# SeoYeonnLee/Video-Chapter-Generation

Hardware: AMD Instinct MI355X
Metric: clip-windows/sec (16f×224²+128tok) train-step at 1/2/4/8 MI355X; % HBM roofline (higher is better)
Workload: dtype bf16; 1 GPU; TwoStream train step: TSM-ResNet-50 + BERT-base + ChapterHead(mlp), B=64 windows/GPU of 16x224^2 frames + 128 tokens, fused clip+AdamW; global_batch=64, seq_len=128, frames=16, resolution=224, text_fill=n_valid ~ U[L/2, L], parallelism=dp1

## Files before the change

### include/vcg_hip.h

```cpp
#ifndef VCG_HIP_H
#define VCG_HIP_H
#include <hip/hip_runtime.h>
#include <stdint.h>
#include "vcg_gpt_decode.h"
#ifdef __cplusplus
extern "C" {
#endif

#define VCG_API
enum { VCG_F32 = 0, VCG_BF16 = 1 };
enum { VCG_GRAD_F32 = 0x10 };
enum { VCG_OK = 0, VCG_ERR_INVALID = -1, VCG_ERR_UNSUPPORTED = -2, VCG_ERR_HIP = -3 };
enum { VCG_ACT_NONE = 0, VCG_ACT_RELU = 1, VCG_ACT_GELU = 2, VCG_ACT_TANH = 3, VCG_ACT_GELU_BWD = 4 };
enum { VCG_ACT_GELU_TANH = 5, VCG_ACT_GELU_TANH_BWD = 6 };
enum { VCG_ACT_FLAG_ROUND_PRE = 0x100 };
enum { VCG_ACT_FLAG_WIDE = 0x200 };
enum { VCG_ACT_FLAG_F32_OUT = 0x400 };
VCG_API int vcg_gemm_census_enable(int on);
VCG_API int vcg_gemm_census_size(void);
VCG_API int vcg_gemm_census_get(int i, char* key, int n, long long* count);

VCG_API const char* vcg_last_error(void);
VCG_API int vcg_version(void);
VCG_API int vcg_init(int device);
VCG_API int vcg_finalize(void);
VCG_API int vcg_sync(hipStream_t stream);
VCG_API int vcg_timing_enable(int on);
VCG_API int vcg_timing_query(int kernel_id, double* ms_total, long long* launches, double* flops);
VCG_API int vcg_timing_roofline(int kernel_id, double peak_tflops, double peak_gbs, double* ms_total, double* ideal_ms, double* bytes, double* flops);
VCG_API int vcg_patch_stamps(unsigned long long* out, int n);
VCG_API int vcg_fast_stamps(unsigned long long* out, int n);
VCG_API int vcg_g256_stamps(unsigned long long* out, int n);
VCG_API int vcg_wide_stamps(unsigned long long* out, int n);

VCG_API int vcg_conv_stats_tiles(int M);
VCG_API int vcg_conv_fwd(int dtype, const void* x, const void* w, void* y, float* stats, int N, int H, int W, int C, int Cout, int KH, int KW, int stride, int pad, int tsm_T, int tsm_fold, hipStream_t stream);
VCG_API int vcg_conv_fwd_bias_act(int dtype, const void* x, const void* w, const float* bias, int act, void* y, int N, int H, int W, int C, int Cout, int KH, int KW, int stride, int pad, int tsm_T, int tsm_fold, hipStream_t stream);
VCG_API int vcg_conv_dgrad(int dtype, const void* dy, const void* wt, void* dx, int N, int H, int W, int C, int Cout, int KH, int KW, int stride, int pad, hipStream_t stream);
VCG_API long long vcg_conv_dgrad_bwd_ws_bytes(int C, int Cout, int KH, int KW);
VCG_API long long vcg_conv_dgrad_bwd_p_ws_bytes(int C, int a2_c);
VCG_API int vcg_conv_dgrad_bwd(int dtype, const void* dy, const void* wt, void* g, int N, int H, int W, int C, int Cout, int KH, int KW, int stride, int pad, int tsm_T, int tsm_fold, const void* res, int res_stride, const unsigned char* bits, const void* y, const float* mean, const float* invstd, const float* mscale, const float* mshift, const void* y2, const float* mean2, const float* invstd2, float* ws, long long ws_bytes, float* sum_g, float* sum_gx, float* dgamma, float* dbeta, float* sum_gx2, float* dgamma2, float* dbeta2, const void* a2, int a2_c, float* pg, float* pws, long long pws_bytes, hipStream_t s);
VCG_API long long vcg_conv_wgrad_ws_bytes(int dtype, int N, int H, int W, int C, int Cout, int KH, int KW, int stride, int pad);
VCG_API int vcg_conv_wgrad(int dtype, const void* x, const void* dy, float* dw, int accumulate, float* ws, long long ws_bytes, int N, int H, int W, int C, int Cin, int Cout, int KH, int KW, int stride, int pad, int tsm_T, int tsm_fold, hipStream_t stream);
VCG_API int vcg_conv1x1_bn_res_relu(const void* x, const void* wfold, const float* bias, const void* res, const float* res_scale, const float* res_shift, void* out, unsigned char* bits, int M, int N, int K, hipStream_t stream);
VCG_API int vcg_bn_bwd_fold_weights(const void* wt, int N, int K, const float* mean, const float* invstd, const float* gamma, const float* sum_g, const float* sum_gx, float inv_count, void* wfold, float* bias, hipStream_t stream);
VCG_API long long vcg_bn_apply_colsum_ws_bytes(long long P, int C);
VCG_API int vcg_bn_apply_colsum(const void* y, const float* scale, const float* shift, int relu, void* out, float* colsum, float* ws, long long ws_bytes, long long P, int C, hipStream_t s);
VCG_API long long vcg_bn_apply_gram_ws_bytes(long long P, int C);
VCG_API int vcg_bn_apply_gram(const void* y, const float* scale, const float* shift, const float* mean, const float* invstd, void* out, float* colsum, float* gram, double* g64, float* ws, long long ws_bytes, long long P, int C, hipStream_t s);
VCG_API int vcg_bn_stats_from_gram(const double* g64, const void* w, long long M, int N, int C, float* stats, int mtiles, hipStream_t s);
VCG_API int vcg_bn_finalize_from_gram(const double* g64, const void* w, long long M, int N, int C, const float* gamma,
                                      const float* beta, float* mean, float* invstd, float* scale, float* shift,
                                      float* running_mean, float* running_var, float momentum, float eps,
                                      const float* w32, void* wfold, hipStream_t s);
VCG_API int vcg_conv1x1_stats(const void* x, const void* w, float* stats, int M, int N, int K, hipStream_t stream);
VCG_API int vcg_bn_bwd_sumgx_from_wgrad(const float* P, const void* w, int K, int C, const float* mean, const float* invstd, const float* sum_g, float* sum_gx, float* dgamma, hipStream_t stream);
VCG_API int vcg_bn_bwd_fold_weights_a2(const void* wt, int C, int K, const float* invstd, const float* gamma, const float* sum_g, const float* sum_gx, float inv_count, const float* colsum_a, void* wfold, float* bias, hipStream_t stream);
VCG_API int vcg_bn_bwd_fold_wgrad_a2(const float* P, const float* G, const float* w3, int K, int C, const float* mean, const float* invstd, const float* gamma, const float* sum_g, const float* sum_gx, float inv_count, const float* colsum_a, float* dw, int accumulate, hipStream_t stream);
VCG_API int vcg_conv_dgrad_bwd_bnfold(const void* g, const void* yg, int Ky, const void* wfold, const float* bias, void* out, int N, int H, int W, int C, int Cout, const void* y, const float* mean, const float* invstd, const float* mscale, const float* mshift, float* ws, long long ws_bytes, float* sum_g, float* sum_gx, float* dgamma, float* dbeta, hipStream_t stream);
VCG_API long long vcg_conv_wgrad_bnfold_ws_bytes(int N, int H, int W, int C, int Cout);
VCG_API int vcg_conv_wgrad_bnfold(const void* x, const void* g, const void* yg, const float* mean, const float* invstd, const float* gamma, const float* sum_g, const float* sum_gx, float inv_count, const float* colsum_x, float* dw, int accumulate, float* ws, long long ws_bytes, int N, int H, int W, int C, int Cout, hipStream_t stream);
VCG_API int vcg_gemm(int dtype, int transA, int transB, int M, int N, int K, const void* A, long long lda, const void* B, long long ldb, void* C, long long ldc, const float* bias, int act, const void* residual, long long ldr, void* aux, float alpha, hipStream_t stream);
VCG_API int vcg_gemm_batched(int dtype, int transA, int transB, int M, int N, int K, const void* A, long long lda, long long a_so, long long a_si, const void* B, long long ldb, long long b_so, long long b_si, void* C, long long ldc, long long c_so, long long c_si, int batch_outer, int batch_inner, const float* bias, int act, float alpha, hipStream_t stream);
VCG_API long long vcg_gemm_splitk_ws_bytes(int dtype, int M, int N, int K);
VCG_API int vcg_gemm_splitk(int dtype, int transA, int transB, int M, int N, int K, const void* A, long long lda, const void* B, long long ldb, float* out, int accumulate, float* ws, long long ws_bytes, hipStream_t stream);

VCG_API int vcg_bn_finalize(const float* stats, int mtiles, int M, int C, const float* gamma, const float* beta, float* mean_out, float* invstd_out, float* scale_out, float* shift_out, float* running_mean, float* running_var, float momentum, float eps, hipStream_t s);
VCG_API int vcg_bn_eval_params(const float* gamma, const float* beta, const float* rm, const float* rv, float eps, int C, float* mean_out, float* invstd_out, float* scale, float* shift, hipStream_t s);
VCG_API int vcg_bn_apply(int dtype, const void* y, const float* scale, const float* shift, const void* res, const float* rscale, const float* rshift, int relu, void* out, unsigned char* bits, long long P, int C, hipStream_t s);
VCG_API long long vcg_bn_bwd_ws_bytes(long long P, int C);
VCG_API int vcg_bn_bwd_reduce(int dtype, const void* dout, int mask_mode, const void* mask, const unsigned char* mbits, const float* mscale, const float* mshift, const void* y, const float* mean, const float* invstd, long long P, int C, float* ws, long long ws_bytes, float* sum_g, float* sum_gx, float* dgamma, float* dbeta, int accumulate, hipStream_t s);
VCG_API int vcg_bn_bwd_apply(int dtype, const void* dout, int mask_mode, const void* mask, const unsigned char* mbits, const float* mscale, const float* mshift, const void* y, const float* mean, const float* invstd, const float* gamma, const float* sum_g, const float* sum_gx, long long count, int train_stats, void* dy, void* gout, long long P, int C, hipStream_t s);
VCG_API int vcg_bn_bwd_apply_dual(int dtype, const void* g, const void* y, const float* mean, const float* invstd, const float* gamma, const float* sum_g, const float* sum_gx, const void* yd, const float* mean_d, const float* invstd_d, const float* gamma_d, const float* sum_g_d, const float* sum_gx_d, long long count, void* dy, void* dyd, long long P, int C, hipStream_t s);
VCG_API int vcg_maxpool_fwd(int dtype, const void* x, void* y, unsigned char* idx, int N, int H, int W, int C, hipStream_t s);
VCG_API int vcg_maxpool_bwd(int dtype, const void* dy, const unsigned char* idx, void* dx, int N, int H, int W, int C, hipStream_t s);
VCG_API long long vcg_maxpool_bwd_bn_ws_bytes(int C);
VCG_API int vcg_maxpool_bwd_bn(int dtype, const void* dy, const unsigned char* idx, void* g, int N, int H, int W, int C, const void* y, const float* mean, const float* invstd, const float* mscale, const float* mshift, float* ws, long long ws_bytes, float* sum_g, float* sum_gx, float* dgamma, float* dbeta, hipStream_t s);
VCG_API int vcg_maxpool_bwd_bn_sums_pooled(int dtype, const void* dy, const void* mp, const unsigned char* idx, const void* y, int N, int H, int W, int C, const float* mean, const float* invstd, const float* mscale, const float* mshift, float* ws, long long ws_bytes, float* sum_g, float* sum_gx, float* dgamma, float* dbeta, hipStream_t s);
VCG_API int vcg_maxpool_bwd_bn_apply(int dtype, const void* dy, const unsigned char* idx, void* dx, int N, int H, int W, int C, const void* y, const float* mean, const float* invstd, const float* mscale, const float* mshift, const float* gamma, const float* sum_g, const float* sum_gx, long long count, int train_stats, hipStream_t s);
VCG_API long long vcg_stem_bwd_fused_ws_bytes(void);
VCG_API int vcg_stem_bwd_fused_fits(int N, int H, int W);
VCG_API int vcg_stem_bwd_fused(const void* dy, const unsigned char* idx, const void* y, const void* x, int N, int H, int W, const float* mean, const float* invstd, const float* mscale, const float* mshift, const float* gamma, const float* sum_g, const float* sum_gx, long long count, int train_stats, float* ws, long long ws_bytes, float* dw, int accumulate, hipStream_t s);
VCG_API int vcg_bn_relu_maxpool(int dtype, const void* y, const float* scale, const float* shift, void* out, unsigned char* idx, int N, int H, int W, int C, hipStream_t s);
VCG_API int vcg_avgpool_fwd(int dtype, const void* x, float* y, int N, int HW, int C, hipStream_t s);
VCG_API int vcg_avgpool_bwd(int dtype, const float* dy, void* dx, int N, int HW, int C, hipStream_t s);
VCG_API int vcg_frames_to_nhwc(int dtype, const float* src, void* dst, int N, int C, int H, int W, int Cpad, hipStream_t s);
VCG_API int vcg_window_frames_u8(int dtype, const uint8_t* frames, const long long* idx, void* dst, long long n_rows, int F, int H, int W, const float* mean3, const float* std3, hipStream_t s);
VCG_API int vcg_window_frames_u8_cpad(int dtype, const uint8_t* frames, const long long* idx, void* dst, long long n_rows, int F, int H, int W, int Cpad, const float* mean3, const float* std3, hipStream_t s);
VCG_API int vcg_weight_prep(int dtype, const float* w, void* out, int Cout, int Cin, int KH, int KW, int Cpad, int transposed, hipStream_t s);
VCG_API int vcg_weight_fold(int dtype, const float* w, const float* scale, void* out, int rows, int cols, hipStream_t s);
VCG_API int vcg_weight_prep_multi(int dtype, const long long* desc, int n, hipStream_t s);
VCG_API int vcg_transpose(int dtype, const void* in, void* out, int rows, int cols, long long ld_in, long long ld_out, hipStream_t s);
VCG_API int vcg_transpose_multi(const long long* desc, int n, int total_tiles, hipStream_t s);
VCG_API int vcg_cast_from_f32(int dtype, const float* in, void* out, long long n, hipStream_t s);
VCG_API int vcg_cast_to_f32(int dtype, const void* in, float* out, long long n, hipStream_t s);
VCG_API int vcg_tsm_shift(int dtype, const void* x, void* y, long long n_batch, int T, int C, long long HW, int fold_div, int direction, hipStream_t s);
VCG_API int vcg_tsm_unshift_add(int dtype, const void* dshift, const void* other, const unsigned char* other_bits, void* dx, long long NT, int T, long long HW, int C, int fold, hipStream_t s);

VCG_API int vcg_embed_ln_fwd(int dtype, const long long* ids, const float* word, const float* pos, const float* type, const float* gamma, const float* beta, void* out, float* mean, float* rstd, int B, int L, int H, float eps, float dropout_p, unsigned long long seed, hipStream_t s);
VCG_API long long vcg_ln_bwd_ws_bytes(int rows, int H);
VCG_API int vcg_embed_ln_bwd(int dtype, const void* dout, const long long* ids, const float* word, const float* pos, const float* type, const float* gamma, const float* mean, const float* rstd, float* word_grad, float* pos_grad, float* type_grad, float* gamma_grad, float* beta_grad, float* ws, long long ws_bytes, int B, int L, int H, float dropout_p, unsigned long long seed, long long pad_idx, hipStream_t s);
VCG_API int vcg_ln_fwd(int dtype, const void* x, const void* res, const float* gamma, const float* beta, void* out, float* mean, float* rstd, int rows, int H, float eps, float dropout_p, unsigned long long seed, hipStream_t s);
VCG_API int vcg_ln_bwd(int dtype, const void* dout, const void* x, const void* res, const float* gamma, const float* mean, const float* rstd, void* dx, void* dres, float* gamma_grad, float* beta_grad, float* bias_grad, float* ws, long long ws_bytes, int rows, int H, float dropout_p, unsigned long long seed, hipStream_t s);
VCG_API long long vcg_colsum_ws_bytes(int rows, int N);
VCG_API int vcg_colsum(int dtype, const void* x, long long ld, int rows, int N, float* out, int accumulate, float* ws, long long ws_bytes, hipStream_t s);
VCG_API int vcg_attn_softmax_fwd(int dtype, const void* S, const long long* mask, void* P, void* Pd, int B, int nh, int L, int Lp, float scale, float dropout_p, unsigned long long seed, hipStream_t s);
VCG_API int vcg_attn_softmax_bwd(int dtype, const void* dPd, const void* P, void* dS, int Z, int L, int Lp, float scale, float dropout_p, unsigned long long seed, hipStream_t s);
VCG_API long long vcg_bert_attn_stats_bytes(int B, int nh, int L);
VCG_API int vcg_bert_attn_fwd(const void* qkv, const long long* mask, void* ctx, void* stats, int B, int nh, int L, int Lp, float scale, float dropout_p, unsigned long long seed, hipStream_t s);
VCG_API int vcg_bert_attn_bwd(const void* qkv, const void* dctx, const void* ctx, const long long* mask, const void* stats, void* dqkv, int B, int nh, int L, int Lp, float scale, float dropout_p, unsigned long long seed, hipStream_t s);
VCG_API int vcg_bert_attn_fwd_varlen(const void* qkv, const long long* mask, const int* seq, void* ctx, void* stats, int B, int nh, int Lmax, int Lp, float scale, float dropout_p, unsigned long long seed, hipStream_t s);
VCG_API int vcg_bert_attn_bwd_varlen(const void* qkv, const void* dctx, const long long* mask, const int* seq, const void* stats, void* dqkv, int B, int nh, int Lmax, int Lp, float scale, float dropout_p, unsigned long long seed, hipStream_t s);
enum { VCG_ATTN_CAUSAL = 1 };
VCG_API int vcg_bert_attn_fwd_ex(const void* qkv, const long long* mask, const int* seq, void* ctx, void* stats, int B, int nh, int Lmax, int Lp, float scale, float dropout_p, unsigned long long seed, int flags, hipStream_t s);
VCG_API int vcg_bert_attn_bwd_ex(const void* qkv, const void* dctx, const long long* mask, const int* seq, const void* stats, void* dqkv, int B, int nh, int Lmax, int Lp, float scale, float dropout_p, unsigned long long seed, int flags, hipStream_t s);
VCG_API int vcg_attn_softmax_fwd_ex(int dtype, const void* S, const long long* mask, void* P, void* Pd, int B, int nh, int L, int Lp, float scale, float dropout_p, unsigned long long seed, int flags, hipStream_t s);
VCG_API int vcg_attn_softmax_bwd_ex(int dtype, const void* dPd, const void* P, void* dS, int Z, int L, int Lp, float scale, float dropout_p, unsigned long long seed, int flags, hipStream_t s);
VCG_API int vcg_gpt_embed_fwd(int dtype, const long long* ids, const float* tok, const float* pos, void* out, int B, int L, int H, float dropout_p, unsigned long long seed, hipStream_t s);
VCG_API int vcg_gpt_embed_bwd(int dtype, const void* dout, const long long* ids, float* tok_grad, float* pos_grad, float* ws, long long ws_bytes, int B, int L, int H, float dropout_p, unsigned long long seed, hipStream_t s);
VCG_API int vcg_tanh_bwd(int dtype, const void* dy, const void* t, void* dx, long long n, hipStream_t s);

VCG_API int vcg_head_mlp_fwd(int dtype, const void* Vout, const void* Lout, const float* W, const float* bias, float* logits, float* prob, int B, int T, int hid, int O, hipStream_t s);
VCG_API int vcg_head_mlp_bwd(int dtype, const void* Vout, const void* Lout, const float* W, const float* dlogits, void* dV, void* dL, float* dW, float* dbias, int B, int T, int hid, int O, int relu_mask, hipStream_t s);
VCG_API long long vcg_head_attn_saved_floats(int B, int T, int hid, int nh);
VCG_API int vcg_head_attn_fwd(int dtype, const void* Vout, const void* Lout, const float* Wq, const float* bq, const float* Wk, const float* bk, const float* Wv, const float* bv, const float* Wp, const float* bp, float* saved, long long saved_floats, float* logits, float* prob, int B, int T, int hid, int nh, int O, float dropout_p, unsigned long long seed, hipStream_t s);
VCG_API long long vcg_head_attn_bwd_ws_floats(int B, int T, int hid);
VCG_API int vcg_head_attn_bwd(int dtype, const float* saved, const float* Wq, const float* Wk, const float* Wv, const float* Wp, const float* dlogits, void* dVout, void* dLout, float* dWq, float* dbq, float* dWk, float* dbk, float* dWv, float* dbv, float* dWp, float* dbp, float* ws, long long ws_floats, int B, int T, int hid, int nh, int O, float dropout_p, unsigned long long seed, int relu_mask, hipStream_t s);
VCG_API long long vcg_window_attn_weight_floats(int H, int nh, int P);
VCG_API int vcg_window_attn_fwd(const float* emb, const float* weights, long long weight_floats, float* logits, float* prob, int B, int S, int H, int nh, int P, hipStream_t s);
VCG_API long long vcg_cross_attn_weight_floats(int H);
VCG_API int vcg_cross_attn_fwd(const float* lang, const float* vis, const float* weights, long long weight_floats, float* out, int B, int T, int H, int nh, hipStream_t s);
VCG_API int vcg_mul_fwd(const float* a, const float* b, float* out, long long n, hipStream_t s);
VCG_API int vcg_rowdot_fwd(const float* U, const float* x, const float* bias, float* out, int B, int R, int K, hipStream_t s);
VCG_API int vcg_rowdot_bwd(const float* U, const float* x, const float* dy, float* dU, float* dx, int B, int R, int K, hipStream_t s);
VCG_API int vcg_ln_act_fwd(const float* x, const float* gamma, const float* beta, float* out, int rows, int D, float eps, int act, hipStream_t s);
VCG_API int vcg_cross_entropy_fwd(const float* logits, const long long* labels, float* loss, int B, int C, hipStream_t s);
VCG_API int vcg_cross_entropy_bwd(const float* logits, const long long* labels, const float* dloss, float* dlogits, int B, int C, hipStream_t s);

VCG_API long long vcg_sumsq_ws_bytes(void);
VCG_API int vcg_sumsq(const float* x, long long n, float* ws, float* out, hipStream_t s);
VCG_API int vcg_adamw(float* p, const float* g, float* m, float* v, const unsigned char* wd_flags, int flag_shift, long long n, float lr, float beta1, float beta2, float eps, float wd, float step_size, float bc2_sqrt, const float* sumsq, float max_norm, float grad_scale, void* bf16_shadow, hipStream_t s);

VCG_API int vcg_ln_act_drop_fwd(const float* x, const float* gamma, const float* beta, float* out, float* mean, float* rstd, int rows, int D, float eps, int act, float dropout_p, unsigned long long seed, hipStream_t s);
VCG_API long long vcg_ln_act_drop_bwd_ws_bytes(int rows, int D);
VCG_API int vcg_ln_act_drop_bwd(const float* dout, const float* x, const float* gamma, const float* beta, const float* mean, const float* rstd, float* dx, float* gamma_grad, float* beta_grad, float* ws, long long ws_bytes, int rows, int D, int act, float dropout_p, unsigned long long seed, hipStream_t s);
VCG_API int vcg_act_drop_fwd(const float* x, const float* res, float* out, long long n, int act, float dropout_p, unsigned long long seed, hipStream_t s);
VCG_API int vcg_act_drop_bwd(const float* dout, const float* x, float* dx, long long n, int act, float dropout_p, unsigned long long seed, hipStream_t s);
VCG_API int vcg_mul_bwd(const float* dout, const float* a, const float* b, float* da, float* db, long long n, hipStream_t s);
VCG_API int vcg_mha_small_fwd(const float* q, long long ldq, const float* k, long long ldk, const float* v, long long ldv, const float* bias, int Pb, float* ctx, long long ldc, float* probs, int B, int Sq, int Sk, int nh, int dh, float scale, float dropout_p, unsigned long long seed, hipStream_t s);
VCG_API long long vcg_mha_small_bwd_ws_bytes(int B, int nh, int Pb);
VCG_API int vcg_mha_small_bwd(const float* q, long long ldq, const float* k, long long ldk, const float* v, long long ldv, const float* probs, const float* dctx, long long lddc, float* dq, long long lddq, float* dk, long long lddk, float* dv, long long lddv, float* dbias, int Pb, float* ws, long long ws_bytes, int B, int Sq, int Sk, int nh, int dh, float scale, float dropout_p, unsigned long long seed, hipStream_t s);

VCG_API int vcg_posenc_fwd(const float* x, const float* pos, const float* w, const float* b, float* out, long long rows, int S, int H, hipStream_t s);
VCG_API int vcg_posenc_bwd(const float* d, const float* pos, float* dw, float* db, long long rows, int S, int H, hipStream_t s);
VCG_API int vcg_linear_small_fwd(const float* x, const float* W, const float* b, const float* res, float* y, int M, int N, int K, int act, hipStream_t s);
VCG_API int vcg_linear_small_bwd(const float* g, const float* x, const float* W, float* dx, float* dw, float* db, int M, int N, int K, hipStream_t s);
VCG_API int vcg_softmax_rows(const float* x, float* out, int rows, int C, hipStream_t s);

VCG_API long long vcg_mlm_loss_ws_bytes(int R, int V, int H);
VCG_API int vcg_mlm_loss_fwd(const void* hidden, int rows_total, const long long* rows, const void* W, const long long* targets, int R, int V, int H, float* ws, long long ws_bytes, float* lse, float* row_loss, float* mean_loss, long long* n_correct, hipStream_t stream);
VCG_API int vcg_mlm_loss_bwd(const void* hidden, int rows_total, const long long* rows, const void* W, const long long* targets, const float* lse, const float* dloss, int R, int V, int H, void* dZ, long long ldz, hipStream_t stream);
VCG_API int vcg_mlm_logits(const void* hidden, int rows, const void* W, int V, int H, float* logits, long long ldz, hipStream_t stream);
VCG_API int vcg_mlm_reduce_f32(const float* logits, long long ldz, const long long* targets, int R, int V, float* ws, long long ws_bytes, float* lse, float* row_loss, float* mean_loss, long long* n_correct, hipStream_t stream);
VCG_API int vcg_mlm_dz_f32(float* logits, long long ldz, const float* lse, const long long* targets, const float* dloss, int R, int V, hipStream_t stream);
VCG_API int vcg_seq_softmax_fwd(const float* logits, long long ldz, float* prob, long long ldp, int B, int L, int V, hipStream_t stream);

VCG_API int vcg_momentum_update(float* k, const float* q, long long n, float m, float one_minus_m, void* k_shadow, hipStream_t stream);
VCG_API int vcg_l2norm_fwd(int dtype, const void* x, void* y, float* denom, int N, int H, float eps, hipStream_t stream);
VCG_API int vcg_l2norm_bwd(int dtype, const float* g, const void* x, const float* denom, float* dx, int N, int H, hipStream_t stream);
VCG_API int vcg_contrast_select(int dtype, const void* q, const void* cand, int B, int C, int H, float eps, long long* k0, hipStream_t stream);
VCG_API int vcg_queue_enqueue(int key_dtype, int km_dtype, const void* keys, float* queue, void* queue_km, long long* queue_ptr, int N, int K, int H, hipStream_t stream);
VCG_API int vcg_queue_rebuild(int km_dtype, const float* queue, void* queue_km, int K, int H, hipStream_t stream);
VCG_API int vcg_rowdot(int dtype, const void* a, const void* b, int N, int H, float scale, float* out, long long ldo, hipStream_t stream);
VCG_API long long vcg_infonce_ws_bytes(int N, int K, int H);
VCG_API int vcg_infonce_fwd(const void* q, const void* queue_km, const float* lpos, int N, int K, int H, float inv_T, float* ws, long long ws_bytes, float* lse, float* row_loss, float* one_minus_p0, float* mean_loss, long long* n_correct, hipStream_t stream);
VCG_API int vcg_infonce_dz(const void* q, const void* queue_km, const float* lse, int N, int K, int H, float inv_T, float scale, void* dZ, long long ldz, hipStream_t stream);
VCG_API int vcg_infonce_logits(const void* q, const void* queue_km, int N, int K, int H, float inv_T, float* key_logits, long long ldz, hipStream_t stream);
VCG_API int vcg_infonce_reduce_f32(const float* key_logits, long long ldz, const float* lpos, int N, int K, float* ws, long long ws_bytes, float* lse, float* row_loss, float* one_minus_p0, float* mean_loss, long long* n_correct, hipStream_t stream);
VCG_API int vcg_infonce_dz_f32(float* key_logits, long long ldz, const float* lse, float scale, int N, int K, hipStream_t stream);
VCG_API int vcg_infonce_dq_pos(int dtype, float* dq, const void* k, const float* one_minus_p0, float scale, int N, int H, hipStream_t stream);

VCG_API int vcg_listnet_max_slate(void);
VCG_API int vcg_listnet_max_hidden(void);
VCG_API int vcg_listnet_fwd(int dtype, const void* P, const float* targets, const long long* sel, const long long* cls, const float* W, const float* bias, int B, int S, int H, int M, float* p, float* logits, float* prob, float* part, float* loss3, hipStream_t stream);
VCG_API int vcg_listnet_bwd(int dtype, const void* P, const float* targets, const long long* sel, const long long* cls, const float* W, const float* p, const float* prob, const float* dloss, int B, int S, int H, int M, float* dP, float* dW, float* db, hipStream_t stream);

VCG_API int vcg_attn_decode(int dtype, const void* qkv_new, void* kcache, void* vcache, const int* len0, int max_len0, int t, void* ctx, int B, int nh, int dh, int Tcap, float scale, hipStream_t s);
VCG_API int vcg_sample_topk(const float* logits, long long ldz, int B, int V, float temperature, int top_k, int greedy, const float* u, long long* seq, int Tcap, const int* len0, int max_len0, int col_off, const long long* forced, long long forced_ld, long long* chosen, long long chosen_ld, float* prob, hipStream_t s);
VCG_API int vcg_gpt_embed_at(int dtype, const long long* seq, int Tcap, const int* len0, int max_len0, int t, const float* tok, const float* pos, void* out, int B, int H, int V, int n_pos, hipStream_t s);
VCG_API int vcg_gemm_skinny(const void* x, const void* W, const float* bias, void* y, int M, int N, int K, long long ldc, int act, int f32_out, hipStream_t s);
VCG_API long long vcg_gpt_decode_desc_bytes(void);
VCG_API int vcg_gpt_decode_step(const vcg_gpt_decode_desc* d, int t, hipStream_t s);

VCG_API int vcg_cross_attn_kv_fwd(int dtype, const void* q, long long ldq, const void* kv, long long ldkv, const long long* key_mask, void* ctx, float* stats, int B, int nh, int dh, int Lq, int Lk, float scale, hipStream_t s);
VCG_API int vcg_pegasus_embed_fwd(int dtype, const long long* ids, const float* tok, const float* pos, void* out, int B, int L, int H, int V, int n_pos, float scale, int pos0, hipStream_t s);

VCG_API int vcg_cross_attn_kv_fwd_ex(int dtype, const void* q, long long ldq, const void* kv, long long ldkv, const long long* key_mask, void* ctx, float* stats, int B, int nh, int dh, int Lq, int Lk, float scale, float dropout_p, unsigned long long seed, hipStream_t s);
VCG_API int vcg_cross_attn_kv_bwd(int dtype, const void* q, long long ldq, const void* kv, long long ldkv, const long long* key_mask, const void* dctx, long long lddo, const float* stats, float* d_ws, void* dq, long long lddq, void* dkv, long long lddkv, int B, int nh, int dh, int Lq, int Lk, float scale, float dropout_p, unsigned long long seed, hipStream_t s);
VCG_API int vcg_pegasus_embed_fwd_ex(int dtype, const long long* ids, const float* tok, const float* pos, void* out, int B, int L, int H, int V, int n_pos, float scale, int pos0, float dropout_p, unsigned long long seed, hipStream_t s);
VCG_API int vcg_pegasus_embed_bwd(int dtype, const void* dout, const long long* ids, float* tok_grad, float* ws, long long ws_bytes, int B, int L, int H, float scale, long long pad_idx, float dropout_p, unsigned long long seed, hipStream_t s);
VCG_API int vcg_ln_bwd_acc(int dtype, const void* dout, const float* x, const float* gamma, const float* mean, const float* rstd, float* dh, float* gamma_grad, float* beta_grad, float* ws, long long ws_bytes, int rows, int H, hipStream_t s);
VCG_API int vcg_dropout_add_fwd(int dtype, float* h, const void* branch, long long n, float dropout_p, unsigned long long seed, hipStream_t s);
VCG_API int vcg_dropout_add_bwd(int dtype, const float* dh, void* dbranch, long long n, float dropout_p, unsigned long long seed, hipStream_t s);
VCG_API int vcg_relu_dropout_fwd(int dtype, const void* pre, void* f, long long n, float dropout_p, unsigned long long seed, hipStream_t s);
VCG_API int vcg_relu_dropout_bwd(int dtype, const void* dy, const void* f, void* dpre, long long n, float dropout_p, hipStream_t s);

VCG_API int vcg_comm_unique_id(void* uid_out, int uid_bytes);
VCG_API int vcg_comm_init(int rank, int world, const void* uid, int uid_bytes);
VCG_API int vcg_comm_world(int* rank, int* world);
VCG_API int vcg_allreduce_bucket(void* ptr, long long count, int dtype, hipStream_t s);
VCG_API int vcg_broadcast_bucket(void* ptr, long long count, int dtype, int root, hipStream_t s);
VCG_API int vcg_comm_finalize(void);

VCG_API int vcg_synth(int kind, void* out, long long n, unsigned long long key, double a, double b, hipStream_t s);

#ifdef __cplusplus
}
#endif
#endif
```

### video-chapter-generation_amd/csrc/igemm.h

```cpp
#pragma once
#include "common.h"

namespace vcg {

enum { OP_DENSE_K = 0, OP_IM2COL = 1, OP_DGRAD = 2, OP_DENSE_MN = 3, OP_IM2COL_T = 4 };
enum { EPI_STORE = 0, EPI_STATS = 1, EPI_SPLITK = 2, EPI_BWD = 3, EPI_BWD_AFF = 4, EPI_STORE_AUX = 5,
       EPI_BWD_STREAM = 6 };
enum { ACT_NONE = 0, ACT_RELU = 1, ACT_GELU = 2, ACT_TANH = 3, ACT_GELU_BWD = 4, ACT_GELU_TANH = 5, ACT_GELU_TANH_BWD = 6 };
__host__ __device__ __forceinline__ bool act_is_gelu_bwd(int act) { return act == ACT_GELU_BWD || act == ACT_GELU_TANH_BWD; }
enum { ACT_FLAG_ROUND_PRE = 0x100 };
enum { ACT_FLAG_WIDE = 0x200 };
enum { ACT_FLAG_F32_OUT = 0x400 };

template <typename T> struct Cfg;
template <> struct Cfg<float> { static constexpr int VEC = 4, BK = 16, LDK = 20; };
template <> struct Cfg<bf16_t> { static constexpr int VEC = 8, BK = 32, LDK = 40; };

template <typename T, int COLS> struct LdMN {
  static constexpr int v = sizeof(T) == 2 ? (COLS == 128 ? 144 : 80) : (COLS == 128 ? 132 : 68);
};

constexpr bool is_kcontig(int mode) { return mode == OP_DENSE_K || mode == OP_IM2COL || mode == OP_DGRAD; }

struct OpArgs {
  const void* ptr;
  long long bytes;
  long long ld;
  int rows;
  int N, H, W, C, logC;
  int GH, GW;
  int KH, KW, stride, pad;
  int tsm_T, tsm_fold;
  FastDiv fd_ghw, fd_gw, fd_T;
  int tKH, tKW, tkh0, tkw0, ry, rx;
  int sw, pw;
  const void* ptr2;
  int split2;
  long long ld2, bytes2;
};

struct BwdEpi {
  int tsm_T, tsm_fold;
  FastDiv fd_hw, fd_T;
  int hw;
  const void* res;
  int res_s;
  int rH, rW;
  FastDiv fd_w;
  const uint8_t* bits;
  const void* y;
  const float *mean, *invstd, *msc, *msh;
  const void* y2;
  const float *mean2, *invstd2;
  float* part;
  int nred;
  const void* a2;
  int pj;
  float* ppart;
  int sub, cW, ry, rx, fH, fW;
  FastDiv fd_chw, fd_cw;
};

struct GemmParams {
  int M, N, K;
  int k_per_split;
  OpArgs a, b;
  void* C;
  long long ldc;
  const float* bias;
  int act;
  const void* residual;
  long long ldr;
  void* aux;
  float alpha;
  float* stats;
  float* ws;
  int batch_inner;
  long long a_so, a_si, b_so, b_si, c_so, c_si;
  int res_round;
  int fast_act;
  BwdEpi bwd;
  uint8_t* obits;
  const float *res_sc, *res_sh;
};


template <typename T> __device__ __forceinline__ void load4(const T* p, float (&v)[4]) {
  if constexpr (sizeof(T) == 4) {
    const float4 q = *reinterpret_cast<const float4*>(p);
    v[0] = q.x; v[1] = q.y; v[2] = q.z; v[3] = q.w;
  } else {
    const uint2 q = *reinterpret_cast<const uint2*>(p);
    v[0] = __uint_as_float(q.x << 16); v[1] = __uint_as_float(q.x & 0xffff0000u);
    v[2] = __uint_as_float(q.y << 16); v[3] = __uint_as_float(q.y & 0xffff0000u);
  }
}
template <typename T> __device__ __forceinline__ void store4(T* p, const float (&v)[4]) {
  if constexpr (sizeof(T) == 4) {
    *reinterpret_cast<float4*>(p) = make_float4(v[0], v[1], v[2], v[3]);
  } else {
    uint2 q;
    q.x = (uint32_t)f2bf(v[0]) | ((uint32_t)f2bf(v[1]) << 16);
    q.y = (uint32_t)f2bf(v[2]) | ((uint32_t)f2bf(v[3]) << 16);
    *reinterpret_cast<uint2*>(p) = q;
  }
}

__device__ __forceinline__ float apply_act(float v, int act, bool fast = false) {
  if (act == ACT_RELU) return fmaxf(v, 0.f);
  if (act == ACT_GELU) return fast ? gelu_erf_fast(v) : gelu_erf(v);
  if (act == ACT_TANH) return tanhf(v);
  if (act == ACT_GELU_TANH) return fast ? gelu_tanh_fast(v) : gelu_tanh(v);
  return v;
}


__device__ __forceinline__ float row16_sum(float v) {
  v += __builtin_bit_cast(float, __builtin_amdgcn_update_dpp(0, __builtin_bit_cast(int, v), 0xB1, 0xF, 0xF, false));
  v += __builtin_bit_cast(float, __builtin_amdgcn_update_dpp(0, __builtin_bit_cast(int, v), 0x4E, 0xF, 0xF, false));
  v += __builtin_bit_cast(float, __builtin_amdgcn_update_dpp(0, __builtin_bit_cast(int, v), 0x141, 0xF, 0xF, false));
  v += __builtin_bit_cast(float, __builtin_amdgcn_update_dpp(0, __builtin_bit_cast(int, v), 0x140, 0xF, 0xF, false));
  return v;
}

template <int BN>
__device__ __forceinline__ void load_bias(float (&bv)[BN / 32][4], const float* bias, int n0, int wn, int lane, int N) {
#pragma unroll
  for (int j = 0; j < BN / 32; ++j) {
    const int n = n0 + wn * (BN / 2) + 4 * (lane >> 4) + j * 16;
    float4 b4 = make_float4(0.f, 0.f, 0.f, 0.f);
    if (bias && n < N) b4 = *reinterpret_cast<const float4*>(bias + n);
    bv[j][0] = b4.x; bv[j][1] = b4.y; bv[j][2] = b4.z; bv[j][3] = b4.w;
  }
}

__device__ __forceinline__ void ep_barrier() {
  __builtin_amdgcn_s_waitcnt(0xC07F);
  __builtin_amdgcn_s_barrier();
}

template <typename T, int BM, int BN, int EPI>
__device__ __forceinline__ void gemm_epilogue(f32x4 (&acc)[BM / 32][BN / 32], const GemmParams& p, float* red,
                                              const float (&bv)[BN / 32][4], T* Cout, const T* Res, int m0, int n0,
                                              int wm, int wn, int lane, int mtile, int mtiles) {
  constexpr int MT = BM / 32, NT = BN / 32;
  const int g = lane >> 4, ci = lane & 15;
  const int mbase = m0 + wm * (BM / 2) + ci, nbase = n0 + wn * (BN / 2) + 4 * g;
#pragma unroll
  for (int j = 0; j < NT; ++j) {
    const int n = nbase + j * 16;
#pragma unroll
    for (int i = 0; i < MT; ++i) {
      const int m = mbase + i * 16;
      if (m >= p.M || n >= p.N) {
        acc[i][j] = f32x4{0.f, 0.f, 0.f, 0.f};
        continue;
      }
      float v[4];
#pragma unroll
      for (int r = 0; r < 4; ++r) v[r] = acc[i][j][r] * p.alpha + bv[j][r];
      if (Res) {
        float rv[4];
        load4<T>(Res + (long long)m * p.ldr + n, rv);
        if (p.act == ACT_GELU_BWD) {
#pragma unroll
          for (int r = 0; r < 4; ++r) v[r] *= (sizeof(T) == 2 && p.fast_act) ? gelu_erf_grad_fast(rv[r]) : gelu_erf_grad(rv[r]);
        } else if (p.act == ACT_GELU_TANH_BWD) {
#pragma unroll
          for (int r = 0; r < 4; ++r) v[r] *= (sizeof(T) == 2 && p.fast_act) ? gelu_tanh_grad_fast(rv[r]) : gelu_tanh_grad(rv[r]);
        } else {
#pragma unroll
          for (int r = 0; r < 4; ++r) v[r] += rv[r];
        }
      }
      if (p.aux) store4<T>(reinterpret_cast<T*>(p.aux) + (long long)m * p.ldc + n, v);
      if (p.act != ACT_NONE && !act_is_gelu_bwd(p.act)) {
#pragma unroll
        for (int r = 0; r < 4; ++r) v[r] = apply_act(v[r], p.act, sizeof(T) == 2 && p.fast_act);
      }
      if constexpr (EPI == EPI_STATS) {
#pragma unroll
        for (int r = 0; r < 4; ++r) acc[i][j][r] = to_f<T>(from_f<T>(v[r]));
      } else {
        store4<T>(Cout + (long long)m * p.ldc + n, v);
      }
    }
  }
  if constexpr (EPI == EPI_STATS) {
    const int r0 = m0 + wm * (BM / 2);
    const int cw = min(BM / 2, max(0, p.M - r0));
    const float inv_cw = cw > 0 ? 1.f / (float)cw : 0.f;
#pragma unroll
    for (int j = 0; j < NT; ++j)
#pragma unroll
      for (int r = 0; r < 4; ++r) {
        float t = 0.f;
#pragma unroll
        for (int i = 0; i < MT; ++i) t += acc[i][j][r];
        t = row16_sum(t);
        const float mean = t * inv_cw;
        float q = 0.f;
#pragma unroll
        for (int i = 0; i < MT; ++i) {
          const float d = acc[i][j][r] - mean;
          q += (mbase + i * 16 < p.M) ? d * d : 0.f;
        }
        q = row16_sum(q);
        if (ci == 0) {
          const int lc = wn * (BN / 2) + j * 16 + 4 * g + r;
          red[wm * 2 * BN + lc] = mean;
          red[wm * 2 * BN + BN + lc] = q;
        }
      }
    ep_barrier();
    if (wm == 0 && ci == 0) {
      const float n1 = (float)min(BM / 2, max(0, p.M - m0));
      const float n2 = (float)min(BM / 2, max(0, p.M - m0 - BM / 2));
#pragma unroll
      for (int j = 0; j < NT; ++j)
#pragma unroll
        for (int r = 0; r < 4; ++r) {
          const int lc = wn * (BN / 2) + j * 16 + 4 * g + r;
          const int col = n0 + lc;
          if (col >= p.N) continue;
          float mean = red[lc], m2 = red[BN + lc];
          if (n2 > 0.f) {
            const float mb = red[2 * BN + lc], d = mb - mean, nt = n1 + n2;
            mean += d * (n2 / nt);
            m2 += red[3 * BN + lc] + d * d * (n1 * n2 / nt);
          }
          reinterpret_cast<float2*>(p.stats)[(long long)col * mtiles + mtile] = make_float2(mean, m2);
        }
    }
    if (blockIdx.x == 0 && threadIdx.x == 0)
      reinterpret_cast<float2*>(p.stats)[(long long)p.N * mtiles + mtile] =
          make_float2((float)min(BM, p.M - m0), 0.f);
#pragma unroll
    for (int j = 0; j < NT; ++j) {
      const int n = nbase + j * 16;
#pragma unroll
      for (int i = 0; i < MT; ++i) {
        const int m = mbase + i * 16;
        if (m >= p.M || n >= p.N) continue;
        float v[4] = {acc[i][j][0], acc[i][j][1], acc[i][j][2], acc[i][j][3]};
        store4<T>(Cout + (long long)m * p.ldc + n, v);
      }
    }
  }
}

int run_fast_gemm(GemmParams& p, int amode, int epi, int z, hipStream_t s);
int fast_grid_rows(int M, int N, int z, int epi);
bool fast_bwd_streams(const GemmParams& p);
int wide_gemm_class(const GemmParams& p);
int wide_gemm_class_f32(const GemmParams& p);
int run_gemm_wide(GemmParams& p, int we, hipStream_t s);
int fast_bwd_slots(const GemmParams& p);
int run_patch_conv(const GemmParams& p, int amode, int epi, hipStream_t s);
int patch_bwd_slots(const GemmParams& p);
int bn_bwd_finalize_launch(const float* partial, int nb, int C, long long ld, int gx_off, float* sum_g, float* sum_gx,
                           float* dgamma, float* dbeta, int accumulate, hipStream_t s);
int run_fast_wgrad(const GemmParams& p, int splits, hipStream_t s, bool dense_b = false);
int wgrad_patch_rows(int dtype, int H, int W, int C, int Cin, int Cout, int KH, int KW, int stride, int pad,
                     int tsm_fold);
int wgrad_patch_splits(int C, int Cout);
int run_rs1x1_bnres(const void* x, const void* wfold, const float* bias, const void* res, void* out, uint8_t* bits,
                    long long M, int N, int K, hipStream_t s);
int run_wgrad_patch(const void* x, const void* dy, float* ws, int N, int H, int W, int C, int Cout, int R,
                    hipStream_t s);
int wgrad_fast_tile_m(int M);
int wgrad_fast_tile_n(int N);

bool gemm256_ok(const GemmParams& p, int amode, int epi, int z);
int run_gemm256(const GemmParams& p, int amode, int epi, hipStream_t s);

}
```

### video-chapter-generation_amd/csrc/igemm.hip

```cpp
#include <cstdio>

#include "igemm.h"

namespace vcg {

template <typename T, int ROWS, int MODE> struct Loader {
  static constexpr int VEC = Cfg<T>::VEC, BK = Cfg<T>::BK;
  static constexpr int NC = ROWS * 4 / 256;
  static constexpr bool KC = is_kcontig(MODE);
  static constexpr int CPR = ROWS / VEC;

  uint4 reg[NC];
  const T* ptr[NC];
  int ra[NC], rb[NC], rc[NC];
  int sub[NC];
  int lds_off[NC];

  __device__ __forceinline__ void init(const OpArgs& a, int row0, int tid) {
    const T* base = reinterpret_cast<const T*>(a.ptr);
#pragma unroll
    for (int j = 0; j < NC; ++j) {
      const int q = tid + j * 256;
      if constexpr (KC) {
        const int row = q >> 2;
// ... 810 lines not shown
}

static void wgrad_geometry(int dtype, int N, int H, int W, int C, int Cout, int KH, int KW, int stride, int pad,
                           int* M, int* Nn, int* K, int* splits, int* kps, bool* fast) {
  const int OH = (H + 2 * pad - KH) / stride + 1, OW = (W + 2 * pad - KW) / stride + 1;
  const bool pair = stem_pair(dtype, C);
  int KWp = KW, pwp = 0;
  if (pair) pair_taps(KW, pad, &KWp, &pwp);
  *M = Cout;
  *Nn = pair ? KH * KWp * 8 : KH * KW * C;
  *K = N * OH * OW;
  *fast = wgrad_fast_ok(dtype, N, H, pair ? W / 2 : W, pair ? 8 : C, Cout, *K);
  int BK, sp;
  if (*fast) {
    BK = 64;
    const int tiles = ((*Nn + wgrad_fast_tile_n(*Nn) - 1) / wgrad_fast_tile_n(*Nn)) *
                      ((*M + wgrad_fast_tile_m(*M) - 1) / wgrad_fast_tile_m(*M));
    sp = (splitk_target() + tiles - 1) / tiles;
    const int max_sp = (*K + 8 * BK - 1) / (8 * BK);
    sp = sp > max_sp ? max_sp : sp;
    sp = sp < 1 ? 1 : sp;
  } else {
    BK = dtype == VCG_BF16 ? 32 : 16;
    sp = choose_splits(*M, *Nn, *K, BK);
  }
  int k = (*K + sp - 1) / sp;
  k = (k + BK - 1) / BK * BK;
  *kps = k;
  *splits = (*K + k - 1) / k;
}

VCG_API long long vcg_conv_wgrad_ws_bytes(int dtype, int N, int H, int W, int C, int Cout, int KH, int KW,
                                          int stride, int pad) {
  int M, Nn, K, splits, kps;
  bool fast;
  wgrad_geometry(dtype, N, H, W, C, Cout, KH, KW, stride, pad, &M, &Nn, &K, &splits, &kps, &fast);
  if (wgrad_patch_rows(dtype, H, W, C, C, Cout, KH, KW, stride, pad, 0) > 0 && splits < wgrad_patch_splits(C, Cout))
    splits = wgrad_patch_splits(C, Cout);
  return (long long)splits * M * Nn * 4;
}

static int conv_wgrad_impl(int dtype, const void* x, const float* in_sc, const float* in_sh, const void* dy,
                           float* dw, int accumulate, float* ws, long long ws_bytes, int N, int H, int W, int C, int Cin,
                           int Cout, int KH, int KW, int stride, int pad, int tsm_T, int tsm_fold, hipStream_t stream);

VCG_API int vcg_conv_wgrad(int dtype, const void* x, const void* dy, float* dw, int accumulate, float* ws,
                           long long ws_bytes, int N, int H, int W, int C, int Cin, int Cout, int KH, int KW,
                           int stride, int pad, int tsm_T, int tsm_fold, hipStream_t stream) {
  return conv_wgrad_impl(dtype, x, nullptr, nullptr, dy, dw, accumulate, ws, ws_bytes, N, H, W, C, Cin, Cout, KH, KW,
                         stride, pad, tsm_T, tsm_fold, stream);
}

static int conv_wgrad_impl(int dtype, const void* x, const float* in_sc, const float* in_sh, const void* dy,
                           float* dw, int accumulate, float* ws, long long ws_bytes, int N, int H, int W, int C, int Cin,
                           int Cout, int KH, int KW, int stride, int pad, int tsm_T, int tsm_fold, hipStream_t stream) {
  const int logC = ilog2_exact(C);
  VCG_REQUIRE(logC >= 0, "C must be a power of two");
  VCG_REQUIRE(Cout % 64 == 0, "Cout must be a multiple of 64");
  int M, Nn, K, splits, kps;
  bool fast;
  wgrad_geometry(dtype, N, H, W, C, Cout, KH, KW, stride, pad, &M, &Nn, &K, &splits, &kps, &fast);
  const bool pair = stem_pair(dtype, C);
  int KWp = KW, pwp = 0;
  if (pair) pair_taps(KW, pad, &KWp, &pwp);
  VCG_REQUIRE(!pair || (fast && stride == 2 && W % 2 == 0 && tsm_fold == 0),
              "bf16 C = 4 (pair-packed stem) needs stride 2, even W, no TSM and the fast engine");
  VCG_REQUIRE(ws_bytes >= (long long)splits * M * Nn * 4, "workspace too small");
  const int OH = (H + 2 * pad - KH) / stride + 1, OW = (W + 2 * pad - KW) / stride + 1;
  GemmParams p{};
  p.M = M;
  p.N = Nn;
  p.K = K;
  p.k_per_split = kps;
  p.a = dense_op(dy, Cout, Cout);
  p.a.bytes = (long long)K * Cout * (dtype == VCG_BF16 ? 2 : 4);
  OpArgs b{};
  b.ptr = x; b.rows = Nn; b.N = N; b.H = H; b.W = W; b.C = C; b.logC = logC;
  b.bytes = (long long)N * H * W * C * (dtype == VCG_BF16 ? 2 : 4);
  b.GH = OH; b.GW = OW; b.KH = KH; b.KW = KW; b.stride = stride; b.pad = pad;
  b.tsm_T = tsm_T > 0 ? tsm_T : 1; b.tsm_fold = tsm_fold;
  b.fd_ghw = make_fastdiv(OH * OW); b.fd_gw = make_fastdiv(OW); b.fd_T = make_fastdiv(b.tsm_T);
  if (pair) {
    b.W = W / 2; b.C = 8; b.logC = 3; b.KW = KWp; b.sw = 1; b.pw = pwp;
  }
  p.b = b;
  p.ws = ws;
  p.alpha = 1.f;
  const int wpr = wgrad_patch_rows(dtype, H, W, C, Cin, Cout, KH, KW, stride, pad, tsm_fold);
  if (wpr > 0) {
    const int wsp = wgrad_patch_splits(C, Cout);
    VCG_REQUIRE(ws_bytes >= (long long)wsp * M * Nn * 4, "workspace too small");
    if (FILE* f = gemm_log())
      fprintf(f, "a=3 b=4 epi=2 M=%d N=%d K=%d z=%d fast=3 conv=%dx%d/%d C=%d\n", M, Nn, K, wsp, KH, KW, stride, C);
    int rc = run_wgrad_patch(x, dy, ws, N, H, W, C, Cout, wpr, stream);
    if (rc) return rc;
    const long long MN = (long long)M * Nn;
    splitk_reduce(stream, ws, wsp, MN,
                       Nn, dw, accumulate, 1, KH, KW, C, Cin, 1.f, KW, 0, pad);
    VCG_LAUNCH_CHECK();
    return VCG_OK;
  }
  FILE* f = fast ? gemm_log() : nullptr;
  if (f)
    fprintf(f, "a=3 b=4 epi=2 M=%d N=%d K=%d z=%d fast=2 conv=%dx%d/%d C=%d\n", M, Nn, K, splits, KH, KW, stride, C);
  int rc;
  if (fast)
    rc = run_fast_wgrad(p, splits, stream);
  else
    rc = dtype == VCG_BF16 ? run_gemm<bf16_t, OP_DENSE_MN, OP_IM2COL_T>(p, EPI_SPLITK, splits, stream)
                           : run_gemm<float, OP_DENSE_MN, OP_IM2COL_T>(p, EPI_SPLITK, splits, stream);
  if (rc) return rc;
  const long long MN = (long long)M * Nn;
  splitk_reduce(stream, ws, splits,
                     MN, Nn, dw, accumulate, pair ? 2 : 1, KH, KW, C, Cin, 1.f, KWp, pwp, pad);
  VCG_LAUNCH_CHECK();
  return VCG_OK;
}

namespace {
__global__ __launch_bounds__(256) void bn_fold_weights_kernel(const bf16_t* __restrict__ wt, int K,
                                                              const float* __restrict__ mean,
                                                              const float* __restrict__ invstd,
                                                              const float* __restrict__ gamma,
                                                              const float* __restrict__ sum_g,
                                                              const float* __restrict__ sum_gx, float ic,
                                                              bf16_t* __restrict__ wf, float* __restrict__ bias) {
  __shared__ float red[256];
  const int n = blockIdx.x, t = threadIdx.x;
  float acc = 0.f;
  for (int k = t; k < K; k += 256) {
    const float is = invstd[k], A = (gamma ? gamma[k] : 1.f) * is;
    const float B = -A * is * sum_gx[k] * ic;
    const float w = bf2f(wt[(long long)n * K + k]);
    const bf16_t wy = f2bf(B * w);
    wf[(long long)n * 2 * K + k] = f2bf(A * w);
    wf[(long long)n * 2 * K + K + k] = wy;
    acc += (-A * sum_g[k] * ic) * w - mean[k] * bf2f(wy);
  }
  red[t] = acc;
  __syncthreads();
  for (int o = 128; o > 0; o >>= 1) {
    if (t < o) red[t] += red[t + o];
    __syncthreads();
  }
  if (t == 0) bias[n] = red[0];
}

template <int G>
__global__ __launch_bounds__(256) void splitk_reduce_bnfold_kernel(const float* __restrict__ ws, int splits, int Cout,
                                                                   int N, const float* __restrict__ mean,
                                                                   const float* __restrict__ invstd,
                                                                   const float* __restrict__ gamma,
                                                                   const float* __restrict__ sum_g,
                                                                   const float* __restrict__ sum_gx, float ic,
                                                                   const float* __restrict__ cs, float* __restrict__ out,
                                                                   int accumulate) {
  const long long MN = (long long)Cout * N, slab = 2 * MN;
  const long long gid = blockIdx.x * (long long)blockDim.x + threadIdx.x;
  const long long idx = gid / G;
  const int t = (int)(gid - idx * G);
  if (idx >= MN) return;
  float v1 = 0.f, v2 = 0.f;
  const float* p = ws + idx;
  for (int s = t; s < splits; s += G) {
    v1 += p[(long long)s * slab];
    v2 += p[(long long)s * slab + MN];
  }
#pragma unroll
  for (int o = G / 2; o > 0; o >>= 1) {
    v1 += __shfl_xor(v1, o, 64);
    v2 += __shfl_xor(v2, o, 64);
  }
  if (t != 0) return;
  const int k = (int)(idx / N), n = (int)(idx - (long long)k * N);
  const float is = invstd[k], A = (gamma ? gamma[k] : 1.f) * is;
  const float B = -A * is * sum_gx[k] * ic;
  const float Cc = -A * sum_g[k] * ic - B * mean[k];
  const float v = fmaf(A, v1, fmaf(B, v2, Cc * cs[n]));
  if (accumulate) out[idx] += v;
  else out[idx] = v;
}
}

VCG_API int vcg_bn_bwd_fold_weights(const void* wt, int N, int K, const float* mean, const float* invstd,
                                    const float* gamma, const float* sum_g, const float* sum_gx, float inv_count,
                                    void* wfold, float* bias, hipStream_t stream) {
  VCG_REQUIRE(wt && wfold && bias && mean && invstd && sum_g && sum_gx, "null argument");
  VCG_REQUIRE(N > 0 && K > 0, "empty weight");
  hipLaunchKernelGGL(bn_fold_weights_kernel, dim3(N), dim3(256), 0, stream, (const bf16_t*)wt, K, mean, invstd, gamma,
                     sum_g, sum_gx, inv_count, (bf16_t*)wfold, bias);
  VCG_LAUNCH_CHECK();
  return VCG_OK;
}

namespace {
constexpr int FW_NB = 2;
__global__ __launch_bounds__(256) void bn_fold_weights_a2_kernel(const bf16_t* __restrict__ wt, int C, int K,
                                                                 const float* __restrict__ invstd,
                                                                 const float* __restrict__ gamma,
                                                                 const float* __restrict__ sum_g,
                                                                 const float* __restrict__ sum_gx, float ic,
                                                                 const float* __restrict__ colsum_a,
                                                                 bf16_t* __restrict__ wf, float* __restrict__ bias) {
  __shared__ float bw[FW_NB][2048];
  __shared__ float red[FW_NB][256];
  const int n0 = blockIdx.x * FW_NB, t = threadIdx.x;
  float acc[FW_NB];
#pragma unroll
  for (int q = 0; q < FW_NB; ++q) acc[q] = 0.f;
  for (int k = t; k < K; k += 256) {
    const float is = invstd[k], A = (gamma ? gamma[k] : 1.f) * is;
    const float B = -A * is * sum_gx[k] * ic;
#pragma unroll
    for (int q = 0; q < FW_NB; ++q) {
      const int n = n0 + q;
      if (n < C) {
        const float w = bf2f(wt[(long long)n * K + k]);
        bw[q][k] = B * w;
        wf[(long long)n * (K + C) + k] = f2bf(A * w);
        acc[q] += (-A * sum_g[k] * ic) * w;
      }
    }
  }
  __syncthreads();
  for (int j = t; j < C; j += 256) {
    const bf16_t* row = wt + (long long)j * K;
    float qv[FW_NB];
#pragma unroll
    for (int q = 0; q < FW_NB; ++q) qv[q] = 0.f;
    for (int k0 = 0; k0 < K; k0 += 64) {
      uint4 u8[8];
#pragma unroll
      for (int b = 0; b < 8; ++b) u8[b] = *reinterpret_cast<const uint4*>(row + k0 + 8 * b);
#pragma unroll
      for (int b = 0; b < 8; ++b) {
        const uint32_t w4[4] = {u8[b].x, u8[b].y, u8[b].z, u8[b].w};
#pragma unroll
        for (int e = 0; e < 8; ++e) {
          const float w = __uint_as_float((e & 1) ? (w4[e >> 1] & 0xffff0000u) : (w4[e >> 1] << 16));
#pragma unroll
          for (int q = 0; q < FW_NB; ++q) qv[q] = fmaf(w, bw[q][k0 + 8 * b + e], qv[q]);
        }
      }
    }
#pragma unroll
    for (int q = 0; q < FW_NB; ++q) {
      const int n = n0 + q;
      if (n < C) {
        const bf16_t qb = f2bf(qv[q]);
        wf[(long long)n * (K + C) + K + j] = qb;
        acc[q] -= colsum_a[j] * ic * bf2f(qb);
      }
    }
  }
#pragma unroll
  for (int q = 0; q < FW_NB; ++q) red[q][t] = acc[q];
  __syncthreads();
  for (int o = 128; o > 0; o >>= 1) {
    if (t < o) {
#pragma unroll
      for (int q = 0; q < FW_NB; ++q) red[q][t] += red[q][t + o];
    }
    __syncthreads();
  }
  if (t < FW_NB && n0 + t < C) bias[n0 + t] = red[t][0];
}

__global__ __launch_bounds__(256) void bn_fold_wgrad_a2_kernel(const float* __restrict__ P, const float* __restrict__ G,
                                                               const float* __restrict__ w3, int K, int C,
                                                               const float* __restrict__ mean,
                                                               const float* __restrict__ invstd,
                                                               const float* __restrict__ gamma,
                                                               const float* __restrict__ sum_g,
                                                               const float* __restrict__ sum_gx, float ic,
                                                               const float* __restrict__ cs, float* __restrict__ dw,
                                                               int accumulate) {
  __shared__ float wr[512];
  const int k = blockIdx.x;
  for (int i = threadIdx.x; i < C; i += 256) wr[i] = w3[(long long)k * C + i];
  __syncthreads();
  const float is = invstd[k], A = (gamma ? gamma[k] : 1.f) * is;
  const float B = -A * is * sum_gx[k] * ic;
  const float Cc = -A * sum_g[k] * ic - B * mean[k];
  for (int j = threadIdx.x; j < C; j += 256) {
    float wg = 0.f;
    for (int i0 = 0; i0 < C; i0 += 16) {
      float gv[16];
#pragma unroll
      for (int u = 0; u < 16; ++u) gv[u] = G[(long long)(i0 + u) * C + j];
#pragma unroll
      for (int u = 0; u < 16; ++u) wg = fmaf(wr[i0 + u], gv[u], wg);
    }
    const float v = fmaf(A, P[(long long)k * C + j], fmaf(B, wg, Cc * cs[j]));
    float* o = dw + (long long)k * C + j;
    *o = accumulate ? *o + v : v;
  }
}
}

namespace {
__global__ __launch_bounds__(64) void bn_sumgx_kernel(const float* __restrict__ P, const bf16_t* __restrict__ w, int C,
                                                      const float* __restrict__ mean, const float* __restrict__ invstd,
                                                      const float* __restrict__ sum_g, float* __restrict__ sum_gx,
                                                      float* __restrict__ dgamma) {
  const int k = blockIdx.x, t = threadIdx.x;
  float a = 0.f;
  for (int j = t; j < C; j += 64) a = fmaf(bf2f(w[(long long)k * C + j]), P[(long long)k * C + j], a);
#pragma unroll
  for (int o = 32; o > 0; o >>= 1) a += __shfl_xor(a, o, 64);
  if (t == 0) {
    const float v = invstd[k] * (a - mean[k] * sum_g[k]);
    sum_gx[k] = v;
    if (dgamma) dgamma[k] += v;
  }
}
}

VCG_API int vcg_bn_bwd_sumgx_from_wgrad(const float* P, const void* w, int K, int C, const float* mean,
                                        const float* invstd, const float* sum_g, float* sum_gx, float* dgamma,
                                        hipStream_t stream) {
  VCG_REQUIRE(P && w && mean && invstd && sum_g && sum_gx, "null argument");
  VCG_REQUIRE(K > 0 && C > 0, "empty");
  hipLaunchKernelGGL(bn_sumgx_kernel, dim3(K), dim3(64), 0, stream, P, (const bf16_t*)w, C, mean, invstd, sum_g,
                     sum_gx, dgamma);
  VCG_LAUNCH_CHECK();
  return VCG_OK;
}

VCG_API int vcg_bn_bwd_fold_weights_a2(const void* wt, int C, int K, const float* invstd, const float* gamma,
                                       const float* sum_g, const float* sum_gx, float inv_count, const float* colsum_a,
                                       void* wfold, float* bias, hipStream_t stream) {
  VCG_REQUIRE(wt && wfold && bias && invstd && sum_g && sum_gx && colsum_a, "null argument");
  VCG_REQUIRE(C > 0 && K > 0 && K <= 2048 && K % 64 == 0, "K must be a multiple of 64, <= 2048");
  VCG_REQUIRE(((uintptr_t)wt & 15) == 0, "wt must be 16-B aligned");
  hipLaunchKernelGGL(bn_fold_weights_a2_kernel, dim3((C + FW_NB - 1) / FW_NB), dim3(256), 0, stream, (const bf16_t*)wt, C, K, invstd, gamma,
                     sum_g, sum_gx, inv_count, colsum_a, (bf16_t*)wfold, bias);
  VCG_LAUNCH_CHECK();
  return VCG_OK;
}

VCG_API int vcg_bn_bwd_fold_wgrad_a2(const float* P, const float* G, const float* w3, int K, int C, const float* mean,
                                     const float* invstd, const float* gamma, const float* sum_g, const float* sum_gx,
                                     float inv_count, const float* colsum_a, float* dw, int accumulate,
                                     hipStream_t stream) {
  VCG_REQUIRE(P && G && w3 && mean && invstd && sum_g && sum_gx && colsum_a && dw, "null argument");
  VCG_REQUIRE(C > 0 && C <= 512 && C % 16 == 0 && K > 0, "C must be a multiple of 16, <= 512");
  hipLaunchKernelGGL(bn_fold_wgrad_a2_kernel, dim3(K), dim3(256), 0, stream, P, G, w3, K, C, mean, invstd, gamma,
                     sum_g, sum_gx, inv_count, colsum_a, dw, accumulate);
  VCG_LAUNCH_CHECK();
  return VCG_OK;
}

VCG_API int vcg_conv_dgrad_bwd_bnfold(const void* g, const void* yg, int Ky, const void* wfold, const float* bias,
                                      void* out, int N, int H, int W, int C, int Cout, const void* y, const float* mean,
                                      const float* invstd, const float* mscale, const float* mshift, float* ws,
                                      long long ws_bytes, float* sum_g, float* sum_gx, float* dgamma, float* dbeta,
                                      hipStream_t stream) {
  VCG_REQUIRE(g && yg && wfold && bias && out, "null argument");
  VCG_REQUIRE(C % 64 == 0 && Cout % 64 == 0 && Ky % 64 == 0, "C, Cout and Ky must be multiples of 64");
  VCG_REQUIRE(!mscale || (mshift && y), "mscale needs mshift and y");
  VCG_REQUIRE(!y || (mean && invstd && sum_g && sum_gx), "the reduction needs mean/invstd/sum_g/sum_gx");
  VCG_REQUIRE(ws_bytes >= vcg_conv_dgrad_bwd_ws_bytes(C, Cout + Ky, 1, 1), "workspace too small");
  const long long M = (long long)N * H * W;
  if (!fast_gemm_enabled() || M * C * 2 >= 0xFFFFFF00LL || M * Cout * 2 >= 0xFFFFFF00LL || M * Ky * 2 >= 0xFFFFFF00LL ||
      M >= (1LL << 31))
    return VCG_ERR_UNSUPPORTED;
  GemmParams p{};
  p.M = (int)M;
  p.N = C;
  p.K = Cout + Ky;
  p.k_per_split = p.K + 64;
  p.a = dense_op(g, Cout, p.M, Cout, 2);
  p.a.ptr2 = yg;
  p.a.split2 = Cout;
  p.a.ld2 = Ky;
  p.a.bytes2 = M * Ky * 2;
  p.b = dense_op(wfold, p.K, C, p.K, 2);
  p.bias = bias;
  p.C = out;
  p.ldc = C;
  p.alpha = 1.f;
  BwdEpi& e = p.bwd;
  e.hw = H * W;
  e.fd_hw = make_fastdiv((uint32_t)(H * W));
  e.fd_T = make_fastdiv(1u);
  e.fd_w = make_fastdiv((uint32_t)W);
  e.res_s = 1;
  e.y = y; e.mean = mean; e.invstd = invstd; e.msc = mscale; e.msh = mshift;
  e.part = ws;
  e.nred = y ? 2 : 0;
  if (FILE* f = gemm_log()) {
    fprintf(f, "a=0 b=0 epi=3 M=%d N=%d K=%d z=1 fast=1 conv=1x1/1 C=%d bnfold=1\n", p.M, p.N, p.K, Cout);
    fflush(f);
  }
  int rc = run_fast_gemm(p, OP_DENSE_K, EPI_BWD, 1, stream);
  if (rc < 0) return VCG_ERR_UNSUPPORTED;
  if (rc) return rc;
  if (e.nred > 0) {
    rc = bn_bwd_finalize_launch(ws, fast_bwd_slots(p), C, 2LL * C, C, sum_g, sum_gx, dgamma, dbeta, 1, stream);
    if (rc) return rc;
  }
  return VCG_OK;
}

VCG_API long long vcg_conv_wgrad_bnfold_ws_bytes(int N, int H, int W, int C, int Cout) {
  int M, Nn, K, splits, kps;
  bool fast;
  wgrad_geometry(VCG_BF16, N, H, W, C, 2 * Cout, 1, 1, 1, 0, &M, &Nn, &K, &splits, &kps, &fast);
  return (long long)splits * M * Nn * 4;
}

VCG_API int vcg_conv_wgrad_bnfold(const void* x, const void* g, const void* yg, const float* mean, const float* invstd,
                                  const float* gamma, const float* sum_g, const float* sum_gx, float inv_count,
                                  const float* colsum_x, float* dw, int accumulate, float* ws, long long ws_bytes, int N,
                                  int H, int W, int C, int Cout, hipStream_t stream) {
  VCG_REQUIRE(x && g && yg && mean && invstd && sum_g && sum_gx && colsum_x && dw, "null argument");
  const int logC = ilog2_exact(C);
  VCG_REQUIRE(logC >= 6 && Cout % 128 == 0, "C must be a power of two >= 64, Cout a multiple of 128");
  int M, Nn, K, splits, kps;
  bool fast;
  wgrad_geometry(VCG_BF16, N, H, W, C, 2 * Cout, 1, 1, 1, 0, &M, &Nn, &K, &splits, &kps, &fast);
  if (!fast || wgrad_fast_tile_m(M) != 128 || (long long)K * Cout * 2 >= 0xFFFFFF00LL) return VCG_ERR_UNSUPPORTED;
  VCG_REQUIRE(ws_bytes >= (long long)splits * M * Nn * 4, "workspace too small");
  GemmParams p{};
  p.M = M;
  p.N = Nn;
  p.K = K;
  p.k_per_split = kps;
  p.a = dense_op(g, Cout, Cout);
  p.a.bytes = (long long)K * Cout * 2;
  p.a.ptr2 = yg;
  p.a.split2 = Cout;
  OpArgs b{};
  b.ptr = x; b.rows = Nn; b.N = N; b.H = H; b.W = W; b.C = C; b.logC = logC;
  b.bytes = (long long)N * H * W * C * 2;
  b.GH = H; b.GW = W; b.KH = 1; b.KW = 1; b.stride = 1; b.pad = 0;
  b.tsm_T = 1; b.tsm_fold = 0;
  b.fd_ghw = make_fastdiv(H * W); b.fd_gw = make_fastdiv(W); b.fd_T = make_fastdiv(1);
  p.b = b;
  p.ws = ws;
  p.alpha = 1.f;
  if (FILE* f = gemm_log())
    fprintf(f, "a=3 b=4 epi=2 M=%d N=%d K=%d z=%d fast=2 conv=1x1/1 C=%d bnfold=1\n", M, Nn, K, splits, C);
  int rc = run_fast_wgrad(p, splits, stream);
  if (rc) return rc;
  const long long MN = (long long)Cout * Nn;
  if ((MN + 255) / 256 < 1024 && splits >= 16)
    hipLaunchKernelGGL(splitk_reduce_bnfold_kernel<8>, dim3((unsigned)((MN * 8 + 255) / 256)), dim3(256), 0, stream,
                       ws, splits, Cout, Nn, mean, invstd, gamma, sum_g, sum_gx, inv_count, colsum_x, dw, accumulate);
  else
    hipLaunchKernelGGL(splitk_reduce_bnfold_kernel<1>, dim3((unsigned)((MN + 255) / 256)), dim3(256), 0, stream, ws,
                       splits, Cout, Nn, mean, invstd, gamma, sum_g, sum_gx, inv_count, colsum_x, dw, accumulate);
  VCG_LAUNCH_CHECK();
  return VCG_OK;
}

VCG_API int vcg_conv1x1_stats(const void* x, const void* w, float* stats, int M, int N, int K, hipStream_t stream) {
  VCG_REQUIRE(x && w && stats, "null argument");
  VCG_REQUIRE(M > 0 && N % 64 == 0 && K % 64 == 0, "N and K must be multiples of 64");
  if (!fast_gemm_enabled() || (long long)M * K * 2 >= 0xFFFFFF00LL) return VCG_ERR_UNSUPPORTED;
  GemmParams p{};
  p.M = M;
  p.N = N;
  p.K = K;
  p.k_per_split = K + 64;
  p.a = dense_op(x, K, M, K, 2);
  p.b = dense_op(w, K, N, K, 2);
  p.C = nullptr;
  p.ldc = N;
  p.alpha = 1.f;
  p.stats = stats;
  if (FILE* f = gemm_log()) {
    fprintf(f, "a=0 b=0 epi=1 M=%d N=%d K=%d z=1 fast=1 conv=1x1/1 C=%d nostore=1\n", M, N, K, K);
    fflush(f);
  }
  const int rc = run_fast_gemm(p, OP_DENSE_K, EPI_STATS, 1, stream);
  return rc < 0 ? VCG_ERR_UNSUPPORTED : rc;
}

VCG_API int vcg_conv1x1_bn_res_relu(const void* x, const void* wfold, const float* bias, const void* res,
                                    const float* res_scale, const float* res_shift, void* out, unsigned char* bits,
                                    int M, int N, int K, hipStream_t stream) {
  VCG_REQUIRE(x && wfold && bias && res && out && bits, "null argument");
  VCG_REQUIRE(M > 0 && N % 64 == 0 && K % 64 == 0, "N and K must be multiples of 64");
  VCG_REQUIRE((((uintptr_t)x | (uintptr_t)wfold | (uintptr_t)res | (uintptr_t)out) & 15) == 0, "16-B alignment");
  VCG_REQUIRE(!res_scale == !res_shift, "res_scale and res_shift go together");
  if (!res_scale) {
    const int rc = run_rs1x1_bnres(x, wfold, bias, res, out, bits, M, N, K, stream);
    if (rc >= 0) {
      if (FILE* f = gemm_log()) {
        fprintf(f, "a=0 b=0 epi=0 M=%d N=%d K=%d z=1 fast=4 conv=1x1/1 C=%d bnres=1\n", M, N, K, K);
        fflush(f);
      }
      return rc;
    }
  }
  if (!fast_gemm_enabled() || (long long)M * K * 2 >= 0xFFFFFF00LL || (long long)M * N * 2 >= 0xFFFFFF00LL)
    return VCG_ERR_UNSUPPORTED;
  GemmParams p{};
  p.M = M;
  p.N = N;
  p.K = K;
  p.k_per_split = K + 64;
  p.a = dense_op(x, K, M, K, 2);
  p.b = dense_op(wfold, K, N, K, 2);
  p.C = out;
  p.ldc = N;
  p.alpha = 1.f;
  p.bias = bias;
  p.act = ACT_RELU;
  p.residual = res;
  p.ldr = N;
  p.res_round = 1;
  p.obits = bits;
  p.res_sc = res_scale;
  p.res_sh = res_shift;
  if (FILE* f = gemm_log()) {
    fprintf(f, "a=0 b=0 epi=0 M=%d N=%d K=%d z=1 fast=1 conv=1x1/1 C=%d bnres=1\n", M, N, K, K);
    fflush(f);
  }
  const int rc = run_fast_gemm(p, OP_DENSE_K, EPI_STORE, 1, stream);
  return rc < 0 ? VCG_ERR_UNSUPPORTED : rc;
}

VCG_API int vcg_gemm(int dtype, int transA, int transB, int M, int N, int K, const void* A, long long lda,
                     const void* B, long long ldb, void* C, long long ldc, const float* bias, int act,
                     const void* residual, long long ldr, void* aux, float alpha, hipStream_t stream) {
  const int VEC = dtype == VCG_BF16 ? 8 : 4;
  VCG_REQUIRE(N % VEC == 0 && ldc % VEC == 0 && K % VEC == 0, "N, ldc, K must be multiples of 16 bytes");
  VCG_REQUIRE(residual == nullptr || ldr % 4 == 0, "ldr must be a multiple of 4");
  VCG_REQUIRE(M > 0 && N > 0 && K > 0, "empty GEMM");
  GemmParams p{};
  p.M = M; p.N = N; p.K = K; p.k_per_split = K + 64;
  const int esz = dtype == VCG_BF16 ? 2 : 4;
  p.a = transA ? dense_op(A, lda, K, M, esz) : dense_op(A, lda, M, K, esz);
  p.b = transB ? dense_op(B, ldb, K, N, esz) : dense_op(B, ldb, N, K, esz);
  p.a.rows = M;
  p.b.rows = N;
  VCG_REQUIRE((act & ~(0xff | ACT_FLAG_ROUND_PRE | ACT_FLAG_WIDE | ACT_FLAG_F32_OUT)) == 0, "unknown act flags");
  const bool wide = (act & ACT_FLAG_WIDE) != 0 && dtype == VCG_BF16 && !transA && !transB;
  const bool f32out = (act & ACT_FLAG_F32_OUT) != 0;
  VCG_REQUIRE(!f32out || (wide && residual && (act & 0xff) == 0 && !aux && alpha == 1.f),
              "VCG_ACT_FLAG_F32_OUT: a wide-engine bf16 GEMM with a residual addend only");
  act &= ~(ACT_FLAG_WIDE | ACT_FLAG_F32_OUT);
  p.C = C; p.ldc = ldc; p.bias = bias; p.act = act & 0xff; p.residual = residual; p.ldr = ldr; p.aux = aux;
  p.res_round = (act & ACT_FLAG_ROUND_PRE) != 0 && residual != nullptr;
  p.alpha = alpha;
  if (wide) {
    p.fast_act = fast_gelu_enabled();
    const int we = f32out ? wide_gemm_class_f32(p) : wide_gemm_class(p);
    VCG_REQUIRE(!f32out || we >= 0, "VCG_ACT_FLAG_F32_OUT: unsupported shape / alignment");
    if (we >= 0) {
      if (FILE* f = gemm_log()) {
        fprintf(f, "wide M=%d N=%d K=%d we=%d\n", M, N, K, we);
        fflush(f);
      }
      return run_gemm_wide(p, we, stream);
    }
  }
#define VCG_GEMM_CASE(TT)                                                                   \
  if (!transA && !transB) return run_gemm<TT, OP_DENSE_K, OP_DENSE_K>(p, EPI_STORE, 1, stream);   \
  if (!transA && transB) return run_gemm<TT, OP_DENSE_K, OP_DENSE_MN>(p, EPI_STORE, 1, stream);   \
  if (transA && !transB) return run_gemm<TT, OP_DENSE_MN, OP_DENSE_K>(p, EPI_STORE, 1, stream);   \
  return run_gemm<TT, OP_DENSE_MN, OP_DENSE_MN>(p, EPI_STORE, 1, stream);
  if (dtype == VCG_BF16) { VCG_GEMM_CASE(bf16_t) }
  VCG_GEMM_CASE(float)
#undef VCG_GEMM_CASE
}

VCG_API long long vcg_gemm_splitk_ws_bytes(int dtype, int M, int N, int K) {
  const int splits = choose_splits(M, N, K, dtype == VCG_BF16 ? 32 : 16, VCG_SPLITK_TARGET_DENSE);
  return (long long)splits * M * N * 4;
}

VCG_API int vcg_gemm_splitk(int dtype, int transA, int transB, int M, int N, int K, const void* A, long long lda,
                            const void* B, long long ldb, float* out, int accumulate, float* ws, long long ws_bytes,
                            hipStream_t stream) {
  const int BK = dtype == VCG_BF16 ? 32 : 16;
  int splits = choose_splits(M, N, K, BK, VCG_SPLITK_TARGET_DENSE);
  VCG_REQUIRE(ws_bytes >= (long long)splits * M * N * 4, "workspace too small");
  int kps = (K + splits - 1) / splits;
  kps = (kps + BK - 1) / BK * BK;
  splits = (K + kps - 1) / kps;
  GemmParams p{};
  p.M = M; p.N = N; p.K = K; p.k_per_split = kps;
  p.a = dense_op(A, lda, M);
  p.b = dense_op(B, ldb, N);
  p.ws = ws;
  p.alpha = 1.f;
  int rc;
  const long long a_ext = ((long long)(K - 1) * lda + M) * 2, b_ext = ((long long)(K - 1) * ldb + N) * 2;
  if (dtype == VCG_BF16 && transA && transB && fast_gemm_enabled() &&
      M % 8 == 0 && N % 8 == 0 && lda % 8 == 0 && ldb % 8 == 0 && a_ext < 0xFFFFFF00LL && b_ext < 0xFFFFFF00LL) {
    p.a.bytes = a_ext;
    p.b.bytes = b_ext;
    int fk = (K + splits - 1) / splits;
    fk = (fk + 63) / 64 * 64;
    const int fsplits = (K + fk - 1) / fk;
    p.k_per_split = fk;
    if (FILE* f = gemm_log()) {
      fprintf(f, "a=3 b=3 epi=2 M=%d N=%d K=%d z=%d fast=2 conv=0x0/0 C=0\n", M, N, K, fsplits);
      fflush(f);
    }
    rc = run_fast_wgrad(p, fsplits, stream, true);
    if (rc) return rc;
    const long long MN = (long long)M * N;
    splitk_reduce(stream, ws, fsplits,
                       MN, N, out, accumulate, 0, 1, 1, 1, 1, 1.f, 0, 0, 0);
    VCG_LAUNCH_CHECK();
    return VCG_OK;
  }
#define VCG_SK_CASE(TT)                                                                             \
  if (!transA && !transB) rc = run_gemm<TT, OP_DENSE_K, OP_DENSE_K>(p, EPI_SPLITK, splits, stream);       \
  else if (!transA && transB) rc = run_gemm<TT, OP_DENSE_K, OP_DENSE_MN>(p, EPI_SPLITK, splits, stream);  \
  else if (transA && !transB) rc = run_gemm<TT, OP_DENSE_MN, OP_DENSE_K>(p, EPI_SPLITK, splits, stream);  \
  else rc = run_gemm<TT, OP_DENSE_MN, OP_DENSE_MN>(p, EPI_SPLITK, splits, stream);
  if (dtype == VCG_BF16) { VCG_SK_CASE(bf16_t) } else { VCG_SK_CASE(float) }
#undef VCG_SK_CASE
  if (rc) return rc;
  const long long MN = (long long)M * N;
  splitk_reduce(stream, ws, splits,
                     MN, N, out, accumulate, 0, 1, 1, 1, 1, 1.f, 0, 0, 0);
  VCG_LAUNCH_CHECK();
  return VCG_OK;
}

VCG_API int vcg_gemm_batched(int dtype, int transA, int transB, int M, int N, int K, const void* A, long long lda,
                             long long a_so, long long a_si, const void* B, long long ldb, long long b_so,
                             long long b_si, void* C, long long ldc, long long c_so, long long c_si, int batch_outer,
                             int batch_inner, const float* bias, int act, float alpha, hipStream_t stream) {
  const int VEC = dtype == VCG_BF16 ? 8 : 4;
  VCG_REQUIRE(N % VEC == 0 && ldc % VEC == 0, "N and ldc must be multiples of 16 bytes");
  VCG_REQUIRE(batch_outer > 0 && batch_inner > 0 && M > 0 && N > 0 && K > 0, "empty batched GEMM");
  GemmParams p{};
  p.M = M; p.N = N; p.K = K; p.k_per_split = K + 64;
  const int esz = dtype == VCG_BF16 ? 2 : 4;
  p.a = transA ? dense_op(A, lda, K, M, esz) : dense_op(A, lda, M, K, esz);
  p.b = transB ? dense_op(B, ldb, K, N, esz) : dense_op(B, ldb, N, K, esz);
  p.a.rows = M;
  p.b.rows = N;
  p.a.bytes += ((long long)(batch_outer - 1) * a_so + (long long)(batch_inner - 1) * a_si) * esz;
  p.b.bytes += ((long long)(batch_outer - 1) * b_so + (long long)(batch_inner - 1) * b_si) * esz;
  p.C = C; p.ldc = ldc; p.bias = bias; p.act = act; p.alpha = alpha;
  p.batch_inner = batch_inner;
  p.a_so = a_so; p.a_si = a_si; p.b_so = b_so; p.b_si = b_si; p.c_so = c_so; p.c_si = c_si;
  const int z = batch_outer * batch_inner;
#define VCG_BT_CASE(TT)                                                                   \
  if (!transA && !transB) return run_gemm<TT, OP_DENSE_K, OP_DENSE_K>(p, EPI_STORE, z, stream);   \
  if (!transA && transB) return run_gemm<TT, OP_DENSE_K, OP_DENSE_MN>(p, EPI_STORE, z, stream);   \
  if (transA && !transB) return run_gemm<TT, OP_DENSE_MN, OP_DENSE_K>(p, EPI_STORE, z, stream);   \
  return run_gemm<TT, OP_DENSE_MN, OP_DENSE_MN>(p, EPI_STORE, z, stream);
  if (dtype == VCG_BF16) { VCG_BT_CASE(bf16_t) }
  VCG_BT_CASE(float)
#undef VCG_BT_CASE
}
```

### video-chapter-generation_amd/csrc/igemm_fast.hip

```cpp
#include "fast_epilogue.h"

#ifdef VCG_FAST_STAMPS
namespace vcg { __device__ unsigned long long g_fast_stamps[64 * 4]; }
#define FAST_STAMP(t, k)                                                                       \
  do {                                                                                         \
    if (blockIdx.x == 0 && threadIdx.x == 0 && (t) < 64) vcg::g_fast_stamps[(t) * 4 + (k)] = __builtin_amdgcn_s_memtime(); \
  } while (0)
#else
#define FAST_STAMP(t, k) do {} while (0)
#endif

#include "bwd_stream.h"

namespace vcg {

template <int BN, int AM, int EPI, int RES>
__device__ __forceinline__ void igemm_fast_body(const GemmParams& p) {
  constexpr int BM = 128, NW = 4;
  constexpr int MT = 4, NT = BN / 32;
  constexpr int AE = BM * FBK, BE = BN * FBK;
  constexpr int NLD = BM / (8 * NW) + BN / (8 * NW);
  constexpr bool BWD = EPI == EPI_BWD || EPI == EPI_BWD_AFF;
  constexpr int CPAR = BWD ? 6 * BN : 0;
  constexpr int RED = 4 * BN + 2 + 4;
  __shared__ __attribute__((aligned(1024))) char smem[2 * (AE + BE) * 2 + (RED + CPAR) * 4];
  bf16_t* As = reinterpret_cast<bf16_t*>(smem);
  bf16_t* Bs = As + 2 * AE;
  float* red = reinterpret_cast<float*>(smem + 2 * (AE + BE) * 2);
  float* cpar = red + RED;

  const int tid = threadIdx.x, lane = tid & 63, wave = __builtin_amdgcn_readfirstlane(tid >> 6);
  const int wm = wave >> 1, wn = wave & 1;
  const int nx = (p.N + BN - 1) / BN, gy = gridDim.x / nx;
  int bx, by;
  xcd_row_decode(nx, gy, bx, by);
  const int n0 = bx * BN;
  long long aoff = 0, boff = 0;
  bf16_t* Cout = reinterpret_cast<bf16_t*>(p.C);
  const bf16_t* Res = RES ? reinterpret_cast<const bf16_t*>(p.residual) : nullptr;
  if (p.batch_inner > 0) {
    const int zo = blockIdx.z / p.batch_inner, zi = blockIdx.z - zo * p.batch_inner;
    aoff = zo * p.a_so + zi * p.a_si;
    boff = zo * p.b_so + zi * p.b_si;
    Cout += zo * p.c_so + zi * p.c_si;
    if (Res) Res += zo * p.c_so + zi * p.c_si;
  }
  const int mtiles = (p.M + BM - 1) / BM;
  const int my_tiles = by < mtiles ? (mtiles - 1 - by) / gy + 1 : 0;
  const int ntiles = (p.K + FBK - 1) / FBK;
  const int steps = my_tiles * ntiles;
  if constexpr (BWD) {
    if (steps == 0) {
      if (p.bwd.nred > 0 && tid < BN && n0 + tid < p.N)
        for (int r = 0; r < p.bwd.nred; ++r) p.bwd.part[((long long)by * p.bwd.nred + r) * p.N + n0 + tid] = 0.f;
      return;
    }
    if (tid < BN) {
      const int n = min(n0 + tid, p.N - 1);
      const BwdEpi& e = p.bwd;
      cpar[tid] = e.mean ? e.mean[n] : 0.f;
      cpar[BN + tid] = e.msc ? e.msc[n] : 0.f;
      cpar[2 * BN + tid] = e.msh ? e.msh[n] : 0.f;
      cpar[3 * BN + tid] = e.mean2 ? e.mean2[n] : 0.f;
      cpar[4 * BN + tid] = e.invstd ? e.invstd[n] : 0.f;
      cpar[5 * BN + tid] = e.invstd2 ? e.invstd2[n] : 0.f;
    }
  }
  if (steps == 0) return;

  float bv[NT][4];
  if constexpr (EPI == EPI_STATS) {
#pragma unroll
    for (int j = 0; j < NT; ++j) bv[j][0] = bv[j][1] = bv[j][2] = bv[j][3] = 0.f;
  } else {
    load_bias<BN>(bv, p.bias, n0, wn, lane, p.N);
#pragma unroll
    for (int j = 0; j < NT; ++j) asm volatile("" ::"v"(bv[j][0]), "v"(bv[j][1]), "v"(bv[j][2]), "v"(bv[j][3]));
  }

  FastLoader<BM, AM, NW> la;
  FastLoader<BN, OP_DENSE_K, NW> lb;
  la.init(p.a, aoff, by * BM, wave, lane);
  lb.init(p.b, boff, n0, wave, lane);

  f32x4 acc[MT][NT];
#pragma unroll
  for (int i = 0; i < MT; ++i)
#pragma unroll
    for (int j = 0; j < NT; ++j) acc[i][j] = f32x4{0.f, 0.f, 0.f, 0.f};

  float b1[8], b2[8], b3[8];
  int scnt = 0;
#pragma unroll
  for (int i = 0; i < 8; ++i) b1[i] = b2[i] = b3[i] = 0.f;

  int ikt = 0, itile = 0;
  auto issue_next = [&](int stage) {
    if (ikt == 0 && itile > 0) la.init(p.a, aoff, (by + itile * gy) * BM, wave, lane);
    la.issue(p.a, ikt * FBK, p.K, As + stage * AE, wave);
    lb.issue(p.b, ikt * FBK, p.K, Bs + stage * BE, wave);
    if (++ikt == ntiles) {
      ikt = 0;
      ++itile;
    }
  };
  issue_next(0);
  int kt = 0, tile = 0, cur = 0;
  for (int s = 0; s < steps; ++s) {
    if (s + 1 < steps) {
      issue_next(cur ^ 1);
      __builtin_amdgcn_s_waitcnt(waitcnt_vm(NLD));
    } else {
      __builtin_amdgcn_s_waitcnt(waitcnt_vm(0));
    }
    __builtin_amdgcn_s_barrier();
    if (kt == 0) FAST_STAMP(tile, 0);
    const bf16_t* Ac = As + cur * AE;
    const bf16_t* Bc = Bs + cur * BE;
#pragma unroll
    for (int s2 = 0; s2 < 2; ++s2) {
      s16x8 af[MT], bfr[NT];
#pragma unroll
      for (int i = 0; i < MT; ++i) af[i] = fast_frag(Ac, wm * 64 + i * 16, lane, s2);
#pragma unroll
      for (int j = 0; j < NT; ++j) bfr[j] = fast_frag(Bc, wn * (BN / 2) + j * 16, lane, s2);
#pragma unroll
      for (int i = 0; i < MT; ++i)
#pragma unroll
        for (int j = 0; j < NT; ++j)
          acc[i][j] = __builtin_amdgcn_mfma_f32_16x16x32_bf16(bfr[j], af[i], acc[i][j], 0, 0, 0);
    }
    __builtin_amdgcn_s_waitcnt(0xC07F);
    __builtin_amdgcn_s_barrier();
    if (++kt == ntiles) {
      FAST_STAMP(tile, 1);
      const int mt = by + tile * gy;
      bf16_t* stA = As + cur * AE;
      bf16_t* stB = Bs + cur * BE;
      if constexpr (BWD) {
#pragma unroll
        for (int j = 0; j < NT; ++j)
#pragma unroll
          for (int i = 0; i < MT; ++i) {
            float v[4] = {acc[i][j][0], acc[i][j][1], acc[i][j][2], acc[i][j][3]};
            if constexpr (AM == OP_DENSE_K2) {
#pragma unroll
              for (int r = 0; r < 4; ++r) v[r] += bv[j][r];
            }
            stage_put<BN>(stA, stB, wm, wn, lane, i, j, v);
          }
        FAST_STAMP(tile, 2);
        stage_flush_bwd<BN, EPI == EPI_BWD_AFF>(stA, stB, p, Cout, mt * BM, n0, cpar, b1, b2, b3, p.M);
      } else if constexpr (EPI == EPI_STATS) {
#pragma unroll
        for (int j = 0; j < NT; ++j)
#pragma unroll
          for (int i = 0; i < MT; ++i) {
            float v[4] = {acc[i][j][0], acc[i][j][1], acc[i][j][2], acc[i][j][3]};
            stage_put<BN>(stA, stB, wm, wn, lane, i, j, v);
          }
        stage_flush_stats<BN>(stA, stB, p, Cout, mt * BM, n0, scnt, b1, b2, b3, p.M);
      } else if constexpr (EPI == EPI_STORE_AUX) {
        epilogue_staged_aux<BN>(acc, p, bv, Cout, stA, stB, mt * BM, n0, wm, wn, lane);
      } else if (!RES && p.aux == nullptr && (p.ldc & 7) == 0 && ((uintptr_t)p.C & 15) == 0) {
        epilogue_staged<BN>(acc, p, bv, Cout, stA, stB, mt * BM, n0, wm, wn, lane, p.M);
      } else if (RES && p.aux == nullptr && (RES >= 2 ? !p.res_sc : (p.res_round && p.act == ACT_RELU)) &&
                 ((p.ldc | p.ldr | p.N) & 7) == 0 && (((uintptr_t)p.residual | (uintptr_t)p.C) & 15) == 0) {
        if constexpr (RES)
          epilogue_staged_res<BN, RES >= 2 ? RES - 1 : 0>(acc, p, bv, Cout, Res, stA, stB, mt * BM, n0, wm, wn, lane, p.M);
      } else {
        gemm_epilogue<bf16_t, BM, BN, EPI>(acc, p, red, bv, Cout, Res, mt * BM, n0, wm, wn, lane, mt, mtiles);
      }
      FAST_STAMP(tile, 3);
#pragma unroll
      for (int i = 0; i < MT; ++i)
#pragma unroll
        for (int j = 0; j < NT; ++j) acc[i][j] = f32x4{0.f, 0.f, 0.f, 0.f};
      kt = 0;
      ++tile;
    }
    cur ^= 1;
  }
  if constexpr (EPI == EPI_STATS)
    stats_finish<BN>(p, reinterpret_cast<float*>(smem), scnt, b1, b2, b3, n0, by, bx, gy, (p.M + 127) / 128);
  if constexpr (BWD) {
    if (p.bwd.nred > 0) bwd_finish<2 * BM, BN>(p, reinterpret_cast<float*>(smem), cpar + 4 * BN, b1, b2, b3, n0, by);
  }
}

template <int BM, int BN, int AM, int EPI, int RES, int XF = 0>
__global__ __launch_bounds__(BM * 2) __attribute__((amdgpu_waves_per_eu(EPI == EPI_BWD_AFF && BN == 64 ? 3 : 2)))
void igemm_fast_kernel(GemmParams p) {
  if constexpr (EPI == EPI_BWD_STREAM && BN == 128) {
    bwd_stream128_body<XF>(p);
  } else if constexpr (EPI == EPI_BWD_STREAM) {
    bwd_stream_body<AM, XF>(p);
  } else {
    static_assert(BM == 128, "the persistent engine runs 128-row tiles");
    igemm_fast_body<BN, AM, EPI, RES>(p);
  }
}

static int grid_rows(int M, int N, int z, int BN, int epi) {
  const int nx = (N + BN - 1) / BN, mtiles = (M + 127) / 128;
  const int resident = (BN == 128 || epi == EPI_BWD ? 2 : 3) * 256;
  int gy = resident / (nx * z);
  if (gy >= 8) gy &= ~7;
  if (gy > mtiles) gy = mtiles >= 8 ? (mtiles & ~7) : mtiles;
  if (gy < 1) gy = 1;
  return gy;
}

static int fast_bn_cols(int N) { return (N % 128 == 0 || N > 64 * 3) ? 128 : 64; }

int fast_grid_rows(int M, int N, int z, int epi) { return grid_rows(M, N, z, fast_bn_cols(N), epi); }

static bool bwd_stream_ok(const GemmParams& p) {
  const char* v = getenv("VCG_BWD_STREAM");
  if (v && v[0] == '0') return false;
  const BwdEpi& e = p.bwd;
  const bool dense = p.a.KH == 0 && p.a.GH == 0;
  if (!dense || (p.K != 64 && p.K != 128 && p.K != 256) || p.N % 64 != 0 || p.batch_inner > 0 || p.ldc != p.N || p.a.ld != p.K ||
      !e.res || e.msc || e.sub || bwd_light(p))
    return false;
  if ((e.y && !e.bits) || (e.y2 && !e.y)) return false;
  if ((e.y || e.bits) && e.nred < 2) return false;
  if (e.tsm_T > 0 && e.tsm_fold % 32 != 0) return false;
  if (p.K == 256 && ((e.tsm_T > 0 && e.tsm_fold % 64 != 0) || e.y)) return false;
  if (p.K == 256 && ((uintptr_t)p.b.ptr & 15 || p.b.ld % 8 != 0)) return false;
  if (((uintptr_t)p.C | (uintptr_t)e.res | (uintptr_t)e.y | (uintptr_t)e.y2 | (uintptr_t)p.a.ptr) & 15) return false;
  if (e.res_s > 1 && (p.M % e.hw) != 0) return false;
  if (e.pj > 0) {
    if (e.y || !e.bits || e.pj != 64 || p.K > 128 || ((uintptr_t)e.a2 & 15) || !e.ppart) return false;
    if (((uintptr_t)p.b.ptr & 15) || p.b.ld % 8 != 0) return false;
  }
  return true;
}

static int bwd_stream_tn(const GemmParams& p) {
  const BwdEpi& e = p.bwd;
  const char* v = getenv("VCG_BWD_STREAM");
  if ((v && v[0] == '6') || p.bwd.pj > 0) return 64;
  return p.K == 256 && p.N % 128 == 0 && !e.y && (e.tsm_T <= 0 || e.tsm_fold % 128 == 0) ? 128 : 64;
}

static int bwd_stream_rows(const GemmParams& p) {
  const int nx = p.N / bwd_stream_tn(p), mtiles = (p.M + 63) / 64;
  int gy = 256 / nx;
  if (gy >= 8) gy &= ~7;
  if (gy > mtiles) gy = mtiles >= 8 ? (mtiles & ~7) : mtiles;
  return gy < 1 ? 1 : gy;
}

bool fast_bwd_streams(const GemmParams& p) { return bwd_stream_ok(p); }

int fast_bwd_slots(const GemmParams& p) {
  if (bwd_stream_ok(p)) return bwd_stream_rows(p);
  const int ps = patch_bwd_slots(p);
  if (ps > 0) return ps;
  return fast_grid_rows(p.M, p.N, 1, bwd_light(p) ? EPI_BWD_AFF : EPI_BWD);
}

template <int BN, int AM, int EPI, int RES>
static int launch_fast(const GemmParams& p, int z, hipStream_t s) {
  const int nx = (p.N + BN - 1) / BN;
  const int gy = grid_rows(p.M, p.N, z, BN, EPI);
  dim3 grid(nx * gy, 1, z);
  const int tk = timing_begin(s);
  hipLaunchKernelGGL((igemm_fast_kernel<128, BN, AM, EPI, RES>), grid, dim3(256), 0, s, p);
  if (census_on()) { char t_[96]; snprintf(t_, sizeof(t_), "igemm_fast 128x%d a%d e%d r%d z%d", BN, AM, EPI, RES, z); census_add(t_, p.M, p.N, p.K); }
  timing_end(tk, s, TIMING_FAST_GEMM, 2.0 * p.M * p.N * (double)p.K * z, algorithmic_bytes<AM, EPI, RES>(p, z));
  VCG_LAUNCH_CHECK();
  return VCG_OK;
}

template <int KC, int XF, int TN = 64>
static int launch_bwd_stream(const GemmParams& p, hipStream_t s) {
  const int nx = p.N / TN, gy = bwd_stream_rows(p);
  const int tk = timing_begin(s);
  hipLaunchKernelGGL((igemm_fast_kernel<256, TN, KC, EPI_BWD_STREAM, false, XF>), dim3(nx * gy), dim3(512), 0, s, p);
  if (census_on()) { char t_[96]; snprintf(t_, sizeof(t_), "igemm_fast_stream tn%d xf%d", TN, XF); census_add(t_, p.M, p.N, p.K); }
  const double pj = bwd_stream_pj(XF);
  timing_end(tk, s, TIMING_FAST_GEMM, 2.0 * p.M * p.N * (double)p.K + 2.0 * p.M * p.N * pj,
             algorithmic_bytes<OP_DENSE_K, EPI_BWD, false>(p, 1) + 2.0 * p.M * pj + 4.0 * p.N * pj);
  VCG_LAUNCH_CHECK();
  return VCG_OK;
}

template <int KC>
static int run_bwd_stream(const GemmParams& p, hipStream_t s) {
  if constexpr (KC == 4) {
    if (bwd_stream_tn(p) == 128)
      return p.bwd.bits ? launch_bwd_stream<4, XF_BITS, 128>(p, s) : launch_bwd_stream<4, 0, 128>(p, s);
    return p.bwd.bits ? launch_bwd_stream<4, XF_BITS>(p, s) : launch_bwd_stream<4, 0>(p, s);
  } else {
    if (p.bwd.pj == 64) return launch_bwd_stream<KC, XF_BITS | XF_P64>(p, s);
    if (!p.bwd.y) return p.bwd.bits ? launch_bwd_stream<KC, XF_BITS>(p, s) : launch_bwd_stream<KC, 0>(p, s);
    if (!p.bwd.y2) return launch_bwd_stream<KC, XF_HASY>(p, s);
    return launch_bwd_stream<KC, XF_HASY | XF_Y2>(p, s);
  }
}

template <int AM, int EPI, int RES = 0>
static int fast_bn(const GemmParams& p, int z, hipStream_t s) {
  if (fast_bn_cols(p.N) == 128) return launch_fast<128, AM, EPI, RES>(p, z, s);
  return launch_fast<64, AM, EPI, RES>(p, z, s);
}

int run_fast_gemm(GemmParams& p, int amode, int epi, int z, hipStream_t s) {
  if (p.a.ptr2) {
    if (amode != OP_DENSE_K || epi != EPI_BWD || z != 1 || !bwd_light(p) || p.a.split2 % FBK != 0) return -1;
    return fast_bn<OP_DENSE_K2, EPI_BWD_AFF>(p, z, s);
  }
  if (amode == OP_IM2COL && p.a.tsm_fold > 0) amode = OP_IM2COL_TSM;
  if (amode == OP_IM2COL && p.a.C < FBK) amode = OP_IM2COL_SMALLC;
  if (amode == OP_IM2COL_TSM && p.a.C < FBK) return -1;
  if (amode == OP_DGRAD && p.a.C < FBK) return -1;
  if (z == 1) {
    const int r = run_patch_conv(p, amode, epi, s);
    if (r != -1) return r;
  }
  if (amode != OP_IM2COL_SMALLC && gemm256_ok(p, amode, epi, z)) return run_gemm256(p, amode, epi, s);
  if (epi == EPI_BWD && amode == OP_DENSE_K && z == 1 && bwd_stream_ok(p))
    return p.K == 64 ? run_bwd_stream<1>(p, s) : p.K == 128 ? run_bwd_stream<2>(p, s) : run_bwd_stream<4>(p, s);
  if (epi == EPI_BWD && bwd_light(p)) {
    if (amode == OP_DGRAD) return fast_bn<OP_DGRAD, EPI_BWD_AFF>(p, z, s);
    if (amode == OP_DENSE_K) return fast_bn<OP_DENSE_K, EPI_BWD_AFF>(p, z, s);
    return -1;
  }
  if (epi == EPI_BWD) {
    if (amode == OP_DGRAD) return fast_bn<OP_DGRAD, EPI_BWD>(p, z, s);
    if (amode == OP_DENSE_K) return fast_bn<OP_DENSE_K, EPI_BWD>(p, z, s);
    return -1;
  }
  if (epi == EPI_STATS) {
    if (amode == OP_IM2COL_SMALLC) return fast_bn<OP_IM2COL_SMALLC, EPI_STATS>(p, z, s);
    if (amode == OP_IM2COL_TSM) return fast_bn<OP_IM2COL_TSM, EPI_STATS>(p, z, s);
    if (amode == OP_IM2COL) return fast_bn<OP_IM2COL, EPI_STATS>(p, z, s);
    if (amode == OP_DGRAD) return fast_bn<OP_DGRAD, EPI_STATS>(p, z, s);
    return fast_bn<OP_DENSE_K, EPI_STATS>(p, z, s);
  }
  if (p.residual) return p.act == ACT_GELU_BWD        ? fast_bn<OP_DENSE_K, EPI_STORE, 2>(p, z, s)
                         : p.act == ACT_GELU_TANH_BWD ? fast_bn<OP_DENSE_K, EPI_STORE, 3>(p, z, s)
                                                      : fast_bn<OP_DENSE_K, EPI_STORE, 1>(p, z, s);
  if (p.aux && amode == OP_DENSE_K && (p.ldc & 7) == 0)
    return fast_bn<OP_DENSE_K, EPI_STORE_AUX>(p, z, s);
  if (amode == OP_IM2COL_SMALLC) return fast_bn<OP_IM2COL_SMALLC, EPI_STORE>(p, z, s);
  if (amode == OP_IM2COL_TSM) return fast_bn<OP_IM2COL_TSM, EPI_STORE>(p, z, s);
  if (amode == OP_IM2COL) return fast_bn<OP_IM2COL, EPI_STORE>(p, z, s);
  if (amode == OP_DGRAD) return fast_bn<OP_DGRAD, EPI_STORE>(p, z, s);
  return fast_bn<OP_DENSE_K, EPI_STORE>(p, z, s);
}

}

VCG_API int vcg_fast_stamps(unsigned long long* out, int n) {
#ifdef VCG_FAST_STAMPS
  n = n < 64 * 4 ? n : 64 * 4;
  return hipMemcpyFromSymbol(out, HIP_SYMBOL(vcg::g_fast_stamps), (size_t)n * 8, 0, hipMemcpyDeviceToHost) == hipSuccess
             ? 0 : 2;
#else
  (void)out;
  (void)n;
  return 1;
#endif
}
```

### video-chapter-generation_amd/csrc/stream1x1.hip

```cpp
#include "igemm.h"
#include "mfma_util.h"

namespace vcg {
namespace {

constexpr int RS_NTH = 512;
constexpr int RS_TN = 256;

__device__ __forceinline__ int rswz(int row, int chunk) { return chunk ^ ((row >> 1) & 7); }

__device__ __forceinline__ s16x8 rs_bfrag(const bf16_t* Bkt, int r0, int lane, int s2) {
  const int g = lane >> 4, i = lane & 15;
  const int row = r0 + i;
  const uint32_t addr = lds_u32(Bkt + row * 64 + 8 * rswz(row, 4 * s2 + g));
  s16x8 v;
  asm volatile("ds_read_b128 %0, %1" : "=v"(v) : "v"(addr) : "memory");
  return v;
}

__device__ __forceinline__ int rs_col(int p, int g) { return 32 * p + 16 * (g & 1) + 8 * (g >> 1); }

template <int K> struct RsTile {
  uint4 a[K / 32];
  uint4 r[RS_TN / 32];
};

template <int K>
__device__ __forceinline__ void rs_load(RsTile<K>& t, const bf16_t* __restrict__ X, const bf16_t* __restrict__ R,
                                        long long tile, long long M, int N, int n0, int lane) {
  const int g = lane >> 4, i = lane & 15;
  long long m = tile * 16 + i;
  m = m < M ? m : M - 1;
#pragma unroll
  for (int s = 0; s < K / 32; ++s) t.a[s] = *reinterpret_cast<const uint4*>(X + m * K + 32 * s + 8 * g);
#pragma unroll
  for (int p = 0; p < RS_TN / 32; ++p) t.r[p] = *reinterpret_cast<const uint4*>(R + m * N + n0 + rs_col(p, g));
}

template <int K>
__device__ __forceinline__ void rs_compute(const RsTile<K>& t, const bf16_t* Bs, const float* bias_s,
                                           bf16_t* __restrict__ out, uint8_t* __restrict__ bits, long long tile,
                                           long long M, int N, int n0, int lane) {
  constexpr int NJ = RS_TN / 16, JG = 4;
  const int g = lane >> 4, i = lane & 15;
  const long long m = tile * 16 + i;
  const bool ok = m < M;
  uint32_t mb[2] = {0u, 0u};
#pragma unroll
  for (int j0 = 0; j0 < NJ; j0 += JG) {
    f32x4 acc[JG];
#pragma unroll
    for (int jj = 0; jj < JG; ++jj) acc[jj] = f32x4{0.f, 0.f, 0.f, 0.f};
#pragma unroll
    for (int s = 0; s < K / 32; ++s) {
      const s16x8 af = __builtin_bit_cast(s16x8, t.a[s]);
      const bf16_t* Bkt = Bs + (s >> 1) * RS_TN * 64;
      s16x8 bf[JG];
#pragma unroll
      for (int jj = 0; jj < JG; ++jj) bf[jj] = rs_bfrag(Bkt, 16 * (j0 + jj), lane, s & 1);
      asm volatile("s_waitcnt lgkmcnt(0)" ::: "memory");
      __builtin_amdgcn_sched_barrier(0);
#pragma unroll
      for (int jj = 0; jj < JG; ++jj) acc[jj] = __builtin_amdgcn_mfma_f32_16x16x32_bf16(bf[jj], af, acc[jj], 0, 0, 0);
    }
#pragma unroll
    for (int pp = 0; pp < JG / 2; ++pp) {
      const int p = j0 / 2 + pp;
      uint32_t vw[2][2];
#pragma unroll
      for (int h = 0; h < 2; ++h) {
        const int jj = 2 * pp + h, j = j0 + jj;
        const float4 bv = *reinterpret_cast<const float4*>(bias_s + 16 * j + 4 * g);
        vw[h][0] = (uint32_t)f2bf(acc[jj][0] + bv.x) | ((uint32_t)f2bf(acc[jj][1] + bv.y) << 16);
        vw[h][1] = (uint32_t)f2bf(acc[jj][2] + bv.z) | ((uint32_t)f2bf(acc[jj][3] + bv.w) << 16);
      }
#pragma unroll
      for (int d = 0; d < 2; ++d) {
        const auto sw = __builtin_amdgcn_permlane16_swap(vw[0][d], vw[1][d], false, false);
        vw[0][d] = sw[0];
        vw[1][d] = sw[1];
      }
      const uint4 cv = make_uint4(vw[0][0], vw[0][1], vw[1][0], vw[1][1]);
      float a8[8], r8[8];
      unpack8(cv, a8);
      unpack8(t.r[p], r8);
      uint32_t byte = 0;
#pragma unroll
      for (int e = 0; e < 8; ++e) {
        a8[e] = fmaxf(a8[e] + r8[e], 0.f);
        byte |= (a8[e] > 0.f ? 1u : 0u) << e;
      }
      const uint4 o = pack8(a8);
      if (ok) *reinterpret_cast<uint4*>(out + m * N + n0 + rs_col(p, g)) = o;
      mb[p >> 2] |= byte << (8 * (p & 3));
    }
  }
  uint32_t gm[4][2];
#pragma unroll
  for (int w = 0; w < 2; ++w) {
    gm[0][w] = mb[w];
    gm[1][w] = (uint32_t)__shfl_xor((int)mb[w], 16);
    gm[2][w] = (uint32_t)__shfl_xor((int)mb[w], 32);
    gm[3][w] = (uint32_t)__shfl_xor((int)mb[w], 48);
  }
  if (g == 0 && ok) {
    uint32_t row[8];
#pragma unroll
    for (int p = 0; p < 8; ++p) {
      const int w = p >> 2, sh = 8 * (p & 3);
      row[p] = ((gm[0][w] >> sh) & 0xffu) | (((gm[2][w] >> sh) & 0xffu) << 8) | (((gm[1][w] >> sh) & 0xffu) << 16) |
               (((gm[3][w] >> sh) & 0xffu) << 24);
    }
    uint8_t* bp = bits + ((m * N + n0) >> 3);
    *reinterpret_cast<uint4*>(bp) = make_uint4(row[0], row[1], row[2], row[3]);
    *reinterpret_cast<uint4*>(bp + 16) = make_uint4(row[4], row[5], row[6], row[7]);
  }
}

template <int K>
__global__ __launch_bounds__(RS_NTH) void rs1x1_bnres_kernel(const bf16_t* __restrict__ X, const bf16_t* __restrict__ W,
                                                            const float* __restrict__ bias,
                                                            const bf16_t* __restrict__ R, bf16_t* __restrict__ out,
                                                            uint8_t* __restrict__ bits, long long M, int N) {
  __shared__ __attribute__((aligned(1024))) bf16_t Bs[RS_TN * K];
  __shared__ __attribute__((aligned(16))) float bias_s[RS_TN];
  const int ncb = N / RS_TN;
  const int cb = blockIdx.x % ncb, q = blockIdx.x / ncb, nq = gridDim.x / ncb;
  const int n0 = cb * RS_TN;
  const int tid = threadIdx.x, lane = tid & 63, wave = tid >> 6;
  for (int c = tid; c < RS_TN * K / 8; c += RS_NTH) {
    const int row = c / (K / 8), ch = c % (K / 8);
    const uint4 v = *reinterpret_cast<const uint4*>(W + (long long)(n0 + row) * K + 8 * ch);
    *reinterpret_cast<uint4*>(Bs + (ch >> 3) * RS_TN * 64 + row * 64 + 8 * rswz(row, ch & 7)) = v;
  }
  for (int c = tid; c < RS_TN; c += RS_NTH) bias_s[c] = bias[n0 + c];
  __syncthreads();
  const long long ntiles = (M + 15) / 16;
  const long long stride = (long long)nq * (RS_NTH / 64);
  long long t = (long long)q * (RS_NTH / 64) + wave;
  if (t >= ntiles) return;
  const long long last = ntiles - 1;
  RsTile<K> T0, T1;
  rs_load<K>(T0, X, R, t, M, N, n0, lane);
  for (; t < ntiles; t += 2 * stride) {
    rs_load<K>(T1, X, R, min(t + stride, last), M, N, n0, lane);
    rs_compute<K>(T0, Bs, bias_s, out, bits, t, M, N, n0, lane);
    if (t + stride >= ntiles) break;
    rs_load<K>(T0, X, R, min(t + 2 * stride, last), M, N, n0, lane);
    rs_compute<K>(T1, Bs, bias_s, out, bits, t + stride, M, N, n0, lane);
  }
}

int rs_grid(int N) {
  int dev = 0, cus = 256;
  if (hipGetDevice(&dev) == hipSuccess) (void)hipDeviceGetAttribute(&cus, hipDeviceAttributeMultiprocessorCount, dev);
  const int ncb = N / RS_TN;
  return (cus / ncb) * ncb;
}

}

int run_rs1x1_bnres(const void* x, const void* wfold, const float* bias, const void* res, void* out, uint8_t* bits,
                    long long M, int N, int K, hipStream_t s) {
  const char* e = getenv("VCG_RS1X1");
  if ((e && e[0] == '0') || (K != 64 && K != 128 && K != 256) || N % RS_TN != 0 || N / RS_TN > 8 || M <= 0) return -1;
  const int g = rs_grid(N);
  if (census_on()) { char t_[96]; snprintf(t_, sizeof(t_), "rs1x1_bnres"); census_add(t_, M, N, K); }
  if (K == 64)
    hipLaunchKernelGGL(rs1x1_bnres_kernel<64>, dim3(g), dim3(RS_NTH), 0, s, (const bf16_t*)x, (const bf16_t*)wfold,
                       bias, (const bf16_t*)res, (bf16_t*)out, bits, M, N);
  else if (K == 128)
    hipLaunchKernelGGL(rs1x1_bnres_kernel<128>, dim3(g), dim3(RS_NTH), 0, s, (const bf16_t*)x, (const bf16_t*)wfold,
                       bias, (const bf16_t*)res, (bf16_t*)out, bits, M, N);
  else
    hipLaunchKernelGGL(rs1x1_bnres_kernel<256>, dim3(g), dim3(RS_NTH), 0, s, (const bf16_t*)x, (const bf16_t*)wfold,
                       bias, (const bf16_t*)res, (bf16_t*)out, bits, M, N);
  VCG_LAUNCH_CHECK();
  return VCG_OK;
}

}
```

### video-chapter-generation_amd/vcg_hip/ops.py

```python
import os

import torch

from . import _lib

F32, BF16 = 0, 1
ACT_NONE, ACT_RELU, ACT_GELU, ACT_TANH, ACT_GELU_BWD = 0, 1, 2, 3, 4
ACT_GELU_TANH, ACT_GELU_TANH_BWD = 5, 6
ATTN_CAUSAL = 1
ACT_FLAG_ROUND_PRE = 0x100
ACT_FLAG_WIDE = 0x200
ACT_FLAG_F32_OUT = 0x400
GRAD_F32 = 0x10

_DT = {torch.float32: F32, torch.bfloat16: BF16}


def dt_code(dtype):
    try:
        return _DT[dtype]
    except KeyError:
        raise TypeError(f"unsupported storage dtype {dtype}; expected float32 or bfloat16")


def torch_dtype(precision):
    return {"fp32": torch.float32, "bf16": torch.bfloat16}[precision]


def stream():
    return torch.cuda.current_stream().cuda_stream


def P(t):
    if t is None:
        return None
    if not t.is_cuda:
        raise RuntimeError("libvcg_hip ops need GPU tensors (no CPU fallback)")
    return t.data_ptr()


def _chk(t, dtype=None, name="tensor"):
    if not t.is_cuda:
        raise RuntimeError(f"{name} must be on the GPU (libvcg_hip has no CPU path)")
    if not t.is_contiguous():
        raise RuntimeError(f"{name} must be contiguous")
    if dtype is not None and t.dtype != dtype:
        raise RuntimeError(f"{name} has dtype {t.dtype}, expected {dtype}")


def ws(nbytes, device):
    return torch.empty((max(int(nbytes), 4) + 3) // 4, dtype=torch.float32, device=device)


def conv_out_hw(H, W, KH, KW, stride, pad):
    return (H + 2 * pad - KH) // stride + 1, (W + 2 * pad - KW) // stride + 1


TIMING_FAST_GEMM, TIMING_WGRAD, TIMING_GENERIC_GEMM, TIMING_PATCH_CONV, TIMING_WIDE_GEMM = 0, 1, 2, 3, 4


def gemm_census_enable(on):
    _lib.call("vcg_gemm_census_enable", int(bool(on)))


def gemm_census():
    import ctypes
    out = {}
    for i in range(_lib.query("vcg_gemm_census_size")):
        buf = ctypes.create_string_buffer(256)
        n = ctypes.c_longlong()
        _lib.call("vcg_gemm_census_get", i, buf, 256, ctypes.addressof(n))
        out[buf.value.decode()] = n.value
    return out


def timing_enable(on):
    _lib.call("vcg_timing_enable", int(bool(on)))


def timing_query(kernel_id):
    import ctypes
    ms, n, fl = ctypes.c_double(), ctypes.c_longlong(), ctypes.c_double()
    _lib.call("vcg_timing_query", int(kernel_id), ctypes.addressof(ms), ctypes.addressof(n), ctypes.addressof(fl))
    return ms.value, n.value, fl.value


def timing_roofline(kernel_id, peak_tflops, peak_gbs):
    import ctypes
    ms, ideal, nb, fl = ctypes.c_double(), ctypes.c_double(), ctypes.c_double(), ctypes.c_double()
    _lib.call("vcg_timing_roofline", int(kernel_id), float(peak_tflops), float(peak_gbs), ctypes.addressof(ms),
              ctypes.addressof(ideal), ctypes.addressof(nb), ctypes.addressof(fl))
    return ms.value, ideal.value, nb.value, fl.value


def stats_tiles(M):
    return _lib.query("vcg_conv_stats_tiles", M)


def stats_buffer(Cout, M, device):
    return torch.empty((Cout + 1, stats_tiles(M), 2), dtype=torch.float32, device=device)


def conv_fwd(x, w, N, H, W, C, Cout, KH, KW, stride, pad, tsm_T=0, tsm_fold=0, stats=None, out=None):
    _chk(x, name="x")
    if stats is not None:
        OH_, OW_ = conv_out_hw(H, W, KH, KW, stride, pad)
        if stats.numel() < (Cout + 1) * stats_tiles(N * OH_ * OW_) * 2:
            raise ValueError("stats buffer too small: use ops.stats_buffer(Cout, M)")
    _chk(w, x.dtype, "w")
    OH, OW = conv_out_hw(H, W, KH, KW, stride, pad)
    y = out if out is not None else torch.empty((N, OH, OW, Cout), dtype=x.dtype, device=x.device)
    _lib.call("vcg_conv_fwd", dt_code(x.dtype), P(x), P(w), P(y), P(stats), N, H, W, C, Cout, KH, KW, stride, pad,
              tsm_T, tsm_fold, stream())
    return y


def conv_fwd_bias_act(x, w, bias, act, N, H, W, C, Cout, KH, KW, stride, pad, tsm_T=0, tsm_fold=0, out=None):
    _chk(x, name="x")
    _chk(w, x.dtype, "w")
    _chk(bias, torch.float32, "bias")
    OH, OW = conv_out_hw(H, W, KH, KW, stride, pad)
    y = out if out is not None else torch.empty((N, OH, OW, Cout), dtype=x.dtype, device=x.device)
    _lib.call("vcg_conv_fwd_bias_act", dt_code(x.dtype), P(x), P(w), P(bias), int(act), P(y), N, H, W, C, Cout, KH,
              KW, stride, pad, tsm_T, tsm_fold, stream())
    return y


def conv_dgrad(dy, wt, N, H, W, C, Cout, KH, KW, stride, pad, out=None):
    _chk(dy, name="dy")
    _chk(wt, dy.dtype, "wt")
    dx = out if out is not None else torch.empty((N, H, W, C), dtype=dy.dtype, device=dy.device)
    _lib.call("vcg_conv_dgrad", dt_code(dy.dtype), P(dy), P(wt), P(dx), N, H, W, C, Cout, KH, KW, stride, pad,
              stream())
    return dx


def conv_dgrad_bwd(dy, wt, N, H, W, C, Cout, KH, KW, stride, pad, tsm_T=0, tsm_fold=0, res=None, res_stride=1,
                   bits=None, y=None, mean=None, invstd=None, mscale=None, mshift=None, y2=None, mean2=None, invstd2=None, sums=None,
                   sum_gx2=None, dgamma=None, dbeta=None, dgamma2=None, dbeta2=None, out=None, workspace=None, a2=None,
                   pg=None):
    OH, OW = conv_out_hw(H, W, KH, KW, stride, pad)
    _chk(dy, None, "dy")
    assert dy.numel() == N * OH * OW * Cout and wt.numel() == C * KH * KW * Cout
    g = out if out is not None else torch.empty((N, H, W, C), dtype=dy.dtype, device=dy.device)
    nbytes = _lib.query("vcg_conv_dgrad_bwd_ws_bytes", C, Cout, KH, KW)
    if workspace is None or workspace.numel() * 4 < nbytes:
        workspace = ws(nbytes, dy.device)
    for t in (res, y, y2):
        if t is not None:
            _chk(t, dy.dtype)
            assert t.numel() == (N * ((H + 1) // 2) * ((W + 1) // 2) * C if t is res and res_stride == 2
                                 else N * H * W * C)
    def call(a2_, pg_, pws_):
        return _lib.query("vcg_conv_dgrad_bwd", dt_code(dy.dtype), P(dy), P(wt), P(g), N, H, W, C, Cout, KH, KW,
                          stride, pad, tsm_T, tsm_fold, P(res), int(res_stride), P(bits), P(y), P(mean), P(invstd),
                          P(mscale), P(mshift), P(y2), P(mean2), P(invstd2), P(workspace), workspace.numel() * 4,
                          P(sums[0]) if sums is not None else None, P(sums[1]) if sums is not None else None,
                          P(dgamma), P(dbeta), P(sum_gx2), P(dgamma2), P(dbeta2), P(a2_),
                          a2_.shape[-1] if a2_ is not None else 0, P(pg_), P(pws_),
                          pws_.numel() * 4 if pws_ is not None else 0, stream())
    done = False
    rc = -2
    if a2 is not None:
        _chk(a2, torch.bfloat16, "a2")
        _chk(pg, torch.float32, "pg")
        assert a2.numel() == N * H * W * a2.shape[-1] and pg.numel() == C * a2.shape[-1]
        pws = ws(_lib.query("vcg_conv_dgrad_bwd_p_ws_bytes", C, a2.shape[-1]), dy.device)
        rc = call(a2, pg, pws)
        done = rc == 0
    if rc == -2:
        rc = call(None, None, None)
    if rc == -2:
        return (None, False) if a2 is not None else None
    if rc != 0:
        raise _lib.VcgError(f"vcg_conv_dgrad_bwd failed ({rc}): {_lib.last_error()}")
    return (g, done) if a2 is not None else g


def bn_apply_colsum(y, scale, shift, C, relu=True):
    _chk(y, torch.bfloat16, "y")
    out = torch.empty_like(y)
    cs = torch.empty(C, dtype=torch.float32, device=y.device)
    P_ = y.numel() // C
    w = ws(_lib.query("vcg_bn_apply_colsum_ws_bytes", P_, C), y.device)
    _lib.call("vcg_bn_apply_colsum", P(y), P(scale), P(shift), int(relu), P(out), P(cs), P(w), w.numel() * 4, P_, C,
              stream())
    return out, cs


def bn_apply_gram(y, scale, shift, C, mean, invstd):
    _chk(y, torch.bfloat16, "y")
    out = torch.empty_like(y)
    cs = torch.empty(C, dtype=torch.float32, device=y.device)
    gram = torch.empty((C, C), dtype=torch.float32, device=y.device)
    g64 = torch.empty(C * C + 2 * C, dtype=torch.float64, device=y.device)
    P_ = y.numel() // C
    w = ws(_lib.query("vcg_bn_apply_gram_ws_bytes", P_, C), y.device)
    _lib.call("vcg_bn_apply_gram", P(y), P(scale), P(shift), P(mean), P(invstd), P(out), P(cs), P(gram), P(g64),
              P(w), w.numel() * 4, P_, C, stream())
    return out, cs, gram, g64


def bn_stats_from_gram(g64, w, M, N, C, stats):
    _chk(w, torch.bfloat16, "w")
    _chk(g64, torch.float64, "g64")
    assert g64.numel() == C * C + 2 * C
    _lib.call("vcg_bn_stats_from_gram", P(g64), P(w), M, N, C, P(stats), stats.shape[1], stream())
    return stats


def bn_finalize_from_gram(g64, w, M, N, C, gamma, beta, mean, invstd, scale, shift, running_mean=None,
                          running_var=None, momentum=0.1, eps=1e-5, w32=None, wfold=None):
    _chk(w, torch.bfloat16, "w")
    _chk(g64, torch.float64, "g64")
    assert g64.numel() == C * C + 2 * C and C <= 256 and C % 16 == 0
    if w32 is not None:
        _chk(w32, torch.float32, "w32")
        _chk(wfold, torch.bfloat16, "wfold")
        assert w32.numel() == N * C and wfold.numel() == N * C
    _lib.call("vcg_bn_finalize_from_gram", P(g64), P(w), M, N, C, P(gamma), P(beta), P(mean), P(invstd), P(scale),
              P(shift), P(running_mean), P(running_var), float(momentum), float(eps), P(w32), P(wfold), stream())


def conv1x1_stats(x, w, stats, M, N, K):
    _chk(x, torch.bfloat16, "x")
    _chk(w, torch.bfloat16, "w")
    rc = _lib.query("vcg_conv1x1_stats", P(x), P(w), P(stats), M, N, K, stream())
    if rc == -2:
        return False
    if rc != 0:
        raise _lib.VcgError(f"vcg_conv1x1_stats failed ({rc}): {_lib.last_error()}")
    return True


def bn_bwd_sumgx_from_wgrad(Pg, w, K, C, mean, invstd, sum_g, sum_gx, dgamma=None):
    _chk(Pg, torch.float32, "Pg")
    _chk(w, torch.bfloat16, "w")
    _lib.call("vcg_bn_bwd_sumgx_from_wgrad", P(Pg), P(w), K, C, P(mean), P(invstd), P(sum_g), P(sum_gx), P(dgamma),
              stream())


def conv1x1_bn_res_relu(x, wfold, bias, res, M, N, K, res_scale=None, res_shift=None):
    _chk(x, torch.bfloat16, "x")
    _chk(res, torch.bfloat16, "res")
    out = torch.empty_like(res)
    bits = torch.empty(res.numel() // 8, dtype=torch.uint8, device=res.device)
    rc = _lib.query("vcg_conv1x1_bn_res_relu", P(x), P(wfold), P(bias), P(res), P(res_scale), P(res_shift), P(out),
                    P(bits), M, N, K, stream())
    if rc == -2:
        return None
    if rc != 0:
        raise _lib.VcgError(f"vcg_conv1x1_bn_res_relu failed ({rc}): {_lib.last_error()}")
    return out, bits


def bn_bwd_fold_weights(wt, N, K, mean, invstd, gamma, sum_g, sum_gx, count):
    _chk(wt, torch.bfloat16, "wt")
    wfold = torch.empty((N, 2 * K), dtype=torch.bfloat16, device=wt.device)
    bias = torch.empty(N, dtype=torch.float32, device=wt.device)
    _lib.call("vcg_bn_bwd_fold_weights", P(wt), N, K, P(mean), P(invstd), P(gamma), P(sum_g), P(sum_gx),
              float(1.0 / count), P(wfold), P(bias), stream())
    return wfold, bias


def conv_dgrad_bwd_bnfold(g, yg, wfold, bias, N, H, W, C, Cout, y=None, mean=None, invstd=None, mscale=None,
                          mshift=None, sums=None, dgamma=None, dbeta=None, out=None, workspace=None, Ky=None):
    Ky = Cout if Ky is None else Ky
    _chk(g, torch.bfloat16, "g")
    _chk(yg, torch.bfloat16, "yg")
    assert g.numel() == N * H * W * Cout and yg.numel() == N * H * W * Ky and wfold.numel() == C * (Cout + Ky)
    gout = out if out is not None else torch.empty((N, H, W, C), dtype=g.dtype, device=g.device)
    nbytes = _lib.query("vcg_conv_dgrad_bwd_ws_bytes", C, Cout + Ky, 1, 1)
    if workspace is None or workspace.numel() * 4 < nbytes:
        workspace = ws(nbytes, g.device)
    rc = _lib.query("vcg_conv_dgrad_bwd_bnfold", P(g), P(yg), int(Ky), P(wfold), P(bias), P(gout), N, H, W, C, Cout, P(y),
                    P(mean), P(invstd), P(mscale), P(mshift), P(workspace), workspace.numel() * 4,
                    P(sums[0]) if sums is not None else None, P(sums[1]) if sums is not None else None, P(dgamma),
                    P(dbeta), stream())
    if rc == -2:
        return None
    if rc != 0:
        raise _lib.VcgError(f"vcg_conv_dgrad_bwd_bnfold failed ({rc}): {_lib.last_error()}")
    return gout


def bn_bwd_fold_weights_a2(wt, C, K, invstd, gamma, sum_g, sum_gx, count, colsum_a):
    _chk(wt, torch.bfloat16, "wt")
    wfold = torch.empty((C, K + C), dtype=torch.bfloat16, device=wt.device)
    bias = torch.empty(C, dtype=torch.float32, device=wt.device)
    _lib.call("vcg_bn_bwd_fold_weights_a2", P(wt), C, K, P(invstd), P(gamma), P(sum_g), P(sum_gx), float(1.0 / count),
              P(colsum_a), P(wfold), P(bias), stream())
    return wfold, bias


def bn_bwd_fold_wgrad_a2(Pg, G, w3, K, C, mean, invstd, gamma, sum_g, sum_gx, count, colsum_a, dw, accumulate=True):
    for t, n in ((Pg, "Pg"), (G, "G"), (w3, "w3"), (dw, "dw")):
        _chk(t, torch.float32, n)
    _lib.call("vcg_bn_bwd_fold_wgrad_a2", P(Pg), P(G), P(w3), K, C, P(mean), P(invstd), P(gamma), P(sum_g), P(sum_gx),
              float(1.0 / count), P(colsum_a), P(dw), int(accumulate), stream())


def conv_wgrad_bnfold(x, g, yg, mean, invstd, gamma, sum_g, sum_gx, count, colsum_x, dw, N, H, W, C, Cout,
                      accumulate=True, workspace=None):
    _chk(x, torch.bfloat16, "x")
    _chk(dw, torch.float32, "dw")
    nbytes = _lib.query("vcg_conv_wgrad_bnfold_ws_bytes", N, H, W, C, Cout)
    if workspace is None or workspace.numel() * 4 < nbytes:
        workspace = ws(nbytes, x.device)
    rc = _lib.query("vcg_conv_wgrad_bnfold", P(x), P(g), P(yg), P(mean), P(invstd), P(gamma), P(sum_g), P(sum_gx),
                    float(1.0 / count), P(colsum_x), P(dw), int(accumulate), P(workspace), workspace.numel() * 4, N, H,
                    W, C, Cout, stream())
    if rc == -2:
        return False
    if rc != 0:
        raise _lib.VcgError(f"vcg_conv_wgrad_bnfold failed ({rc}): {_lib.last_error()}")
    return True


def conv_wgrad(x, dy, dw, N, H, W, C, Cin, Cout, KH, KW, stride, pad, tsm_T=0, tsm_fold=0, accumulate=True,
               workspace=None):
    _chk(x, name="x")
    _chk(dy, x.dtype, "dy")
    _chk(dw, torch.float32, "dw")
    nbytes = _lib.query("vcg_conv_wgrad_ws_bytes", dt_code(x.dtype), N, H, W, C, Cout, KH, KW, stride, pad)
    if workspace is None or workspace.numel() * 4 < nbytes:
        workspace = ws(nbytes, x.device)
    _lib.call("vcg_conv_wgrad", dt_code(x.dtype), P(x), P(dy), P(dw), int(accumulate), P(workspace),
              workspace.numel() * 4, N, H, W, C, Cin, Cout, KH, KW, stride, pad, tsm_T, tsm_fold, stream())
    return workspace


def conv_wgrad_ws_bytes(dtype, N, H, W, C, Cout, KH, KW, stride, pad):
    return _lib.query("vcg_conv_wgrad_ws_bytes", dt_code(dtype), N, H, W, C, Cout, KH, KW, stride, pad)


def gemm(A, B, M, N, K, lda, ldb, transA=False, transB=False, out=None, ldc=None, bias=None, act=ACT_NONE,
         residual=None, ldr=None, aux=None, alpha=1.0):
    if out is None:
        out = torch.empty((M, N), dtype=A.dtype, device=A.device)
        ldc = N
    ldc = ldc if ldc is not None else N
    _lib.call("vcg_gemm", dt_code(A.dtype), int(transA), int(transB), M, N, K, P(A), lda, P(B), ldb, P(out), ldc,
              P(bias), act, P(residual), ldr if ldr is not None else ldc, P(aux), float(alpha), stream())
    return out


def gemm_batched(A, B, C, M, N, K, lda, ldb, ldc, a_so, a_si, b_so, b_si, c_so, c_si, batch_outer, batch_inner,
                 transA=False, transB=False, bias=None, act=ACT_NONE, alpha=1.0):
    _lib.call("vcg_gemm_batched", dt_code(A.dtype), int(transA), int(transB), M, N, K, P(A), lda, a_so, a_si, P(B),
              ldb, b_so, b_si, P(C), ldc, c_so, c_si, batch_outer, batch_inner, P(bias), act, float(alpha), stream())
    return C


def gemm_splitk(A, B, out, M, N, K, lda, ldb, transA=False, transB=False, accumulate=True, workspace=None):
    _chk(out, torch.float32, "out")
    nbytes = _lib.query("vcg_gemm_splitk_ws_bytes", dt_code(A.dtype), M, N, K)
    if workspace is None or workspace.numel() * 4 < nbytes:
        workspace = ws(nbytes, A.device)
    _lib.call("vcg_gemm_splitk", dt_code(A.dtype), int(transA), int(transB), M, N, K, P(A), lda, P(B), ldb, P(out),
              int(accumulate), P(workspace), workspace.numel() * 4, stream())
    return workspace


def bn_finalize(stats, mtiles, M, C, gamma, beta, mean, invstd, scale, shift, running_mean=None, running_var=None,
                momentum=0.1, eps=1e-5):
    _lib.call("vcg_bn_finalize", P(stats), mtiles, M, C, P(gamma), P(beta), P(mean), P(invstd), P(scale), P(shift),
              P(running_mean), P(running_var), float(momentum), float(eps), stream())


def bn_eval_params(gamma, beta, rm, rv, eps, C, mean, invstd, scale, shift):
    _lib.call("vcg_bn_eval_params", P(gamma), P(beta), P(rm), P(rv), float(eps), C, P(mean), P(invstd), P(scale),
              P(shift), stream())


def bn_apply(y, scale, shift, C, relu, res=None, rscale=None, rshift=None, out=None, bits=False):
    out = out if out is not None else torch.empty_like(y)
    b = torch.empty(y.numel() * y.element_size() // 16, dtype=torch.uint8, device=y.device) if bits else None
    _lib.call("vcg_bn_apply", dt_code(y.dtype), P(y), P(scale), P(shift), P(res), P(rscale), P(rshift), int(relu),
              P(out), P(b), y.numel() // C, C, stream())
    return (out, b) if bits else out


def _mask_mode(mask, mbits, mscale):
    if mbits is not None:
        return 2
    if mscale is not None:
        return 3
    return 1 if mask is not None else 0


def bn_bwd_reduce(dout, mask, y, mean, invstd, C, sum_g, sum_gx, dgamma=None, dbeta=None, workspace=None,
                  mbits=None, mscale=None, mshift=None):
    Pn = y.numel() // C
    nbytes = _lib.query("vcg_bn_bwd_ws_bytes", Pn, C)
    if workspace is None or workspace.numel() * 4 < nbytes:
        workspace = ws(nbytes, y.device)
    _lib.call("vcg_bn_bwd_reduce", dt_code(y.dtype), P(dout), _mask_mode(mask, mbits, mscale), P(mask), P(mbits),
              P(mscale), P(mshift), P(y), P(mean), P(invstd), Pn, C, P(workspace), workspace.numel() * 4, P(sum_g),
              P(sum_gx), P(dgamma), P(dbeta), 1, stream())
    return workspace


def bn_bwd_apply(dout, mask, y, mean, invstd, gamma, sum_g, sum_gx, C, train_stats, gout=None, out=None,
                 mbits=None, mscale=None, mshift=None):
    Pn = y.numel() // C
    dy = out if out is not None else torch.empty_like(y)
    _lib.call("vcg_bn_bwd_apply", dt_code(y.dtype), P(dout), _mask_mode(mask, mbits, mscale), P(mask), P(mbits),
              P(mscale), P(mshift), P(y), P(mean), P(invstd), P(gamma), P(sum_g), P(sum_gx), Pn, int(train_stats),
              P(dy), P(gout), Pn, C, stream())
    return dy


def bn_bwd_apply_dual(g, y, mean, invstd, gamma, sum_g, sum_gx, yd, mean_d, invstd_d, gamma_d, sum_g_d, sum_gx_d,
                      C):
    Pn = y.numel() // C
    dy, dyd = torch.empty_like(y), torch.empty_like(yd)
    _lib.call("vcg_bn_bwd_apply_dual", dt_code(y.dtype), P(g), P(y), P(mean), P(invstd), P(gamma), P(sum_g),
              P(sum_gx), P(yd), P(mean_d), P(invstd_d), P(gamma_d), P(sum_g_d), P(sum_gx_d), Pn, P(dy), P(dyd), Pn, C,
              stream())
    return dy, dyd


def maxpool_fwd(x, N, H, W, C):
    OH, OW = (H - 1) // 2 + 1, (W - 1) // 2 + 1
    y = torch.empty((N, OH, OW, C), dtype=x.dtype, device=x.device)
    idx = torch.empty((N, OH, OW, C), dtype=torch.uint8, device=x.device)
    _lib.call("vcg_maxpool_fwd", dt_code(x.dtype), P(x), P(y), P(idx), N, H, W, C, stream())
    return y, idx


def maxpool_bwd(dy, idx, N, H, W, C):
    dx = torch.empty((N, H, W, C), dtype=dy.dtype, device=dy.device)
    _lib.call("vcg_maxpool_bwd", dt_code(dy.dtype), P(dy), P(idx), P(dx), N, H, W, C, stream())
    return dx


def maxpool_bwd_bn(dy, idx, N, H, W, C, y, mean, invstd, mscale, mshift, sums, dgamma=None, dbeta=None,
                   store_g=True):
    g = torch.empty((N, H, W, C), dtype=dy.dtype, device=dy.device) if store_g else None
    w = ws(_lib.query("vcg_maxpool_bwd_bn_ws_bytes", C), dy.device)
    _lib.call("vcg_maxpool_bwd_bn", dt_code(dy.dtype), P(dy), P(idx), P(g), N, H, W, C, P(y), P(mean), P(invstd),
              P(mscale), P(mshift), P(w), w.numel() * 4, P(sums[0]), P(sums[1]), P(dgamma), P(dbeta), stream())
    return g


def maxpool_bwd_bn_sums_pooled(dy, mp, idx, y, N, H, W, C, mean, invstd, mscale, mshift, sums, dgamma=None,
                               dbeta=None):
    OH, OW = (H - 1) // 2 + 1, (W - 1) // 2 + 1
    assert tuple(mp.shape) == (N, OH, OW, C) and idx.shape == mp.shape and tuple(y.shape) == (N, H, W, C)
    w = ws(_lib.query("vcg_maxpool_bwd_bn_ws_bytes", C), dy.device)
    _lib.call("vcg_maxpool_bwd_bn_sums_pooled", dt_code(dy.dtype), P(dy), P(mp), P(idx), P(y), N, H, W, C, P(mean),
              P(invstd), P(mscale), P(mshift), P(w), w.numel() * 4, P(sums[0]), P(sums[1]), P(dgamma), P(dbeta),
              stream())


def maxpool_bwd_bn_apply(dy, idx, N, H, W, C, y, mean, invstd, mscale, mshift, gamma, sums, count, train_stats):
    dx = torch.empty((N, H, W, C), dtype=dy.dtype, device=dy.device)
    _lib.call("vcg_maxpool_bwd_bn_apply", dt_code(dy.dtype), P(dy), P(idx), P(dx), N, H, W, C, P(y), P(mean),
              P(invstd), P(mscale), P(mshift), P(gamma), P(sums[0]), P(sums[1]), int(count), int(bool(train_stats)),
              stream())
    return dx


def stem_bwd_fused(dy, idx, y, x, N, H, W, mean, invstd, mscale, mshift, gamma, sums, count, train_stats, dw,
                   accumulate=True):
    for t, n in ((dy, "dy"), (y, "y"), (x, "x")):
        _chk(t, torch.bfloat16, n)
    _chk(dw, torch.float32, "dw")
    assert tuple(y.shape) == (N, H, W, 64) and tuple(x.shape) == (N, 2 * H, 2 * W, 4) and dw.numel() == 64 * 147
    assert tuple(dy.shape) == (N, (H - 1) // 2 + 1, (W - 1) // 2 + 1, 64) and idx.shape == dy.shape
    w = ws(_lib.query("vcg_stem_bwd_fused_ws_bytes"), dy.device)
    _lib.call("vcg_stem_bwd_fused", P(dy), P(idx), P(y), P(x), N, H, W, P(mean), P(invstd), P(mscale), P(mshift),
              P(gamma), P(sums[0]), P(sums[1]), int(count), int(bool(train_stats)), P(w), w.numel() * 4, P(dw),
              int(bool(accumulate)), stream())


def stem_bwd_fused_fits(N, H, W):
    return bool(_lib.query("vcg_stem_bwd_fused_fits", int(N), int(H), int(W)))


def bn_relu_maxpool(y, scale, shift, N, H, W, C):
    OH, OW = (H - 1) // 2 + 1, (W - 1) // 2 + 1
    out = torch.empty((N, OH, OW, C), dtype=y.dtype, device=y.device)
    idx = torch.empty((N, OH, OW, C), dtype=torch.uint8, device=y.device)
    _lib.call("vcg_bn_relu_maxpool", dt_code(y.dtype), P(y), P(scale), P(shift), P(out), P(idx), N, H, W, C, stream())
    return out, idx


def avgpool_fwd(x, N, HW, C):
    y = torch.empty((N, C), dtype=torch.float32, device=x.device)
    _lib.call("vcg_avgpool_fwd", dt_code(x.dtype), P(x), P(y), N, HW, C, stream())
    return y


def avgpool_bwd(dy, N, HW, C, dtype):
    dx = torch.empty((N, HW, C), dtype=dtype, device=dy.device)
    _lib.call("vcg_avgpool_bwd", dt_code(dtype), P(dy), P(dx), N, HW, C, stream())
    return dx


IMAGENET_MEAN = (0.485, 0.456, 0.406)
IMAGENET_STD = (0.229, 0.224, 0.225)


def stem_cpad(dtype):
    return 4


def window_frames_u8(frames, idx, dtype, mean=IMAGENET_MEAN, std=IMAGENET_STD, cpad=8):
    import ctypes

    _chk(frames, torch.uint8, "frames")
    _chk(idx, torch.int64, "idx")
    F, H, W, C = frames.shape
    if C != 3:
        raise ValueError("frames must be [F,H,W,3] RGB")
    n = idx.numel()
    dst = torch.empty((n, H, W, cpad), dtype=dtype, device=frames.device)
    m = (ctypes.c_float * 3)(*mean)
    sd = (ctypes.c_float * 3)(*std)
    _lib.call("vcg_window_frames_u8_cpad", dt_code(dtype), P(frames), P(idx), P(dst), n, F, H, W, cpad,
              ctypes.addressof(m), ctypes.addressof(sd), stream())
    return dst


def frames_to_nhwc(src, N, C, H, W, Cpad, dtype):
    _chk(src, torch.float32, "frames")
    dst = torch.empty((N, H, W, Cpad), dtype=dtype, device=src.device)
    _lib.call("vcg_frames_to_nhwc", dt_code(dtype), P(src), P(dst), N, C, H, W, Cpad, stream())
    return dst


def pair_taps(KW, pad):
    lo = (-pad) // 2
    return (KW - 1 - pad) // 2 - lo + 1, -lo


def weight_prep(w, Cpad, dtype, transposed=False, out=None, pair_pad=None):
    _chk(w, torch.float32, "weight")
    Cout, Cin, KH, KW = w.shape
    mode = int(transposed)
    if pair_pad is not None:
        shape, mode = (Cout, KH, pair_taps(KW, pair_pad)[0], 8), 2 + pair_pad
    else:
        shape = (Cin, KH, KW, Cout) if transposed else (Cout, KH, KW, Cpad)
    out = out if out is not None else torch.empty(shape, dtype=dtype, device=w.device)
    _lib.call("vcg_weight_prep", dt_code(dtype), P(w), P(out), Cout, Cin, KH, KW, Cpad, mode, stream())
    return out


def weight_fold(w2d, scale, dtype, out=None):
    _chk(w2d, torch.float32, "weight")
    rows, cols = w2d.shape
    out = out if out is not None else torch.empty((rows, cols), dtype=dtype, device=w2d.device)
    _lib.call("vcg_weight_fold", dt_code(dtype), P(w2d), P(scale), P(out), rows, cols, stream())
    return out
# ... 721 lines not shown
```

### video-chapter-generation_amd/vcg_hip/trunk.py

```python
import os

import torch

from . import ops


def bn_mode(bn):
    has_running = bn.running_mean is not None and bn.running_var is not None
    if bn.training:
        return "train" if (bn.track_running_stats and has_running) else "batch"
    return "running" if has_running else "batch"


class BNState:
    __slots__ = ("vec", "mean", "invstd", "scale", "shift", "mode", "count", "bn")

    def __init__(self, C, device, mode, count, bn):
        self.vec = torch.empty((4, C), dtype=torch.float32, device=device)
        self.mean, self.invstd, self.scale, self.shift = self.vec[0], self.vec[1], self.vec[2], self.vec[3]
        self.mode = mode
        self.count = count
        self.bn = bn


_WSTREAMS = {}


def _conv_shape(conv):
    KH, KW = conv.kernel_size
    return conv.out_channels, conv.in_channels, KH, KW, conv.stride[0], conv.padding[0]


def _tsm_info(conv1, Cin):
    if hasattr(conv1, "net") and hasattr(conv1, "n_segment"):
        return conv1.net, conv1.n_segment, Cin // conv1.fold_div
    return conv1, 0, 0


class _ConvWeights:

    def __init__(self, net, flat, stem_cpad):
        self.flat = flat
        self.gen = None
        convs = [m for m in net.modules() if isinstance(m, torch.nn.Conv2d)]
        dev = convs[0].weight.device
        self.fwd, self.bwd = {}, {}
        desc = []
        self.stem_cpad = stem_cpad
        for conv in convs:
            Cout, Cin, KH, KW = conv.weight.shape
            stem = conv is net.conv1
            cpad = stem_cpad if stem else Cin
            if stem and cpad == 4:
                pad = conv.padding[1]
                wf = torch.empty((Cout, KH, ops.pair_taps(KW, pad)[0], 8), dtype=torch.bfloat16, device=dev)
                mode = 2 + pad
            else:
                wf = torch.empty((Cout, KH, KW, cpad), dtype=torch.bfloat16, device=dev)
                mode = 0
            self.fwd[id(conv)] = wf
            desc.append([conv.weight.data_ptr(), wf.data_ptr(), Cout, Cin, KH, KW, cpad, mode])
            if not stem:
                wb = torch.empty((Cin, KH, KW, Cout), dtype=torch.bfloat16, device=dev)
                self.bwd[id(conv)] = wb
                desc.append([conv.weight.data_ptr(), wb.data_ptr(), Cout, Cin, KH, KW, Cin, 1])
        self.desc = torch.tensor(desc, dtype=torch.int64).to(dev)
        self.n = len(desc)
        self.ptrs = [conv.weight.data_ptr() for conv in convs]
        self.convs = convs

    def valid_for(self, net, flat, stem_cpad):
        return (flat is self.flat and stem_cpad == self.stem_cpad
                and [c.weight.data_ptr() for c in self.convs] == self.ptrs)

    def refresh(self):
        if self.gen == self.flat.generation:
            return
        self.gen = self.flat.generation
        ops.weight_prep_multi(self.desc, self.n)


class ResNetTrunk:
    staged = False
    path_counts = {"fused": 0, "unfused": 0}
    census = None
    fused_bwd = True
    wgrad_stream = True
    ds_stream = True
    dual_bn_bwd = True
    fold_eval = True
    bn_fold_bwd = True
    bn_fold_max_c3 = 1024
    bn_fold_a2 = True
    y3_drop = True
    bn3_gemm_max_c3 = 1024
    gram_stats = True
    pooled_stem_sums = True
    fused_stem_bwd = True
    dgrad_p = True
    gram_fin = True

    def __init__(self, net, dtype):
        self.net = net
        self.dtype = dtype
        self._ws = None
        self._pending = []
        self.wc = None
        flat = getattr(net, "_vcg_flat", None)
        if dtype == torch.bfloat16 and flat is not None:
            wc = getattr(net, "_vcg_convw", None)
            if wc is None or not wc.valid_for(net, flat, ops.stem_cpad(dtype)):
                wc = _ConvWeights(net, flat, ops.stem_cpad(dtype))
                object.__setattr__(net, "_vcg_convw", wc)
            wc.refresh()
            self.wc = wc

    def _wprep(self, conv, Cpad):
        if self.wc is not None:
            return self.wc.fwd[id(conv)]
        pair = self.dtype == torch.bfloat16 and Cpad == 4
        return ops.weight_prep(conv.weight.data, Cpad, self.dtype, pair_pad=conv.padding[1] if pair else None)

    def _wprep_t(self, conv, Cin):
        if self.wc is not None:
            return self.wc.bwd[id(conv)]
        return ops.weight_prep(conv.weight.data, Cin, self.dtype, transposed=True)

    def _drop_y3(self, blk, planes, need_grad):
        C3 = blk.conv3.out_channels
        if not need_grad:
            return (ResNetTrunk.y3_drop and blk.downsample is None and self.dtype == torch.bfloat16
                    and C3 <= ResNetTrunk.bn3_gemm_max_c3 and C3 % 64 == 0
                    and planes % 64 == 0 and blk.conv3.stride[0] == 1 and bn_mode(blk.bn3) != "running")
        if blk is self.net.layer4[-1]:
            return False
        return (ResNetTrunk.y3_drop and need_grad and blk.downsample is None and ResNetTrunk.bn_fold_bwd
                and ResNetTrunk.bn_fold_a2 and ResNetTrunk.fused_bwd and self.dtype == torch.bfloat16
                and C3 <= ResNetTrunk.bn_fold_max_c3
                and C3 <= ResNetTrunk.bn3_gemm_max_c3 and C3 % 128 == 0 and planes >= 64
                and (planes & (planes - 1)) == 0 and blk.conv3.stride[0] == 1 and bn_mode(blk.bn3) != "running")

    def _conv_bn(self, x, conv, bn, N, H, W, C, tsm_T=0, tsm_fold=0, store=True):
        Cout, _, KH, KW, s, p = _conv_shape(conv)
        OH, OW = ops.conv_out_hw(H, W, KH, KW, s, p)
        M = N * OH * OW
        mode = bn_mode(bn)
        st = BNState(Cout, x.device, mode, M, bn)
        w = self._wprep(conv, C)
        if mode == "running":
            y = ops.conv_fwd(x, w, N, H, W, C, Cout, KH, KW, s, p, tsm_T, tsm_fold)
            ops.bn_eval_params(bn.weight, bn.bias, bn.running_mean, bn.running_var, bn.eps, Cout, st.mean, st.invstd,
                               st.scale, st.shift)
        else:
            mt = ops.stats_tiles(M)
            stats = ops.stats_buffer(Cout, M, x.device)
            y = None
            if store or (KH, KW, s, p, tsm_fold) != (1, 1, 1, 0, 0) or not ops.conv1x1_stats(x.view(M, C), w, stats,
                                                                                               M, Cout, C):
                y = ops.conv_fwd(x, w, N, H, W, C, Cout, KH, KW, s, p, tsm_T, tsm_fold, stats=stats)
            self._finalize(stats, mt, M, Cout, bn, st)
        return y, st, OH, OW

    @staticmethod
    def _finalize(stats, mt, M, Cout, bn, st):
        upd = st.mode == "train"
        mom = bn.momentum if bn.momentum is not None else 0.1
        ops.bn_finalize(stats, mt, M, Cout, bn.weight, bn.bias, st.mean, st.invstd, st.scale, st.shift,
                        bn.running_mean if upd else None, bn.running_var if upd else None, mom, bn.eps)

    def _bn_from_gram(self, conv, bn, g64, M, C, fold=False):
        Cout = conv.out_channels
        st = BNState(Cout, g64.device, bn_mode(bn), M, bn)
        w = self._wprep(conv, C).view(Cout, C)
        if ResNetTrunk.gram_fin and C <= 256 and C % 16 == 0:
            upd = st.mode == "train"
            w32 = conv.weight.data.view(Cout, C) if fold else None
            wf = torch.empty((Cout, C), dtype=torch.bfloat16, device=g64.device) if fold else None
            ops.bn_finalize_from_gram(g64, w, M, Cout, C, bn.weight, bn.bias, st.mean, st.invstd, st.scale, st.shift,
                                      bn.running_mean if upd else None, bn.running_var if upd else None,
                                      bn.momentum if bn.momentum is not None else 0.1, bn.eps, w32, wf)
            return st, wf
        stats = ops.stats_buffer(Cout, M, g64.device)
        ops.bn_stats_from_gram(g64, w, M, Cout, C, stats)
        self._finalize(stats, stats.shape[1], M, Cout, bn, st)
        return st, None

    def forward(self, x, need_grad):
        net, dt = self.net, self.dtype
        if self.staged:
            N, H, W, cpad = x.shape
            if x.dtype != dt or cpad != ops.stem_cpad(dt) or not x.is_contiguous():
                raise RuntimeError(f"staged frames must be contiguous NHWC [N,H,W,{ops.stem_cpad(dt)}] {dt}, "
                                   f"got {x.dtype} {tuple(x.shape)}")
            xs = x
        else:
            N, C0, H, W = x.shape
            cpad = ops.stem_cpad(dt)
            xs = ops.frames_to_nhwc(x.contiguous(), N, C0, H, W, cpad, dt)
        y0, b0, H1, W1 = self._conv_bn(xs, net.conv1, net.bn1, N, H, W, cpad)
        mp, idx = ops.bn_relu_maxpool(y0, b0.scale, b0.shift, N, H1, W1, 64)
        Hm, Wm = mp.shape[1], mp.shape[2]
        saved = {"stem": (xs, y0, mp, idx, b0, N, H, W, cpad, H1, W1)} if need_grad else None
        if not need_grad:
            del y0, idx
        h, Hc, Wc = mp, Hm, Wm
        self._fold_gen = None
        if ResNetTrunk.fold_eval and not need_grad and dt == torch.bfloat16:
            key = self._fold_key()
            old = getattr(net, "_vcg_fold_key", None)
            if old is None or old[0] != key:
                object.__setattr__(net, "_vcg_fold_key", (key, object()))
            self._fold_gen = net._vcg_fold_key[1]
        blocks = []
        for layer in (net.layer1, net.layer2, net.layer3, net.layer4):
            for blk in layer:
                h, rec, Hc, Wc = self._block_fwd(blk, h, N, Hc, Wc, need_grad)
                if need_grad:
                    blocks.append(rec)
        emb = ops.avgpool_fwd(h, N, Hc * Wc, h.shape[-1])
        if need_grad:
            saved["blocks"] = blocks
            saved["final"] = (N, Hc, Wc, h.shape[-1])
        return emb, saved

    def _block_fwd(self, blk, x, N, H, W, need_grad):
        Cin = x.shape[-1]
        conv1, T, fold = _tsm_info(blk.conv1, Cin)
        planes = conv1.out_channels
        if self._foldable(blk, x, need_grad):
            return self._block_fwd_folded(blk, x, conv1, T, fold, N, H, W)
        yd = bd = side = None
        cur = torch.cuda.current_stream() if x.is_cuda else None
        if blk.downsample is not None:
            side = self._wside(x.device) if self.ds_stream else None
            if side is not None:
                side.wait_stream(cur)
                with torch.cuda.stream(side):
                    yd, bd, _, _ = self._conv_bn(x, blk.downsample[0], blk.downsample[1], N, H, W, Cin)
                yd.record_stream(cur)
                bd.vec.record_stream(cur)
        y1, b1, _, _ = self._conv_bn(x, conv1, blk.bn1, N, H, W, Cin, T, fold)
        a1 = ops.bn_apply(y1, b1.scale, b1.shift, planes, relu=True)
        y2, b2, H2, W2 = self._conv_bn(a1, blk.conv2, blk.bn2, N, H, W, planes)
        drop = self._drop_y3(blk, planes, need_grad)
        C3 = blk.conv3.out_channels
        a2sum = a2gram = g64 = None
        fold_a2 = (need_grad and ResNetTrunk.bn_fold_bwd and ResNetTrunk.bn_fold_a2 and ResNetTrunk.fused_bwd
                   and self.dtype == torch.bfloat16 and bn_mode(blk.bn3) != "running"
                   and C3 <= ResNetTrunk.bn_fold_max_c3 and planes <= 2048)
        if (fold_a2 or drop) and ResNetTrunk.gram_stats and planes in (64, 128, 256) and bn_mode(blk.bn3) != "running":
            a2, a2sum, a2gram, g64 = ops.bn_apply_gram(y2, b2.scale, b2.shift, planes, b2.mean, b2.invstd)
        elif fold_a2:
            a2, a2sum = ops.bn_apply_colsum(y2, b2.scale, b2.shift, planes)
        else:
            a2 = ops.bn_apply(y2, b2.scale, b2.shift, planes, relu=True)
        wf = None
        if drop and a2gram is not None:
            b3, wf = self._bn_from_gram(blk.conv3, blk.bn3, g64, N * H2 * W2, planes,
                                        fold=self.dtype == torch.bfloat16 and C3 <= ResNetTrunk.bn3_gemm_max_c3)
            y3 = None
        else:
            y3, b3, _, _ = self._conv_bn(a2, blk.conv3, blk.bn3, N, H2, W2, planes, store=not drop)
        if not fold_a2:
            a2sum = a2gram = None
        r2 = None
        if blk.downsample is not None:
            if side is not None:
                cur.wait_stream(side)
            else:
                yd, bd, _, _ = self._conv_bn(x, blk.downsample[0], blk.downsample[1], N, H, W, Cin)
            out, obits = ops.bn_apply(y3, b3.scale, b3.shift, C3, relu=True, res=yd, rscale=bd.scale,
                                      rshift=bd.shift, bits=True)
        else:
            if (self.dtype == torch.bfloat16 and C3 <= ResNetTrunk.bn3_gemm_max_c3
                    and b3.mode != "running" and blk.conv3.stride[0] == 1):
                M = N * H2 * W2
                if wf is None:
                    wf = ops.weight_fold(blk.conv3.weight.data.view(C3, planes), b3.scale, self.dtype)
                r2 = ops.conv1x1_bn_res_relu(a2.view(M, planes), wf, b3.shift, x, M, C3, planes)
            if r2 is not None:
                out, obits = r2
            else:
                if y3 is None:
                    y3 = self._conv3_out(blk, a2, N, H2, W2, planes)
                out, obits = ops.bn_apply(y3, b3.scale, b3.shift, C3, relu=True, res=x, bits=True)
        if ResNetTrunk.census is not None:
            ResNetTrunk.census.append(("fwd", C3, blk.downsample is not None,
                                       {"a2sum": a2sum is not None, "y3_drop": y3 is None, "bn3_gemm": r2 is not None}))
        rec = None
        if need_grad:
            rec = dict(blk=blk, x=x, y1=y1, a1=a1, y2=y2, a2=a2, a2sum=a2sum, a2gram=a2gram, y3=y3, yd=yd, obits=obits, b1=b1, b2=b2, b3=b3,
                       bd=bd, N=N, H=H, W=W, H2=H2, W2=W2, Cin=Cin, planes=planes, C3=C3, T=T, fold=fold,
                       conv1=conv1)
        return out, rec, H2, W2

    def _conv3_out(self, blk, a2, N, H2, W2, planes):
        C3 = blk.conv3.out_channels
        return ops.conv_fwd(a2, self._wprep(blk.conv3, planes), N, H2, W2, planes, C3, 1, 1, 1, 0)

    def _y3(self, r):
        if r["y3"] is None:
            r["y3"] = self._conv3_out(r["blk"], r["a2"], r["N"], r["H2"], r["W2"], r["planes"])
        return r["y3"]

    def _foldable(self, blk, x, need_grad):
        if not (ResNetTrunk.fold_eval and not need_grad and self.dtype == torch.bfloat16 and x.is_cuda):
            return False
        bns = [blk.bn1, blk.bn2, blk.bn3] + ([blk.downsample[1]] if blk.downsample is not None else [])
        return all(bn_mode(b) == "running" for b in bns) and _conv_shape(blk.conv3)[2:] == (1, 1, 1, 0)

    def _fold_key(self):
        flat = getattr(self.net, "_vcg_flat", None)
        v = 0
        for m in self.net.modules():
            if isinstance(m, torch.nn.BatchNorm2d):
                for t in (m.weight, m.bias, m.running_mean, m.running_var, m.num_batches_tracked):
                    if t is not None:
                        v += t._version
        return (flat.generation if flat is not None else None, v)

    def _fold(self, conv, bn, Cpad):
        cache = self._fold_cache
        ent = cache.get(id(conv))
        if ent is None:
            ent = cache[id(conv)] = self._fold_new(conv, bn, Cpad)
        return ent

    def _fold_new(self, conv, bn, Cpad):
        Cout, Cin, KH, KW, _, _ = _conv_shape(conv)
        st = BNState(Cout, conv.weight.device, "running", 0, bn)
        ops.bn_eval_params(bn.weight, bn.bias, bn.running_mean, bn.running_var, bn.eps, Cout, st.mean, st.invstd,
                           st.scale, st.shift)
        w2 = conv.weight.data.view(Cout, Cin * KH * KW)
        if KH == KW == 1 and Cpad == Cin:
            return ops.weight_fold(w2, st.scale, self.dtype), st.shift
        wf = ops.weight_fold(w2, st.scale, torch.float32).view(Cout, Cin, KH, KW)
        return ops.weight_prep(wf, Cpad, self.dtype), st.shift

    @property
    def _fold_cache(self):
        c = getattr(self.net, "_vcg_fold_cache", None)
        if c is None or c[0] is not self._fold_gen:
            c = (self._fold_gen, {})
            object.__setattr__(self.net, "_vcg_fold_cache", c)
        return c[1]

    def _block_fwd_folded(self, blk, x, conv1, T, fold, N, H, W):
        Cin = x.shape[-1]
        planes = conv1.out_channels
        w1, c1 = self._fold(conv1, blk.bn1, Cin)
        a1 = ops.conv_fwd_bias_act(x, w1, c1, ops.ACT_RELU, N, H, W, Cin, planes, 1, 1, 1, 0, T, fold)
        _, _, KH, KW, s, p = _conv_shape(blk.conv2)
        w2, c2 = self._fold(blk.conv2, blk.bn2, planes)
        a2 = ops.conv_fwd_bias_act(a1, w2, c2, ops.ACT_RELU, N, H, W, planes, planes, KH, KW, s, p)
        H2, W2 = a2.shape[1], a2.shape[2]
        C3 = blk.conv3.out_channels
        if blk.downsample is not None:
            cd = blk.downsample[0]
            Cd, _, KHd, KWd, sd, pd = _conv_shape(cd)
            wd, bd = self._fold(cd, blk.downsample[1], Cin)
            res = ops.conv_fwd_bias_act(x, wd, bd, ops.ACT_NONE, N, H, W, Cin, Cd, KHd, KWd, sd, pd)
        else:
            res = x
        w3, c3 = self._fold(blk.conv3, blk.bn3, planes)
        M = N * H2 * W2
        out = ops.gemm(a2.view(M, planes), w3, M, C3, planes, planes, planes, bias=c3,
                       act=ops.ACT_RELU | ops.ACT_FLAG_ROUND_PRE, residual=res.view(M, C3), ldr=C3)
        return out.view(N, H2, W2, C3), None, H2, W2

    def _bn_bwd(self, dout, y, st, C, mbits=None, affine=False):
        bn = st.bn
        dev = y.device
        sums = torch.empty((2, C), dtype=torch.float32, device=dev)
        need_affine = bn.weight is not None and bn.weight.requires_grad
        msc, msh = (st.scale, st.shift) if affine else (None, None)
        ops.bn_bwd_reduce(dout, None, y, st.mean, st.invstd, C, sums[0], sums[1],
                          bn.weight.grad if need_affine else None, bn.bias.grad if need_affine else None,
                          mbits=mbits, mscale=msc, mshift=msh)
        return ops.bn_bwd_apply(dout, None, y, st.mean, st.invstd, bn.weight, sums[0], sums[1], C,
                                train_stats=st.mode != "running", mbits=mbits, mscale=msc, mshift=msh)

    def _wside(self, dev):
        if not (ResNetTrunk.fused_bwd and self.dtype == torch.bfloat16 and dev.type == "cuda"):
            return None
        key = dev.index if dev.index is not None else torch.cuda.current_device()
        st = _WSTREAMS.get(key)
        if st is None:
            st = _WSTREAMS[key] = torch.cuda.Stream(device=dev)
        return st

    def _async(self, fn, *tensors):
        ws = self._ws
        if ws is None:
            return fn()
        ws.wait_stream(torch.cuda.current_stream())
        with torch.cuda.stream(ws):
            out = fn()
        self._hold(tensors)
        return out

    def _hold(self, tensors):
        ev = torch.cuda.Event()
        ev.record(self._ws)
        self._pending.append((ev, [t for t in tensors if t is not None]))
        while self._pending and self._pending[0][0].query():
            self._pending.pop(0)

    def _report(self, hooks, params):
        if hooks is None:
            return
        if self._ws is None:
            return hooks(params)
        self._ws.wait_stream(torch.cuda.current_stream())
        with torch.cuda.stream(self._ws):
            hooks(params)

    def _ds_dgrad_side(self, cds, dyd, N, H, W, Cin, C3):
        ws, cur = self._ws, torch.cuda.current_stream()
        ws.wait_stream(cur)
        with torch.cuda.stream(ws):
            if cds.stride[0] == 2:
                wt_ds = self._wprep_t(cds, Cin)
                Mo = dyd.numel() // C3
                res, res_stride = ops.gemm(dyd.view(Mo, C3), wt_ds.view(Cin, C3), Mo, Cin, C3, C3, C3,
                                           act=ops.ACT_FLAG_WIDE), 2
            else:
                res, res_stride = self._dgrad(cds, dyd, N, H, W), 1
            ev = torch.cuda.Event()
            ev.record(ws)
        self._hold((dyd,))
        res.record_stream(cur)
        return res, res_stride, ev

    def _wgrad(self, conv, x, dy, N, H, W, Cpad, T=0, fold=0):
        if not conv.weight.requires_grad:
            return
        Cout, Cin, KH, KW, s, p = _conv_shape(conv)
        self._async(lambda: ops.conv_wgrad(x, dy, conv.weight.grad, N, H, W, Cpad, Cin, Cout, KH, KW, s, p, T, fold,
                                           accumulate=True), x, dy)

    def _dgrad(self, conv, dy, N, H, W):
        Cout, Cin, KH, KW, s, p = _conv_shape(conv)
        wt = self._wprep_t(conv, Cin)
        return ops.conv_dgrad(dy, wt, N, H, W, Cin, Cout, KH, KW, s, p)

    def backward(self, d_emb, saved, hooks=None):
        N, Hc, Wc, C = saved["final"]
        self._ws = self._wside(d_emb.device) if ResNetTrunk.wgrad_stream else None
        dout = ops.avgpool_bwd(d_emb.contiguous(), N, Hc * Wc, C, self.dtype).view(N, Hc, Wc, C)
        blocks = saved["blocks"]
        gin = None
        while blocks:
            rec = blocks.pop()
            prev = blocks[-1] if blocks else None
            dout, gin = self._block_bwd(rec, dout, gin, prev)
            self._report(hooks, list(rec["blk"].parameters()))
            del rec
        xs, y0, mp, idx, b0, N, H, W, cpad, H1, W1 = saved["stem"]
        sums0 = torch.zeros((2, 64), dtype=torch.float32, device=y0.device)
        dg0, db0 = self._bn_grads(b0)
        if ResNetTrunk.pooled_stem_sums:
            ops.maxpool_bwd_bn_sums_pooled(dout, mp, idx, y0, N, H1, W1, 64, b0.mean, b0.invstd, b0.scale, b0.shift,
                                           sums0, dg0, db0)
        else:
            ops.maxpool_bwd_bn(dout, idx, N, H1, W1, 64, y0, b0.mean, b0.invstd, b0.scale, b0.shift, sums0, dg0, db0,
                               store_g=False)
        conv1 = self.net.conv1
        if self._stem_fused_ok(conv1, xs, N, H, W, cpad, H1, W1):
            ops.stem_bwd_fused(dout, idx, y0, xs, N, H1, W1, b0.mean, b0.invstd, b0.scale, b0.shift, b0.bn.weight,
                               sums0, N * H1 * W1, b0.mode != "running", conv1.weight.grad)
        else:
            dy0 = ops.maxpool_bwd_bn_apply(dout, idx, N, H1, W1, 64, y0, b0.mean, b0.invstd, b0.scale, b0.shift,
                                           b0.bn.weight, sums0, N * H1 * W1, b0.mode != "running")
            self._wgrad(conv1, xs, dy0, N, H, W, cpad)
        self._report(hooks, list(self.net.conv1.parameters()) + list(self.net.bn1.parameters()))
        if self._ws is not None:
            torch.cuda.current_stream().wait_stream(self._ws)
            self._pending.clear()

    def _stem_fused_ok(self, conv1, xs, N, H, W, cpad, H1, W1):
        w = conv1.weight
        return (ResNetTrunk.fused_stem_bwd and self.dtype == torch.bfloat16 and cpad == 4 and w.requires_grad
                and w.grad is not None and tuple(w.shape) == (64, 3, 7, 7) and conv1.stride == (2, 2)
                and conv1.padding == (3, 3) and H == 2 * H1 and W == 2 * W1 and H1 % 2 == 0 and W1 % 8 == 0
                and W1 <= 112 and ops.stem_bwd_fused_fits(N, H1, W1))

    def _bn_grads(self, st):
        bn = st.bn
        if bn.weight is not None and bn.weight.requires_grad:
            return bn.weight.grad, bn.bias.grad
        return None, None

    def _bn_apply_bwd(self, g, y, st, C, sums):
        return ops.bn_bwd_apply(g, None, y, st.mean, st.invstd, st.bn.weight, sums[0], sums[1], C,
                                train_stats=st.mode != "running")

    def _dgrad_bn(self, conv, dy, N, H, W, y, st, C):
        Cout, Cin, KH, KW, s, p = _conv_shape(conv)
        wt = self._wprep_t(conv, Cin)
        sums = torch.empty((2, C), dtype=torch.float32, device=y.device)
        dg, db = self._bn_grads(st)
        g = None
        if ResNetTrunk.fused_bwd:
            g = ops.conv_dgrad_bwd(dy, wt, N, H, W, Cin, Cout, KH, KW, s, p, y=y, mean=st.mean, invstd=st.invstd,
                                   mscale=st.scale, mshift=st.shift, sums=sums, dgamma=dg, dbeta=db)
        ResNetTrunk.path_counts["unfused" if g is None else "fused"] += 1
        if g is None:
            da = ops.conv_dgrad(dy, wt, N, H, W, Cin, Cout, KH, KW, s, p)
            return self._bn_bwd(da, y, st, C, affine=True)
        return self._bn_apply_bwd(g, y, st, C, sums)

    def _can_fold(self, r, ds):
        blk, b3, C3, planes = r["blk"], r["b3"], r["C3"], r["planes"]
        if not (ResNetTrunk.bn_fold_bwd and ResNetTrunk.fused_bwd and self.dtype == torch.bfloat16):
            return False
        if b3.mode == "running" or r["a2"] is None or C3 > ResNetTrunk.bn_fold_max_c3 or C3 % 128 != 0:
            return False
        if blk.conv3.stride[0] != 1 or planes < 64 or (planes & (planes - 1)) != 0:
            return False
        return not ds or r["bd"].mode != "running"

    def _fold_conv3(self, r, g, sums3):
        blk = r["blk"]
        if not blk.conv3.weight.requires_grad:
            return True
        N, H2, W2, planes, C3 = r["N"], r["H2"], r["W2"], r["planes"], r["C3"]
        b3, a2, y3 = r["b3"], r["a2"], r["y3"]
        M = N * H2 * W2

        a2s = r.get("a2sum")
        if a2s is not None:
            Pg0 = r.get("Pg")

            G0 = r.get("a2gram")

            def wfn():
                G = G0
                if G is None:
                    G = torch.empty((planes, planes, 1, 1), dtype=torch.float32, device=a2.device)
                    ops.conv_wgrad(a2, a2, G, N, H2, W2, planes, planes, planes, 1, 1, 1, 0, accumulate=False)
                Pg = Pg0
                if Pg is None:
                    Pg = torch.empty((C3, planes, 1, 1), dtype=torch.float32, device=a2.device)
                    ops.conv_wgrad(a2, g, Pg, N, H2, W2, planes, planes, C3, 1, 1, 1, 0, accumulate=False)
                ops.bn_bwd_fold_wgrad_a2(Pg.view(C3, planes), G.view(planes, planes),
                                         blk.conv3.weight.data.view(C3, planes), C3, planes, b3.mean, b3.invstd,
                                         b3.bn.weight, sums3[0], sums3[1], M, a2s,
                                         blk.conv3.weight.grad.view(C3, planes))
                return True
            return self._async(wfn, a2, g, sums3, a2s, Pg0, G0, b3.vec)

        def wfn():
            cs = torch.empty(planes, dtype=torch.float32, device=a2.device)
            ops.colsum(a2.view(M, planes), planes, M, planes, cs, accumulate=False)
            return ops.conv_wgrad_bnfold(a2, g, y3, b3.mean, b3.invstd, b3.bn.weight, sums3[0], sums3[1], M, cs,
                                         blk.conv3.weight.grad, N, H2, W2, planes, C3)
        return self._async(wfn, a2, g, y3, sums3, b3.vec)

    def _dgrad_bn_fold(self, conv, g, y3, b3, sums3, N, H, W, y, st, C, C3, a2=None, a2sum=None):
        Cout, Cin, KH, KW, s, p = _conv_shape(conv)
        wt = self._wprep_t(conv, Cin)
        M = N * H * W
        if a2sum is not None:
            wfold, bias = ops.bn_bwd_fold_weights_a2(wt.view(Cin, C3), Cin, C3, b3.invstd, b3.bn.weight, sums3[0],
                                                     sums3[1], M, a2sum)
            src, Ky = a2, Cin
        else:
            wfold, bias = ops.bn_bwd_fold_weights(wt.view(Cin, C3), Cin, C3, b3.mean, b3.invstd, b3.bn.weight,
                                                  sums3[0], sums3[1], M)
            src, Ky = y3, C3
        sums = torch.empty((2, C), dtype=torch.float32, device=y.device)
        dg, db = self._bn_grads(st)
        g2 = ops.conv_dgrad_bwd_bnfold(g, src, wfold, bias, N, H, W, Cin, C3, y=y, mean=st.mean, invstd=st.invstd,
                                       mscale=st.scale, mshift=st.shift, sums=sums, dgamma=dg, dbeta=db, Ky=Ky)
        if g2 is None:
            return None
        ResNetTrunk.path_counts["fused"] += 1
        return self._bn_apply_bwd(g2, y, st, C, sums)

    def _block_bwd(self, r, dout, gin, prev):
        blk = r["blk"]
        N, H, W, H2, W2 = r["N"], r["H"], r["W"], r["H2"], r["W2"]
        Cin, planes, C3, T, fold = r["Cin"], r["planes"], r["C3"], r["T"], r["fold"]
        obits = r["obits"]
        ds = blk.downsample is not None
        bnf = None
        if gin is not None:
            g, sums3, sumsd = gin
            b3, bd = r["b3"], r.get("bd")
            if r["y3"] is None and not ds:
                Pg = r.get("Pg")
                if Pg is None:
                    Pg = torch.empty((C3, planes, 1, 1), dtype=torch.float32, device=g.device)
                    ops.conv_wgrad(r["a2"], g, Pg, N, H2, W2, planes, planes, C3, 1, 1, 1, 0, accumulate=False)
                ops.bn_bwd_sumgx_from_wgrad(Pg.view(C3, planes), self._wprep(blk.conv3, planes), C3, planes, b3.mean,
                                            b3.invstd, sums3[0], sums3[1], self._bn_grads(b3)[0])
                r["Pg"] = Pg
            if self._can_fold(r, ds):
                bnf = (g, sums3)
                dy3 = dyd = None
                if ds:
                    def dyd_fn():
                        return self._bn_apply_bwd(g, r["yd"], bd, C3, sumsd)
                    if self._ws is not None and self.ds_stream:
                        dyd = self._async(dyd_fn, g, r["yd"], bd.vec, *sumsd)
                    else:
                        dyd = dyd_fn()
            elif ResNetTrunk.dual_bn_bwd and ds and b3.mode != "running" and bd.mode != "running":
                dy3, dyd = ops.bn_bwd_apply_dual(g, r["y3"], b3.mean, b3.invstd, b3.bn.weight, sums3[0], sums3[1],
                                                 r["yd"], bd.mean, bd.invstd, bd.bn.weight, sumsd[0], sumsd[1], C3)
            else:
                dy3 = self._bn_apply_bwd(g, self._y3(r), b3, C3, sums3)
                dyd = self._bn_apply_bwd(g, r["yd"], bd, C3, sumsd) if ds else None
        else:
            g = torch.empty_like(dout)
            dy3 = self._bn_bwd_g(dout, self._y3(r), r["b3"], C3, obits, g)
            dyd = self._bn_bwd(dout, r["yd"], r["bd"], C3, mbits=obits) if ds else None
        ds_res = None
        if ds and self._ws is not None and self.ds_stream:
            ds_res = self._ds_dgrad_side(blk.downsample[0], dyd, N, H, W, Cin, C3)
        if bnf is not None and not self._fold_conv3(r, *bnf):
            dy3 = self._bn_apply_bwd(bnf[0], self._y3(r), r["b3"], C3, bnf[1])
            bnf = None
        if bnf is None:
            self._wgrad(blk.conv3, r["a2"], dy3, N, H2, W2, planes)
        dy2 = None
        if bnf is not None:
            dy2 = self._dgrad_bn_fold(blk.conv3, bnf[0], r["y3"], r["b3"], bnf[1], N, H2, W2, r["y2"], r["b2"], planes,
                                      C3, a2=r["a2"], a2sum=r.get("a2sum"))
            if dy2 is None:
                dy3 = self._bn_apply_bwd(bnf[0], self._y3(r), r["b3"], C3, bnf[1])
        if ResNetTrunk.census is not None:
            ResNetTrunk.census.append(("bwd", C3, ds, {"fold_wgrad": bnf is not None, "fold_dgrad": dy2 is not None,
                                                       "p_dgrad": bool(r.get("Pg_dgrad")),
                                                       "a2_form": bnf is not None and r.get("a2sum") is not None}))
        if dy2 is None:
            dy2 = self._dgrad_bn(blk.conv3, dy3, N, H2, W2, r["y2"], r["b2"], planes)
        del dy3
        self._wgrad(blk.conv2, r["a1"], dy2, N, H, W, planes)
        dy1 = self._dgrad_bn(blk.conv2, dy2, N, H, W, r["y1"], r["b1"], planes)
        del dy2
        self._wgrad(r["conv1"], r["x"], dy1, N, H, W, Cin, T, fold)
        res_stride = 1
        if ds and ds_res is not None:
            self._wgrad(blk.downsample[0], r["x"], dyd, N, H, W, Cin)
            res, res_stride, ev = ds_res
            torch.cuda.current_stream().wait_event(ev)
        elif ds:
            cds = blk.downsample[0]
            self._wgrad(cds, r["x"], dyd, N, H, W, Cin)
            if cds.stride[0] == 2 and self.dtype == torch.bfloat16 and ResNetTrunk.fused_bwd:
                wt_ds = self._wprep_t(cds, Cin)
                Mo = dyd.numel() // C3
                res = ops.gemm(dyd.view(Mo, C3), wt_ds.view(Cin, C3), Mo, Cin, C3, C3, C3, act=ops.ACT_FLAG_WIDE)
                res_stride = 2
            else:
                res = self._dgrad(cds, dyd, N, H, W)
        else:
            res = g
        conv1 = r["conv1"]
        Cout1, Cin1, KH, KW, s, p = _conv_shape(conv1)
        wt = self._wprep_t(conv1, Cin1)
        kw = dict(tsm_T=T if fold else 0, tsm_fold=fold, res=res, res_stride=res_stride)
        sums3 = sumsd = None
        if prev is not None:
            s3 = torch.empty((3 if prev["blk"].downsample is not None else 2, Cin), dtype=torch.float32,
                             device=dy1.device)
            sums3 = s3[:2]
            dg, db = self._bn_grads(prev["b3"])
            kw.update(bits=prev["obits"], y=prev["y3"], mean=prev["b3"].mean, invstd=prev["b3"].invstd, sums=sums3,
                      dgamma=dg, dbeta=db)
            if prev["blk"].downsample is not None:
                sumsd = (s3[0], s3[2])
                dg2, db2 = self._bn_grads(prev["bd"])
                kw.update(y2=prev["yd"], mean2=prev["bd"].mean, invstd2=prev["bd"].invstd, sum_gx2=s3[2],
                          dgamma2=dg2, dbeta2=db2)
        pg = None
        if (ResNetTrunk.fused_bwd and ResNetTrunk.dgrad_p and prev is not None and prev["y3"] is None
                and prev["blk"].downsample is None and prev["a2"] is not None and prev["planes"] == 64
                and prev["a2"].numel() == N * H * W * prev["planes"]):
            pg = torch.empty((Cin1, prev["planes"], 1, 1), dtype=torch.float32, device=dy1.device)
            out, done = ops.conv_dgrad_bwd(dy1, wt, N, H, W, Cin1, Cout1, KH, KW, s, p, a2=prev["a2"],
                                           pg=pg.view(Cin1, prev["planes"]), **kw)
            if done:
                prev["Pg"] = pg
                prev["Pg_dgrad"] = True
        else:
            out = ops.conv_dgrad_bwd(dy1, wt, N, H, W, Cin1, Cout1, KH, KW, s, p, **kw) if ResNetTrunk.fused_bwd else None
        ResNetTrunk.path_counts["unfused" if out is None else "fused"] += 1
        if ds:
            if out is None and res_stride == 2:
                res = self._dgrad(blk.downsample[0], dyd, N, H, W)
            del dyd
        if out is not None:
            if prev is None:
                return out, None
            return None, (out, sums3, sumsd)
        dxs = ops.conv_dgrad(dy1, wt, N, H, W, Cin1, Cout1, KH, KW, s, p)
        return ops.tsm_unshift_add(dxs, res, N, T if T else 1, H * W, Cin, fold), None

    def _bn_bwd_g(self, dout, y, st, C, mbits, gout):
        bn = st.bn
        sums = torch.empty((2, C), dtype=torch.float32, device=y.device)
        dg, db = self._bn_grads(st)
        ops.bn_bwd_reduce(dout, None, y, st.mean, st.invstd, C, sums[0], sums[1], dg, db, mbits=mbits)
        return ops.bn_bwd_apply(dout, None, y, st.mean, st.invstd, bn.weight, sums[0], sums[1], C,
                                train_stats=st.mode != "running", mbits=mbits, gout=gout)
```

Baseline: 912.8 clip-windows/sec.

## Drop stored downsample conv output and fold its BN backward algebraically

Adds new kernels so the ResNet downsample branch no longer keeps its conv output for backward. The forward applies both BN affines inside one 1x1 conv kernel with the residual add and ReLU. The backward takes BN statistics from the weight-gradient product and folds BN into the weights for a two-operand dgrad GEMM, or recomputes the conv output inside a fused BN-backward apply kernel. The aim is to cut HBM traffic and activation memory for the downsample tensor, in exchange for extra GEMM work (Gram of x, recompute) and more complex gating paths.

```diff
diff --git a/include/vcg_hip.h b/include/vcg_hip.h
--- a/include/vcg_hip.h
+++ b/include/vcg_hip.h
@@ -54,10 +54,13 @@
                                       float* running_mean, float* running_var, float momentum, float eps,
                                       const float* w32, void* wfold, hipStream_t s);
 VCG_API int vcg_conv1x1_stats(const void* x, const void* w, float* stats, int M, int N, int K, hipStream_t stream);
-VCG_API int vcg_bn_bwd_sumgx_from_wgrad(const float* P, const void* w, int K, int C, const float* mean, const float* invstd, const float* sum_g, float* sum_gx, float* dgamma, hipStream_t stream);
+VCG_API int vcg_bn_bwd_sumgx_from_wgrad(const float* P, const void* w, int K, int C, const float* mean, const float* invstd, const float* sum_g, float* sum_gx, float* dgamma, float* dbeta, hipStream_t stream);
 VCG_API int vcg_bn_bwd_fold_weights_a2(const void* wt, int C, int K, const float* invstd, const float* gamma, const float* sum_g, const float* sum_gx, float inv_count, const float* colsum_a, void* wfold, float* bias, hipStream_t stream);
 VCG_API int vcg_bn_bwd_fold_wgrad_a2(const float* P, const float* G, const float* w3, int K, int C, const float* mean, const float* invstd, const float* gamma, const float* sum_g, const float* sum_gx, float inv_count, const float* colsum_a, float* dw, int accumulate, hipStream_t stream);
 VCG_API int vcg_conv_dgrad_bwd_bnfold(const void* g, const void* yg, int Ky, const void* wfold, const float* bias, void* out, int N, int H, int W, int C, int Cout, const void* y, const float* mean, const float* invstd, const float* mscale, const float* mshift, float* ws, long long ws_bytes, float* sum_g, float* sum_gx, float* dgamma, float* dbeta, hipStream_t stream);
+VCG_API int vcg_conv1x1_bn2_res_relu(const void* x, const void* w, const float* sx, const float* bx, const void* r, const float* sr, const float* br, void* out, unsigned char* bits, long long M, int N, int K, hipStream_t stream);
+VCG_API int vcg_conv1x1_bn_bwd_apply(const void* x, const void* w, const void* g, const float* mean, const float* invstd, const float* gamma, const float* sum_g, const float* sum_gx, void* dy, long long M, int N, int K, hipStream_t stream);
+VCG_API int vcg_conv_dgrad_bnfold(const void* g, const void* yg, int Ky, const void* wfold, const float* bias, void* out, long long M, int C, int Cout, hipStream_t stream);
 VCG_API long long vcg_conv_wgrad_bnfold_ws_bytes(int N, int H, int W, int C, int Cout);
 VCG_API int vcg_conv_wgrad_bnfold(const void* x, const void* g, const void* yg, const float* mean, const float* invstd, const float* gamma, const float* sum_g, const float* sum_gx, float inv_count, const float* colsum_x, float* dw, int accumulate, float* ws, long long ws_bytes, int N, int H, int W, int C, int Cout, hipStream_t stream);
 VCG_API int vcg_gemm(int dtype, int transA, int transB, int M, int N, int K, const void* A, long long lda, const void* B, long long ldb, void* C, long long ldc, const float* bias, int act, const void* residual, long long ldr, void* aux, float alpha, hipStream_t stream);
diff --git a/video-chapter-generation_amd/csrc/igemm.h b/video-chapter-generation_amd/csrc/igemm.h
--- a/video-chapter-generation_amd/csrc/igemm.h
+++ b/video-chapter-generation_amd/csrc/igemm.h
@@ -266,6 +266,11 @@
 int wgrad_patch_splits(int C, int Cout);
 int run_rs1x1_bnres(const void* x, const void* wfold, const float* bias, const void* res, void* out, uint8_t* bits,
                     long long M, int N, int K, hipStream_t s);
+int run_rs1x1_bn2res(const void* x, const void* w, const float* sx, const float* bx, const void* r, const float* sr,
+                     const float* br, void* out, uint8_t* bits, long long M, int N, int K, hipStream_t s);
+int run_rs1x1_bnbwd(const void* x, const void* w, const void* g, const float* mean, const float* invstd,
+                    const float* gamma, const float* sum_g, const float* sum_gx, float inv_count, void* dy, long long M,
+                    int N, int K, hipStream_t s);
 int run_wgrad_patch(const void* x, const void* dy, float* ws, int N, int H, int W, int C, int Cout, int R,
                     hipStream_t s);
 int wgrad_fast_tile_m(int M);
diff --git a/video-chapter-generation_amd/csrc/igemm.hip b/video-chapter-generation_amd/csrc/igemm.hip
--- a/video-chapter-generation_amd/csrc/igemm.hip
+++ b/video-chapter-generation_amd/csrc/igemm.hip
@@ -1136,7 +1136,7 @@
 __global__ __launch_bounds__(64) void bn_sumgx_kernel(const float* __restrict__ P, const bf16_t* __restrict__ w, int C,
                                                       const float* __restrict__ mean, const float* __restrict__ invstd,
                                                       const float* __restrict__ sum_g, float* __restrict__ sum_gx,
-                                                      float* __restrict__ dgamma) {
+                                                      float* __restrict__ dgamma, float* __restrict__ dbeta) {
   const int k = blockIdx.x, t = threadIdx.x;
   float a = 0.f;
   for (int j = t; j < C; j += 64) a = fmaf(bf2f(w[(long long)k * C + j]), P[(long long)k * C + j], a);
@@ -1146,17 +1146,18 @@
     const float v = invstd[k] * (a - mean[k] * sum_g[k]);
     sum_gx[k] = v;
     if (dgamma) dgamma[k] += v;
+    if (dbeta) dbeta[k] += sum_g[k];
   }
 }
 }
 
 VCG_API int vcg_bn_bwd_sumgx_from_wgrad(const float* P, const void* w, int K, int C, const float* mean,
                                         const float* invstd, const float* sum_g, float* sum_gx, float* dgamma,
-                                        hipStream_t stream) {
+                                        float* dbeta, hipStream_t stream) {
   VCG_REQUIRE(P && w && mean && invstd && sum_g && sum_gx, "null argument");
   VCG_REQUIRE(K > 0 && C > 0, "empty");
   hipLaunchKernelGGL(bn_sumgx_kernel, dim3(K), dim3(64), 0, stream, P, (const bf16_t*)w, C, mean, invstd, sum_g,
-                     sum_gx, dgamma);
+                     sum_gx, dgamma, dbeta);
   VCG_LAUNCH_CHECK();
   return VCG_OK;
 }
@@ -1235,6 +1236,68 @@
     if (rc) return rc;
   }
   return VCG_OK;
+}
+
+VCG_API int vcg_conv_dgrad_bnfold(const void* g, const void* yg, int Ky, const void* wfold, const float* bias,
+                                  void* out, long long M, int C, int Cout, hipStream_t stream) {
+  VCG_REQUIRE(g && yg && wfold && bias && out, "null argument");
+  VCG_REQUIRE(M > 0 && C % 64 == 0 && Cout % 64 == 0 && Ky % 64 == 0, "C, Cout and Ky must be multiples of 64");
+  VCG_REQUIRE((((uintptr_t)g | (uintptr_t)yg | (uintptr_t)wfold | (uintptr_t)out) & 15) == 0, "16-B alignment");
+  if (!fast_gemm_enabled() || M * C * 2 >= 0xFFFFFF00LL || M * Cout * 2 >= 0xFFFFFF00LL || M * Ky * 2 >= 0xFFFFFF00LL ||
+      M >= (1LL << 31))
+    return VCG_ERR_UNSUPPORTED;
+  GemmParams p{};
+  p.M = (int)M;
+  p.N = C;
+  p.K = Cout + Ky;
+  p.k_per_split = p.K + 64;
+  p.a = dense_op(g, Cout, p.M, Cout, 2);
+  p.a.ptr2 = yg;
+  p.a.split2 = Cout;
+  p.a.ld2 = Ky;
+  p.a.bytes2 = M * Ky * 2;
+  p.b = dense_op(wfold, p.K, C, p.K, 2);
+  p.bias = bias;
+  p.C = out;
+  p.ldc = C;
+  p.alpha = 1.f;
+  if (FILE* f = gemm_log()) {
+    fprintf(f, "a=0 b=0 epi=0 M=%d N=%d K=%d z=1 fast=1 conv=1x1/1 C=%d bnfold=1\n", p.M, p.N, p.K, Cout);
+    fflush(f);
+  }
+  const int rc = run_fast_gemm(p, OP_DENSE_K, EPI_STORE, 1, stream);
+  return rc < 0 ? VCG_ERR_UNSUPPORTED : rc;
+}
+
+VCG_API int vcg_conv1x1_bn2_res_relu(const void* x, const void* w, const float* sx, const float* bx, const void* r,
+                                     const float* sr, const float* br, void* out, unsigned char* bits, long long M,
+                                     int N, int K, hipStream_t stream) {
+  VCG_REQUIRE(x && w && sx && bx && r && sr && br && out && bits, "null argument");
+  VCG_REQUIRE(M > 0 && N > 0 && K > 0, "empty");
+  VCG_REQUIRE((((uintptr_t)x | (uintptr_t)w | (uintptr_t)r | (uintptr_t)out | (uintptr_t)bits) & 15) == 0,
+              "16-B alignment");
+  const int rc = run_rs1x1_bn2res(x, w, sx, bx, r, sr, br, out, bits, M, N, K, stream);
+  if (rc < 0) return VCG_ERR_UNSUPPORTED;
+  if (FILE* f = gemm_log()) {
+    fprintf(f, "a=0 b=0 epi=0 M=%lld N=%d K=%d z=1 fast=4 conv=1x1/1 C=%d bn2res=1\n", M, N, K, K);
+    fflush(f);
+  }
+  return rc;
+}
+
+VCG_API int vcg_conv1x1_bn_bwd_apply(const void* x, const void* w, const void* g, const float* mean,
+                                     const float* invstd, const float* gamma, const float* sum_g, const float* sum_gx,
+                                     void* dy, long long M, int N, int K, hipStream_t stream) {
+  VCG_REQUIRE(x && w && g && mean && invstd && sum_g && sum_gx && dy, "null argument");
+  VCG_REQUIRE(M > 0 && N > 0 && K > 0, "empty");
+  VCG_REQUIRE((((uintptr_t)x | (uintptr_t)w | (uintptr_t)g | (uintptr_t)dy) & 15) == 0, "16-B alignment");
+  const int rc = run_rs1x1_bnbwd(x, w, g, mean, invstd, gamma, sum_g, sum_gx, 1.f / (float)M, dy, M, N, K, stream);
+  if (rc < 0) return VCG_ERR_UNSUPPORTED;
+  if (FILE* f = gemm_log()) {
+    fprintf(f, "a=0 b=0 epi=0 M=%lld N=%d K=%d z=1 fast=4 conv=1x1/1 C=%d bnbwd=1\n", M, N, K, K);
+    fflush(f);
+  }
+  return rc;
 }
 
 VCG_API long long vcg_conv_wgrad_bnfold_ws_bytes(int N, int H, int W, int C, int Cout) {
diff --git a/video-chapter-generation_amd/csrc/igemm_fast.hip b/video-chapter-generation_amd/csrc/igemm_fast.hip
--- a/video-chapter-generation_amd/csrc/igemm_fast.hip
+++ b/video-chapter-generation_amd/csrc/igemm_fast.hip
@@ -309,7 +309,12 @@
 
 int run_fast_gemm(GemmParams& p, int amode, int epi, int z, hipStream_t s) {
   if (p.a.ptr2) {
-    if (amode != OP_DENSE_K || epi != EPI_BWD || z != 1 || !bwd_light(p) || p.a.split2 % FBK != 0) return -1;
+    if (amode != OP_DENSE_K || z != 1 || p.a.split2 % FBK != 0) return -1;
+    if (epi == EPI_STORE) {
+      if (p.residual || p.aux || p.act != ACT_NONE || (p.ldc & 7) != 0 || ((uintptr_t)p.C & 15) != 0) return -1;
+      return fast_bn<OP_DENSE_K2, EPI_STORE>(p, z, s);
+    }
+    if (epi != EPI_BWD || !bwd_light(p)) return -1;
     return fast_bn<OP_DENSE_K2, EPI_BWD_AFF>(p, z, s);
   }
   if (amode == OP_IM2COL && p.a.tsm_fold > 0) amode = OP_IM2COL_TSM;
diff --git a/video-chapter-generation_amd/csrc/stream1x1.hip b/video-chapter-generation_amd/csrc/stream1x1.hip
--- a/video-chapter-generation_amd/csrc/stream1x1.hip
+++ b/video-chapter-generation_amd/csrc/stream1x1.hip
@@ -1,3 +1,4 @@
+#include "bn_steps.h"
 #include "igemm.h"
 #include "mfma_util.h"
 
@@ -37,7 +38,7 @@
   for (int p = 0; p < RS_TN / 32; ++p) t.r[p] = *reinterpret_cast<const uint4*>(R + m * N + n0 + rs_col(p, g));
 }
 
-template <int K>
+template <int K, bool AFF2, bool BWD>
 __device__ __forceinline__ void rs_compute(const RsTile<K>& t, const bf16_t* Bs, const float* bias_s,
                                            bf16_t* __restrict__ out, uint8_t* __restrict__ bits, long long tile,
                                            long long M, int N, int n0, int lane) {
@@ -70,9 +71,14 @@
 #pragma unroll
       for (int h = 0; h < 2; ++h) {
         const int jj = 2 * pp + h, j = j0 + jj;
-        const float4 bv = *reinterpret_cast<const float4*>(bias_s + 16 * j + 4 * g);
-        vw[h][0] = (uint32_t)f2bf(acc[jj][0] + bv.x) | ((uint32_t)f2bf(acc[jj][1] + bv.y) << 16);
-        vw[h][1] = (uint32_t)f2bf(acc[jj][2] + bv.z) | ((uint32_t)f2bf(acc[jj][3] + bv.w) << 16);
+        if constexpr (AFF2 || BWD) {
+          vw[h][0] = (uint32_t)f2bf(acc[jj][0]) | ((uint32_t)f2bf(acc[jj][1]) << 16);
+          vw[h][1] = (uint32_t)f2bf(acc[jj][2]) | ((uint32_t)f2bf(acc[jj][3]) << 16);
+        } else {
+          const float4 bv = *reinterpret_cast<const float4*>(bias_s + 16 * j + 4 * g);
+          vw[h][0] = (uint32_t)f2bf(acc[jj][0] + bv.x) | ((uint32_t)f2bf(acc[jj][1] + bv.y) << 16);
+          vw[h][1] = (uint32_t)f2bf(acc[jj][2] + bv.z) | ((uint32_t)f2bf(acc[jj][3] + bv.w) << 16);
+        }
       }
 #pragma unroll
       for (int d = 0; d < 2; ++d) {
@@ -84,17 +90,41 @@
       float a8[8], r8[8];
       unpack8(cv, a8);
       unpack8(t.r[p], r8);
+      if constexpr (AFF2) {
+        float pv[4][8];
+#pragma unroll
+        for (int v = 0; v < 4; ++v) {
+          const float* pp_ = bias_s + v * RS_TN + rs_col(p, g);
+          const float4 lo = *reinterpret_cast<const float4*>(pp_), hi = *reinterpret_cast<const float4*>(pp_ + 4);
+          pv[v][0] = lo.x; pv[v][1] = lo.y; pv[v][2] = lo.z; pv[v][3] = lo.w;
+          pv[v][4] = hi.x; pv[v][5] = hi.y; pv[v][6] = hi.z; pv[v][7] = hi.w;
+        }
+#pragma unroll
+        for (int e = 0; e < 8; ++e) {
+          a8[e] = fmaf(a8[e], pv[0][e], pv[1][e]);
+          r8[e] = fmaf(r8[e], pv[2][e], pv[3][e]);
+        }
+      }
       uint32_t byte = 0;
-#pragma unroll
-      for (int e = 0; e < 8; ++e) {
-        a8[e] = fmaxf(a8[e] + r8[e], 0.f);
-        byte |= (a8[e] > 0.f ? 1u : 0u) << e;
+      if constexpr (BWD) {
+        float pv[3][8];
+#pragma unroll
+        for (int v = 0; v < 3; ++v) load_params<8>(bias_s + v * RS_TN, rs_col(p, g), pv[v]);
+#pragma unroll
+        for (int e = 0; e < 8; ++e) a8[e] = bn_bwd_map(true, pv[0][e], pv[1][e], pv[2][e], r8[e], a8[e]);
+      } else {
+#pragma unroll
+        for (int e = 0; e < 8; ++e) {
+          a8[e] = fmaxf(a8[e] + r8[e], 0.f);
+          byte |= (a8[e] > 0.f ? 1u : 0u) << e;
+        }
       }
       const uint4 o = pack8(a8);
       if (ok) *reinterpret_cast<uint4*>(out + m * N + n0 + rs_col(p, g)) = o;
       mb[p >> 2] |= byte << (8 * (p & 3));
     }
   }
+  if constexpr (BWD) return;
   uint32_t gm[4][2];
 #pragma unroll
   for (int w = 0; w < 2; ++w) {
@@ -117,13 +147,18 @@
   }
 }
 
-template <int K>
+template <int K, bool AFF2, bool BWD = false>
 __global__ __launch_bounds__(RS_NTH) void rs1x1_bnres_kernel(const bf16_t* __restrict__ X, const bf16_t* __restrict__ W,
                                                             const float* __restrict__ bias,
+                                                            const float* __restrict__ aff1, const float* __restrict__ aff2,
+                                                            const float* __restrict__ aff3,
                                                             const bf16_t* __restrict__ R, bf16_t* __restrict__ out,
-                                                            uint8_t* __restrict__ bits, long long M, int N) {
+                                                            uint8_t* __restrict__ bits, long long M, int N,
+                                                            const float* __restrict__ sum_gx = nullptr,
+                                                            float inv_count = 0.f) {
+  constexpr int NV = AFF2 ? 4 : BWD ? 3 : 1;
   __shared__ __attribute__((aligned(1024))) bf16_t Bs[RS_TN * K];
-  __shared__ __attribute__((aligned(16))) float bias_s[RS_TN];
+  __shared__ __attribute__((aligned(16))) float bias_s[NV * RS_TN];
   const int ncb = N / RS_TN;
   const int cb = blockIdx.x % ncb, q = blockIdx.x / ncb, nq = gridDim.x / ncb;
   const int n0 = cb * RS_TN;
@@ -133,7 +168,22 @@
     const uint4 v = *reinterpret_cast<const uint4*>(W + (long long)(n0 + row) * K + 8 * ch);
     *reinterpret_cast<uint4*>(Bs + (ch >> 3) * RS_TN * 64 + row * 64 + 8 * rswz(row, ch & 7)) = v;
   }
-  for (int c = tid; c < RS_TN; c += RS_NTH) bias_s[c] = bias[n0 + c];
+  if constexpr (BWD) {
+    for (int c = tid; c < RS_TN; c += RS_NTH) {
+      const int n = n0 + c;
+      bn_bwd_coef(aff2 ? aff2[n] : 1.f, aff1[n], sum_gx[n], aff3[n], bias[n], inv_count, bias_s[c], bias_s[RS_TN + c],
+                  bias_s[2 * RS_TN + c]);
+    }
+  } else {
+    for (int c = tid; c < RS_TN; c += RS_NTH) bias_s[c] = bias[n0 + c];
+  }
+  if constexpr (AFF2) {
+    for (int c = tid; c < RS_TN; c += RS_NTH) {
+      bias_s[RS_TN + c] = aff1[n0 + c];
+      bias_s[2 * RS_TN + c] = aff2[n0 + c];
+      bias_s[3 * RS_TN + c] = aff3[n0 + c];
+    }
+  }
   __syncthreads();
   const long long ntiles = (M + 15) / 16;
   const long long stride = (long long)nq * (RS_NTH / 64);
@@ -144,10 +194,10 @@
   rs_load<K>(T0, X, R, t, M, N, n0, lane);
   for (; t < ntiles; t += 2 * stride) {
     rs_load<K>(T1, X, R, min(t + stride, last), M, N, n0, lane);
-    rs_compute<K>(T0, Bs, bias_s, out, bits, t, M, N, n0, lane);
+    rs_compute<K, AFF2, BWD>(T0, Bs, bias_s, out, bits, t, M, N, n0, lane);
     if (t + stride >= ntiles) break;
     rs_load<K>(T0, X, R, min(t + 2 * stride, last), M, N, n0, lane);
-    rs_compute<K>(T1, Bs, bias_s, out, bits, t + stride, M, N, n0, lane);
+    rs_compute<K, AFF2, BWD>(T1, Bs, bias_s, out, bits, t + stride, M, N, n0, lane);
   }
 }
 
@@ -166,17 +216,61 @@
   if ((e && e[0] == '0') || (K != 64 && K != 128 && K != 256) || N % RS_TN != 0 || N / RS_TN > 8 || M <= 0) return -1;
   const int g = rs_grid(N);
   if (census_on()) { char t_[96]; snprintf(t_, sizeof(t_), "rs1x1_bnres"); census_add(t_, M, N, K); }
+  const float* no = nullptr;
   if (K == 64)
-    hipLaunchKernelGGL(rs1x1_bnres_kernel<64>, dim3(g), dim3(RS_NTH), 0, s, (const bf16_t*)x, (const bf16_t*)wfold,
-                       bias, (const bf16_t*)res, (bf16_t*)out, bits, M, N);
+    hipLaunchKernelGGL((rs1x1_bnres_kernel<64, false>), dim3(g), dim3(RS_NTH), 0, s, (const bf16_t*)x,
+                       (const bf16_t*)wfold, bias, no, no, no, (const bf16_t*)res, (bf16_t*)out, bits, M, N);
   else if (K == 128)
-    hipLaunchKernelGGL(rs1x1_bnres_kernel<128>, dim3(g), dim3(RS_NTH), 0, s, (const bf16_t*)x, (const bf16_t*)wfold,
-                       bias, (const bf16_t*)res, (bf16_t*)out, bits, M, N);
+    hipLaunchKernelGGL((rs1x1_bnres_kernel<128, false>), dim3(g), dim3(RS_NTH), 0, s, (const bf16_t*)x,
+                       (const bf16_t*)wfold, bias, no, no, no, (const bf16_t*)res, (bf16_t*)out, bits, M, N);
   else
-    hipLaunchKernelGGL(rs1x1_bnres_kernel<256>, dim3(g), dim3(RS_NTH), 0, s, (const bf16_t*)x, (const bf16_t*)wfold,
-                       bias, (const bf16_t*)res, (bf16_t*)out, bits, M, N);
+    hipLaunchKernelGGL((rs1x1_bnres_kernel<256, false>), dim3(g), dim3(RS_NTH), 0, s, (const bf16_t*)x,
+                       (const bf16_t*)wfold, bias, no, no, no, (const bf16_t*)res, (bf16_t*)out, bits, M, N);
   VCG_LAUNCH_CHECK();
   return VCG_OK;
 }
 
-}
+int run_rs1x1_bn2res(const void* x, const void* w, const float* sx, const float* bx, const void* r, const float* sr,
+                     const float* br, void* out, uint8_t* bits, long long M, int N, int K, hipStream_t s) {
+  const char* e = getenv("VCG_RS1X1");
+  if ((e && e[0] == '0') || (K != 64 && K != 128 && K != 256) || N % RS_TN != 0 || N / RS_TN > 8 || M <= 0) return -1;
+  const int g = rs_grid(N);
+  if (census_on()) { char t_[96]; snprintf(t_, sizeof(t_), "rs1x1_bn2res"); census_add(t_, M, N, K); }
+  if (K == 64)
+    hipLaunchKernelGGL((rs1x1_bnres_kernel<64, true>), dim3(g), dim3(RS_NTH), 0, s, (const bf16_t*)x,
+                       (const bf16_t*)w, sx, bx, sr, br, (const bf16_t*)r, (bf16_t*)out, bits, M, N);
+  else if (K == 128)
+    hipLaunchKernelGGL((rs1x1_bnres_kernel<128, true>), dim3(g), dim3(RS_NTH), 0, s, (const bf16_t*)x,
+                       (const bf16_t*)w, sx, bx, sr, br, (const bf16_t*)r, (bf16_t*)out, bits, M, N);
+  else
+    hipLaunchKernelGGL((rs1x1_bnres_kernel<256, true>), dim3(g), dim3(RS_NTH), 0, s, (const bf16_t*)x,
+                       (const bf16_t*)w, sx, bx, sr, br, (const bf16_t*)r, (bf16_t*)out, bits, M, N);
+  VCG_LAUNCH_CHECK();
+  return VCG_OK;
+}
+
+int run_rs1x1_bnbwd(const void* x, const void* w, const void* g, const float* mean, const float* invstd,
+                    const float* gamma, const float* sum_g, const float* sum_gx, float inv_count, void* dy, long long M,
+                    int N, int K, hipStream_t s) {
+  const char* e = getenv("VCG_RS1X1");
+  if ((e && e[0] == '0') || (K != 64 && K != 128 && K != 256) || N % RS_TN != 0 || N / RS_TN > 8 || M <= 0) return -1;
+  const int gr = rs_grid(N);
+  if (census_on()) { char t_[96]; snprintf(t_, sizeof(t_), "rs1x1_bnbwd"); census_add(t_, M, N, K); }
+  uint8_t* nobits = nullptr;
+  if (K == 64)
+    hipLaunchKernelGGL((rs1x1_bnres_kernel<64, false, true>), dim3(gr), dim3(RS_NTH), 0, s, (const bf16_t*)x,
+                       (const bf16_t*)w, mean, invstd, gamma, sum_g, (const bf16_t*)g, (bf16_t*)dy, nobits, M, N, sum_gx,
+                       inv_count);
+  else if (K == 128)
+    hipLaunchKernelGGL((rs1x1_bnres_kernel<128, false, true>), dim3(gr), dim3(RS_NTH), 0, s, (const bf16_t*)x,
+                       (const bf16_t*)w, mean, invstd, gamma, sum_g, (const bf16_t*)g, (bf16_t*)dy, nobits, M, N, sum_gx,
+                       inv_count);
+  else
+    hipLaunchKernelGGL((rs1x1_bnres_kernel<256, false, true>), dim3(gr), dim3(RS_NTH), 0, s, (const bf16_t*)x,
+                       (const bf16_t*)w, mean, invstd, gamma, sum_g, (const bf16_t*)g, (bf16_t*)dy, nobits, M, N, sum_gx,
+                       inv_count);
+  VCG_LAUNCH_CHECK();
+  return VCG_OK;
+}
+
+}
diff --git a/video-chapter-generation_amd/vcg_hip/ops.py b/video-chapter-generation_amd/vcg_hip/ops.py
--- a/video-chapter-generation_amd/vcg_hip/ops.py
+++ b/video-chapter-generation_amd/vcg_hip/ops.py
@@ -233,11 +233,11 @@
     return True
 
 
-def bn_bwd_sumgx_from_wgrad(Pg, w, K, C, mean, invstd, sum_g, sum_gx, dgamma=None):
+def bn_bwd_sumgx_from_wgrad(Pg, w, K, C, mean, invstd, sum_g, sum_gx, dgamma=None, dbeta=None):
     _chk(Pg, torch.float32, "Pg")
     _chk(w, torch.bfloat16, "w")
     _lib.call("vcg_bn_bwd_sumgx_from_wgrad", P(Pg), P(w), K, C, P(mean), P(invstd), P(sum_g), P(sum_gx), P(dgamma),
-              stream())
+              P(dbeta), stream())
 
 
 def conv1x1_bn_res_relu(x, wfold, bias, res, M, N, K, res_scale=None, res_shift=None):
@@ -252,6 +252,55 @@
     if rc != 0:
         raise _lib.VcgError(f"vcg_conv1x1_bn_res_relu failed ({rc}): {_lib.last_error()}")
     return out, bits
+
+
+def conv1x1_bn2_res_relu(x, w, sx, bx, r, sr, br, M, N, K):
+    _chk(x, torch.bfloat16, "x")
+    _chk(w, torch.bfloat16, "w")
+    _chk(r, torch.bfloat16, "r")
+    for t, n in ((sx, "sx"), (bx, "bx"), (sr, "sr"), (br, "br")):
+        _chk(t, torch.float32, n)
+        assert t.numel() == N
+    assert x.numel() == M * K and w.numel() == N * K and r.numel() == M * N
+    out = torch.empty_like(r)
+    bits = torch.empty(r.numel() // 8, dtype=torch.uint8, device=r.device)
+    rc = _lib.query("vcg_conv1x1_bn2_res_relu", P(x), P(w), P(sx), P(bx), P(r), P(sr), P(br), P(out), P(bits), M, N, K,
+                    stream())
+    if rc == -2:
+        return None
+    if rc != 0:
+        raise _lib.VcgError(f"vcg_conv1x1_bn2_res_relu failed ({rc}): {_lib.last_error()}")
+    return out, bits
+
+
+def conv1x1_bn_bwd_apply(x, w, g, mean, invstd, gamma, sum_g, sum_gx, M, N, K):
+    _chk(x, torch.bfloat16, "x")
+    _chk(w, torch.bfloat16, "w")
+    _chk(g, torch.bfloat16, "g")
+    assert x.numel() == M * K and w.numel() == N * K and g.numel() == M * N
+    dy = torch.empty_like(g)
+    rc = _lib.query("vcg_conv1x1_bn_bwd_apply", P(x), P(w), P(g), P(mean), P(invstd), P(gamma), P(sum_g), P(sum_gx),
+                    P(dy), M, N, K, stream())
+    if rc == -2:
+        return None
+    if rc != 0:
+        raise _lib.VcgError(f"vcg_conv1x1_bn_bwd_apply failed ({rc}): {_lib.last_error()}")
+    return dy
+
+
+def conv_dgrad_bnfold(g, yg, wfold, bias, M, C, Cout, Ky):
+    _chk(g, torch.bfloat16, "g")
+    _chk(yg, torch.bfloat16, "yg")
+    _chk(wfold, torch.bfloat16, "wfold")
+    _chk(bias, torch.float32, "bias")
+    assert g.numel() == M * Cout and yg.numel() == M * Ky and wfold.numel() == C * (Cout + Ky) and bias.numel() == C
+    out = torch.empty((M, C), dtype=g.dtype, device=g.device)
+    rc = _lib.query("vcg_conv_dgrad_bnfold", P(g), P(yg), int(Ky), P(wfold), P(bias), P(out), M, C, Cout, stream())
+    if rc == -2:
+        return None
+    if rc != 0:
+        raise _lib.VcgError(f"vcg_conv_dgrad_bnfold failed ({rc}): {_lib.last_error()}")
+    return out
 
 
 def bn_bwd_fold_weights(wt, N, K, mean, invstd, gamma, sum_g, sum_gx, count):
diff --git a/video-chapter-generation_amd/vcg_hip/trunk.py b/video-chapter-generation_amd/vcg_hip/trunk.py
--- a/video-chapter-generation_amd/vcg_hip/trunk.py
+++ b/video-chapter-generation_amd/vcg_hip/trunk.py
@@ -99,6 +99,8 @@
     fused_stem_bwd = True
     dgrad_p = True
     gram_fin = True
+    ds_xform = False
+    ds_onepass = True
 
     def __init__(self, net, dtype):
         self.net = net
@@ -231,13 +233,15 @@
             return self._block_fwd_folded(blk, x, conv1, T, fold, N, H, W)
         yd = bd = side = None
         cur = torch.cuda.current_stream() if x.is_cuda else None
+        dsx = blk.downsample is not None and self._ds_xform_ok(blk, x, planes, need_grad)
         if blk.downsample is not None:
             side = self._wside(x.device) if self.ds_stream else None
             if side is not None:
                 side.wait_stream(cur)
                 with torch.cuda.stream(side):
-                    yd, bd, _, _ = self._conv_bn(x, blk.downsample[0], blk.downsample[1], N, H, W, Cin)
-                yd.record_stream(cur)
+                    yd, bd, _, _ = self._conv_bn(x, blk.downsample[0], blk.downsample[1], N, H, W, Cin, store=not dsx)
+                if yd is not None:
+                    yd.record_stream(cur)
                 bd.vec.record_stream(cur)
         y1, b1, _, _ = self._conv_bn(x, conv1, blk.bn1, N, H, W, Cin, T, fold)
         a1 = ops.bn_apply(y1, b1.scale, b1.shift, planes, relu=True)
@@ -268,9 +272,19 @@
             if side is not None:
                 cur.wait_stream(side)
             else:
-                yd, bd, _, _ = self._conv_bn(x, blk.downsample[0], blk.downsample[1], N, H, W, Cin)
-            out, obits = ops.bn_apply(y3, b3.scale, b3.shift, C3, relu=True, res=yd, rscale=bd.scale,
-                                      rshift=bd.shift, bits=True)
+                yd, bd, _, _ = self._conv_bn(x, blk.downsample[0], blk.downsample[1], N, H, W, Cin, store=not dsx)
+            rd = None
+            if yd is None or self._ds_onepass_ok(blk, x):
+                M = N * H2 * W2
+                rd = ops.conv1x1_bn2_res_relu(x.view(M, Cin), self._wprep(blk.downsample[0], Cin), bd.scale, bd.shift,
+                                              y3, b3.scale, b3.shift, M, C3, Cin)
+                if rd is None and yd is None:
+                    yd = self._ds_out(blk, x, N, H, W, Cin)
+            if rd is not None:
+                out, obits = rd
+            else:
+                out, obits = ops.bn_apply(y3, b3.scale, b3.shift, C3, relu=True, res=yd, rscale=bd.scale,
+                                          rshift=bd.shift, bits=True)
         else:
             if (self.dtype == torch.bfloat16 and C3 <= ResNetTrunk.bn3_gemm_max_c3
                     and b3.mode != "running" and blk.conv3.stride[0] == 1):
@@ -298,6 +312,33 @@
         C3 = blk.conv3.out_channels
         return ops.conv_fwd(a2, self._wprep(blk.conv3, planes), N, H2, W2, planes, C3, 1, 1, 1, 0)
 
+    def _ds_xform_ok(self, blk, x, planes, need_grad):
+        C3 = blk.downsample[0].out_channels
+        return (ResNetTrunk.ds_xform and need_grad and self._ds_pass_shape(blk, x)
+                and ResNetTrunk.fused_bwd and ResNetTrunk.bn_fold_bwd and C3 <= ResNetTrunk.bn_fold_max_c3
+                and planes >= 64 and (planes & (planes - 1)) == 0)
+
+    def _ds_pass_shape(self, blk, x):
+        cds, bnd = blk.downsample[0], blk.downsample[1]
+        C3, Cin = cds.out_channels, cds.in_channels
+        return (x.is_cuda and self.dtype == torch.bfloat16
+                and bn_mode(bnd) != "running" and bn_mode(blk.bn3) != "running"
+                and _conv_shape(cds)[2:] == (1, 1, 1, 0) and blk.conv2.stride[0] == 1 and blk.conv3.stride[0] == 1
+                and Cin in (64, 128, 256) and C3 % 256 == 0 and C3 <= 2048)
+
+    def _ds_onepass_ok(self, blk, x):
+        return ResNetTrunk.ds_onepass and self._ds_pass_shape(blk, x)
+
+    def _ds_out(self, blk, x, N, H, W, Cin):
+        cds = blk.downsample[0]
+        Cd, _, KH, KW, s, p = _conv_shape(cds)
+        return ops.conv_fwd(x, self._wprep(cds, Cin), N, H, W, Cin, Cd, KH, KW, s, p)
+
+    def _yd(self, r):
+        if r["yd"] is None:
+            r["yd"] = self._ds_out(r["blk"], r["x"], r["N"], r["H"], r["W"], r["Cin"])
+        return r["yd"]
+
     def _y3(self, r):
         if r["y3"] is None:
             r["y3"] = self._conv3_out(r["blk"], r["a2"], r["N"], r["H2"], r["W2"], r["planes"])
@@ -431,6 +472,43 @@
         self._hold((dyd,))
         res.record_stream(cur)
         return res, res_stride, ev
+
+    def _ds_xform_bwd(self, r, g, sumsd):
+        blk, bd, x = r["blk"], r["bd"], r["x"]
+        cds, bnd = blk.downsample[0], blk.downsample[1]
+        N, H, W, Cin, C3 = r["N"], r["H"], r["W"], r["Cin"], r["C3"]
+        M = N * H * W
+
+        def fn():
+            Pd = torch.empty((C3, Cin, 1, 1), dtype=torch.float32, device=x.device)
+            ops.conv_wgrad(x, g, Pd, N, H, W, Cin, Cin, C3, 1, 1, 1, 0, accumulate=False)
+            dgd, dbd = self._bn_grads(bd)
+            ops.bn_bwd_sumgx_from_wgrad(Pd.view(C3, Cin), self._wprep(cds, Cin), C3, Cin, bd.mean, bd.invstd,
+                                        sumsd[0], sumsd[1], dgd, dbeta=dbd)
+            cs = torch.empty(Cin, dtype=torch.float32, device=x.device)
+            ops.colsum(x.view(M, Cin), Cin, M, Cin, cs, accumulate=False)
+            wfold, bias = ops.bn_bwd_fold_weights_a2(self._wprep_t(cds, Cin).view(Cin, C3), Cin, C3, bd.invstd,
+                                                     bnd.weight, sumsd[0], sumsd[1], M, cs)
+            res = ops.conv_dgrad_bnfold(g.view(M, C3), x.view(M, Cin), wfold, bias, M, Cin, C3, Cin)
+            if res is None:
+                raise RuntimeError("ds_xform: the folded downsample input gradient (vcg_conv_dgrad_bnfold) does not "
+                                   "apply to a shape its forward accepted")
+            ev = torch.cuda.Event()
+            ev.record(torch.cuda.current_stream())
+            if cds.weight.requires_grad:
+                Gx = torch.empty((Cin, Cin, 1, 1), dtype=torch.float32, device=x.device)
+                ops.conv_wgrad(x, x, Gx, N, H, W, Cin, Cin, Cin, 1, 1, 1, 0, accumulate=False)
+                ops.bn_bwd_fold_wgrad_a2(Pd.view(C3, Cin), Gx.view(Cin, Cin), cds.weight.data.view(C3, Cin), C3, Cin,
+                                         bd.mean, bd.invstd, bnd.weight, sumsd[0], sumsd[1], M, cs,
+                                         cds.weight.grad.view(C3, Cin))
+            return res.view(N, H, W, Cin), ev
+
+        if self._ws is not None and self.ds_stream:
+            res, ev = self._async(fn, x, g, bd.vec, *sumsd)
+            res.record_stream(torch.cuda.current_stream())
+        else:
+            res, ev = fn()
+        return res, 1, ev
 
     def _wgrad(self, conv, x, dy, N, H, W, Cpad, T=0, fold=0):
         if not conv.weight.requires_grad:
@@ -585,6 +663,8 @@
         obits = r["obits"]
         ds = blk.downsample is not None
         bnf = None
+        ds_res = None
+        dsx = ds and r["yd"] is None and gin is not None
         if gin is not None:
             g, sums3, sumsd = gin
             b3, bd = r["b3"], r.get("bd")
@@ -596,14 +676,26 @@
                 ops.bn_bwd_sumgx_from_wgrad(Pg.view(C3, planes), self._wprep(blk.conv3, planes), C3, planes, b3.mean,
                                             b3.invstd, sums3[0], sums3[1], self._bn_grads(b3)[0])
                 r["Pg"] = Pg
+            if dsx and not self._can_fold(r, ds):
+                raise RuntimeError("ds_xform: the forward kept no downsample conv output, but bn3's backward fold "
+                                   "(bn_fold_bwd / fused_bwd) was switched off before the backward")
             if self._can_fold(r, ds):
                 bnf = (g, sums3)
                 dy3 = dyd = None
-                if ds:
+                if dsx:
+                    ds_res = self._ds_xform_bwd(r, g, sumsd)
+                elif ds:
                     def dyd_fn():
+                        if self._ds_onepass_ok(blk, r["x"]):
+                            M = N * H * W
+                            d = ops.conv1x1_bn_bwd_apply(r["x"].view(M, Cin), self._wprep(blk.downsample[0], Cin), g,
+                                                         bd.mean, bd.invstd, bd.bn.weight, sumsd[0], sumsd[1], M, C3,
+                                                         Cin)
+                            if d is not None:
+                                return d
                         return self._bn_apply_bwd(g, r["yd"], bd, C3, sumsd)
                     if self._ws is not None and self.ds_stream:
-                        dyd = self._async(dyd_fn, g, r["yd"], bd.vec, *sumsd)
+                        dyd = self._async(dyd_fn, g, r["yd"], r["x"], bd.vec, *sumsd)
                     else:
                         dyd = dyd_fn()
             elif ResNetTrunk.dual_bn_bwd and ds and b3.mode != "running" and bd.mode != "running":
@@ -615,9 +707,8 @@
         else:
             g = torch.empty_like(dout)
             dy3 = self._bn_bwd_g(dout, self._y3(r), r["b3"], C3, obits, g)
-            dyd = self._bn_bwd(dout, r["yd"], r["bd"], C3, mbits=obits) if ds else None
-        ds_res = None
-        if ds and self._ws is not None and self.ds_stream:
+            dyd = self._bn_bwd(dout, self._yd(r), r["bd"], C3, mbits=obits) if ds else None
+        if ds and not dsx and self._ws is not None and self.ds_stream:
             ds_res = self._ds_dgrad_side(blk.downsample[0], dyd, N, H, W, Cin, C3)
         if bnf is not None and not self._fold_conv3(r, *bnf):
             dy3 = self._bn_apply_bwd(bnf[0], self._y3(r), r["b3"], C3, bnf[1])
@@ -643,7 +734,8 @@
         self._wgrad(r["conv1"], r["x"], dy1, N, H, W, Cin, T, fold)
         res_stride = 1
         if ds and ds_res is not None:
-            self._wgrad(blk.downsample[0], r["x"], dyd, N, H, W, Cin)
+            if not dsx:
+                self._wgrad(blk.downsample[0], r["x"], dyd, N, H, W, Cin)
             res, res_stride, ev = ds_res
             torch.cuda.current_stream().wait_event(ev)
         elif ds:
@@ -672,9 +764,10 @@
                       dgamma=dg, dbeta=db)
             if prev["blk"].downsample is not None:
                 sumsd = (s3[0], s3[2])
-                dg2, db2 = self._bn_grads(prev["bd"])
-                kw.update(y2=prev["yd"], mean2=prev["bd"].mean, invstd2=prev["bd"].invstd, sum_gx2=s3[2],
-                          dgamma2=dg2, dbeta2=db2)
+                if prev["yd"] is not None:
+                    dg2, db2 = self._bn_grads(prev["bd"])
+                    kw.update(y2=prev["yd"], mean2=prev["bd"].mean, invstd2=prev["bd"].invstd, sum_gx2=s3[2],
+                              dgamma2=dg2, dbeta2=db2)
         pg = None
         if (ResNetTrunk.fused_bwd and ResNetTrunk.dgrad_p and prev is not None and prev["y3"] is None
                 and prev["blk"].downsample is None and prev["a2"] is not None and prev["planes"] == 64
```

Result: faster. 922.3 clip-windows/sec, median of 6 (+1.0%).
